# ratschlab/secedo

Hardware: AMD Instinct MI355X
Metric: cell-pair x locus updates/sec (similarity matrix) (higher is better)
Workload: dtype int64; 1 GPU; C3: 8000 cells x 100000 loci; entries=24345058, kept_entries=24223307, reads=23997029, block_cells=128, tiles=2016, normalization=ADD_MIN, max_fragment_length=1000, num_threads=8, parallelism=single GPU, backend=none, world_size=1, rccl_world_size=1

## Files before the change

include/secedo_simmat.h:

```cpp
#ifndef SECEDO_SIMMAT_H
#define SECEDO_SIMMAT_H

#include <stdint.h>

#ifdef __cplusplus
extern "C" {
#endif

#define SECEDO_OK 0
#define SECEDO_E_INVALID_ARG (-1)
#define SECEDO_E_INVALID_NORMALIZATION (-2)
#define SECEDO_E_NO_DEVICE (-3)
#define SECEDO_E_HIP (-4)
#define SECEDO_E_STATE (-5)
#define SECEDO_E_LIMIT (-6)

#define SECEDO_NORM_ADD_MIN 0
#define SECEDO_NORM_EXPONENTIATE 1
#define SECEDO_NORM_SCALE_MAX_1 2

int secedo_simmat_normalization_from_string(const char *name);

const char *secedo_simmat_last_error(void);
const char *secedo_simmat_version(void);
int secedo_simmat_device_count(void);

int secedo_simmat_compute(const uint32_t *chr_locus_off, uint32_t n_chr, const uint32_t *locus_pos,
                          const uint64_t *locus_entry_off, const uint32_t *read_ids,
                          const uint16_t *id_base16, const uint32_t *id_base32,
                          const uint32_t *group_id_to_pos, uint32_t n_groups, uint32_t num_cells,
                          uint32_t max_fragment_length, double mutation_rate,
                          double homozygous_rate, double seq_error_rate, uint32_t num_threads,
                          int normalization, double *out);
int secedo_simmat_set_devices(const int *device_ids, uint32_t n_devices);
int secedo_simmat_get_devices(int *device_ids, uint32_t capacity);

int secedo_simmat_staging_acquire(const uint64_t bytes[5], void *ptrs[5]);
void secedo_simmat_staging_release(void);

void secedo_simmat_release_cache(void);

typedef struct secedo_simmat secedo_simmat_t;

int secedo_simmat_create(secedo_simmat_t **handle, int device_id);
void secedo_simmat_destroy(secedo_simmat_t *handle);

int secedo_simmat_set_pileup(secedo_simmat_t *handle, const uint32_t *chr_locus_off, uint32_t n_chr,
                             const uint32_t *locus_pos, const uint64_t *locus_entry_off,
                             const uint32_t *read_ids, const uint16_t *id_base16,
                             const uint32_t *id_base32, const uint32_t *group_id_to_pos,
                             uint32_t n_groups);

int secedo_simmat_set_pileup_device(secedo_simmat_t *handle, const uint32_t *d_chr_locus_off,
                                    uint32_t n_chr, const uint32_t *d_locus_pos,
                                    const uint64_t *d_locus_entry_off, const uint32_t *d_read_ids,
                                    const uint16_t *d_id_base16, const uint32_t *d_id_base32,
                                    const uint32_t *d_group_id_to_pos, uint32_t n_groups,
                                    uint32_t n_loci, uint64_t n_entries);

int secedo_simmat_set_packing(secedo_simmat_t *handle, int mode);
int secedo_simmat_used_device_packing(const secedo_simmat_t *handle);

int secedo_simmat_prepare(secedo_simmat_t *handle, uint32_t num_cells, uint32_t max_fragment_length,
                          uint32_t num_threads, uint32_t block_cells, void *stream);

uint32_t secedo_simmat_num_tiles(const secedo_simmat_t *handle);
uint32_t secedo_simmat_block_cells(const secedo_simmat_t *handle);
uint64_t secedo_simmat_acc_elems(const secedo_simmat_t *handle);
uint64_t secedo_simmat_num_entries(const secedo_simmat_t *handle);
uint64_t secedo_simmat_num_reads(const secedo_simmat_t *handle);
uint64_t secedo_simmat_num_loci(const secedo_simmat_t *handle);

uint64_t secedo_simmat_pair_bound(const secedo_simmat_t *handle);
uint32_t secedo_simmat_max_read_entries(const secedo_simmat_t *handle);
int secedo_simmat_cell_squares(secedo_simmat_t *handle, uint64_t *d_out , void *stream);
int secedo_simmat_set_scale_bounds(secedo_simmat_t *handle, uint64_t pair_bound, uint32_t max_read_entries);
int secedo_simmat_set_pair_bound(secedo_simmat_t *handle, uint64_t pair_bound);
int secedo_simmat_scale_bounds_state(const secedo_simmat_t *handle);
int secedo_simmat_scale_log2(const secedo_simmat_t *handle);

int secedo_simmat_zero_acc(secedo_simmat_t *handle, int64_t *d_acc, void *stream);
int secedo_simmat_accumulate(secedo_simmat_t *handle, double mutation_rate, double homozygous_rate,
                             double seq_error_rate, uint32_t tile_begin, uint32_t tile_end,
                             int64_t *d_acc, void *stream);
int secedo_simmat_assign(secedo_simmat_t *handle, double mutation_rate, double homozygous_rate,
                         double seq_error_rate, uint32_t tile_begin, uint32_t tile_end, int64_t *d_acc,
                         void *stream);
int secedo_simmat_finalize(secedo_simmat_t *handle, int normalization, const int64_t *d_acc,
                           double *d_out, void *stream);
int secedo_simmat_assign_finalize(secedo_simmat_t *handle, double mutation_rate, double homozygous_rate,
                                  double seq_error_rate, int normalization, int64_t *d_acc, double *d_out,
                                  void *stream);
int secedo_simmat_tiles_of_rows(const secedo_simmat_t *handle, uint32_t row_begin, uint32_t row_end,
                                uint32_t *tile_ids, uint32_t *n_tile_ids);
int secedo_simmat_accumulate_list(secedo_simmat_t *handle, double mutation_rate, double homozygous_rate,
                                  double seq_error_rate, const uint32_t *tile_ids, uint32_t n_tile_ids,
                                  int64_t *d_acc, void *stream);
int secedo_simmat_assign_list(secedo_simmat_t *handle, double mutation_rate, double homozygous_rate,
                              double seq_error_rate, const uint32_t *tile_ids, uint32_t n_tile_ids,
                              int64_t *d_acc, void *stream);
int secedo_simmat_max_of_tiles(secedo_simmat_t *handle, const int64_t *d_acc, const uint32_t *tile_ids,
                               uint32_t n_tile_ids, double *max_value, void *stream);
int secedo_simmat_finalize_rows_max(secedo_simmat_t *handle, int normalization, const int64_t *d_acc,
                                    uint32_t row_begin, uint32_t row_end, double max_value, double *d_out_rows,
                                    void *stream);
int secedo_simmat_finalize_rows(secedo_simmat_t *handle, int normalization, const int64_t *d_acc,
                                uint32_t row_begin, uint32_t row_end, double *d_out_rows, void *stream);
int secedo_simmat_finalize_raw(secedo_simmat_t *handle, const int64_t *d_acc, double *d_out,
                               void *stream);

int secedo_simmat_last_counts(secedo_simmat_t *handle, uint64_t *updates, uint64_t *read_pairs);
int secedo_simmat_last_accumulate_ms(secedo_simmat_t *handle, float *ms);
int secedo_simmat_last_pair_kernel_ms(secedo_simmat_t *handle, float *ms);
const char *secedo_simmat_pair_kernel(const secedo_simmat_t *handle);
int secedo_simmat_last_correction_fused(const secedo_simmat_t *handle);
int secedo_simmat_last_locus_words(const secedo_simmat_t *handle);
uint32_t secedo_simmat_last_workgroups(const secedo_simmat_t *handle);
int secedo_simmat_debug_flag_lists(secedo_simmat_t *handle, uint64_t *n_flagged, uint32_t *grp, uint32_t *rec,
                                   uint32_t *idx);

double secedo_simmat_llr(uint32_t x_s, uint32_t x_d, double mutation_rate, double homozygous_rate,
                         double seq_error_rate);
double secedo_simmat_llr_closed_form(uint32_t x_s, uint32_t x_d, double mutation_rate, double homozygous_rate,
                                     double seq_error_rate);

int secedo_is_significant(const uint16_t *base_count , double seq_error_rate,
                          uint32_t cell_proportion);

int secedo_filter(const uint32_t *chr_locus_off, uint32_t n_chr, const uint32_t *locus_pos,
                  const uint64_t *locus_entry_off, const uint32_t *read_ids, const uint16_t *id_base16,
                  const uint32_t *id_base32, const uint32_t *id_to_pos, uint32_t n_groups,
                  double seq_error_rate, uint32_t cell_proportion, uint32_t *out_chr_locus_off,
                  uint32_t *out_locus_pos, uint64_t *out_locus_entry_off, uint32_t *out_read_ids,
                  void *out_id_base, uint64_t *out_n_loci, uint64_t *out_n_entries, double *avg_coverage);

int secedo_filter_device(const uint32_t *d_chr_locus_off, uint32_t n_chr, const uint32_t *d_locus_pos,
                         const uint64_t *d_locus_entry_off, const uint32_t *d_read_ids,
                         const uint16_t *d_id_base16, const uint32_t *d_id_base32, const uint32_t *d_id_to_pos,
                         uint32_t n_groups, uint32_t n_loci, uint64_t n_entries, double seq_error_rate,
                         uint32_t cell_proportion, uint32_t *d_out_chr_locus_off, uint32_t *d_out_locus_pos,
                         uint64_t *d_out_locus_entry_off, uint32_t *d_out_read_ids, void *d_out_id_base,
                         uint64_t *out_n_loci, uint64_t *out_n_entries, double *avg_coverage, void *stream);

typedef struct secedo_pileup_info {
    uint64_t n_loci;
    uint64_t n_entries;
    uint32_t num_cells;
    uint32_t max_read_length;
} secedo_pileup_info;

int secedo_pileup_read(const char *path, const uint16_t *id_to_group, uint32_t n_ids, uint32_t max_coverage,
                       const uint32_t *positions, uint64_t n_positions, int compute_max_read_len,
                       int write_bin, secedo_pileup_info *info, uint32_t *locus_pos,
                       uint64_t *locus_entry_off, uint32_t *read_ids, uint16_t *id_base16);
const char *secedo_pileup_last_error(void);

#ifdef __cplusplus
}
#endif
#endif
```

secedo_amd/_lib.py:

```python
from __future__ import annotations

import ctypes as C
import os

import numpy as np

HERE = os.path.dirname(os.path.abspath(__file__))
LIB_PATH = os.environ.get("SECEDO_LIB_PATH") or os.path.join(HERE, "libsecedo_simmat.so")

OK = 0
E_INVALID_ARG = -1
E_INVALID_NORMALIZATION = -2
E_NO_DEVICE = -3
E_HIP = -4
E_STATE = -5
E_LIMIT = -6

_u16p = C.POINTER(C.c_uint16)
_u32p = C.POINTER(C.c_uint32)
_u64p = C.POINTER(C.c_uint64)
_f64p = C.POINTER(C.c_double)
_vp = C.c_void_p


class PileupInfo(C.Structure):
    _fields_ = [("n_loci", C.c_uint64), ("n_entries", C.c_uint64), ("num_cells", C.c_uint32),
                ("max_read_length", C.c_uint32)]


class SpectralInfo(C.Structure):
    _fields_ = [("cycles", C.c_uint32), ("block_products", C.c_uint32), ("converged", C.c_uint32),
                ("reserved", C.c_uint32), ("max_residual_vectors", C.c_double),
                ("max_residual_values", C.c_double)]


ALLREDUCE_SUM_FN = C.CFUNCTYPE(C.c_int, C.c_void_p, C.c_void_p, C.c_uint64, C.c_void_p)


class SynthSpec(C.Structure):
    _fields_ = [
        ("num_cells", C.c_uint32), ("num_loci", C.c_uint32), ("num_chromosomes", C.c_uint32),
        ("gap_max", C.c_uint32), ("new_frag_prob", C.c_double), ("frag_min", C.c_uint32),
        ("frag_max", C.c_uint32), ("base_error", C.c_double), ("mate_frac", C.c_double),
        ("seed", C.c_uint64),
    ]


SIGNATURES = {
    "secedo_simmat_normalization_from_string": (C.c_int, [C.c_char_p]),
    "secedo_simmat_last_error": (C.c_char_p, []),
    "secedo_simmat_version": (C.c_char_p, []),
    "secedo_simmat_device_count": (C.c_int, []),
    "secedo_simmat_compute": (C.c_int, [_vp, C.c_uint32, _vp, _vp, _vp, _vp, _vp, _vp, C.c_uint32,
                                        C.c_uint32, C.c_uint32, C.c_double, C.c_double, C.c_double,
                                        C.c_uint32, C.c_int, _vp]),
    "secedo_simmat_release_cache": (None, []),
    "secedo_simmat_staging_acquire": (C.c_int, [_vp, _vp]),
    "secedo_simmat_staging_release": (None, []),
    "secedo_simmat_create": (C.c_int, [C.POINTER(_vp), C.c_int]),
    "secedo_simmat_destroy": (None, [_vp]),
    "secedo_simmat_set_pileup": (C.c_int, [_vp, _vp, C.c_uint32, _vp, _vp, _vp, _vp, _vp, _vp,
                                           C.c_uint32]),
    "secedo_simmat_set_pileup_device": (C.c_int, [_vp, _vp, C.c_uint32, _vp, _vp, _vp, _vp, _vp, _vp,
                                                  C.c_uint32, C.c_uint32, C.c_uint64]),
    "secedo_simmat_set_packing": (C.c_int, [_vp, C.c_int]),
    "secedo_simmat_used_device_packing": (C.c_int, [_vp]),
    "secedo_simmat_prepare": (C.c_int, [_vp, C.c_uint32, C.c_uint32, C.c_uint32, C.c_uint32, _vp]),
    "secedo_simmat_num_tiles": (C.c_uint32, [_vp]),
    "secedo_simmat_block_cells": (C.c_uint32, [_vp]),
    "secedo_simmat_acc_elems": (C.c_uint64, [_vp]),
    "secedo_simmat_num_entries": (C.c_uint64, [_vp]),
    "secedo_simmat_num_reads": (C.c_uint64, [_vp]),
    "secedo_simmat_num_loci": (C.c_uint64, [_vp]),
    "secedo_simmat_zero_acc": (C.c_int, [_vp, _vp, _vp]),
    "secedo_simmat_accumulate": (C.c_int, [_vp, C.c_double, C.c_double, C.c_double, C.c_uint32,
                                           C.c_uint32, _vp, _vp]),
    "secedo_simmat_finalize": (C.c_int, [_vp, C.c_int, _vp, _vp, _vp]),
    "secedo_simmat_tiles_of_rows": (C.c_int, [_vp, C.c_uint32, C.c_uint32, _vp, C.POINTER(C.c_uint32)]),
    "secedo_simmat_assign": (C.c_int, [_vp, C.c_double, C.c_double, C.c_double, C.c_uint32, C.c_uint32, _vp, _vp]),
    "secedo_simmat_assign_list": (C.c_int, [_vp, C.c_double, C.c_double, C.c_double, _vp, C.c_uint32, _vp, _vp]),
    "secedo_simmat_assign_finalize": (C.c_int, [_vp, C.c_double, C.c_double, C.c_double, C.c_int, _vp, _vp, _vp]),
    "secedo_simmat_accumulate_list": (C.c_int, [_vp, C.c_double, C.c_double, C.c_double, _vp, C.c_uint32, _vp, _vp]),
    "secedo_simmat_max_of_tiles": (C.c_int, [_vp, _vp, _vp, C.c_uint32, C.POINTER(C.c_double), _vp]),
    "secedo_simmat_finalize_rows_max": (C.c_int, [_vp, C.c_int, _vp, C.c_uint32, C.c_uint32, C.c_double, _vp, _vp]),
    "secedo_simmat_finalize_rows": (C.c_int, [_vp, C.c_int, _vp, C.c_uint32, C.c_uint32, _vp, _vp]),
    "secedo_simmat_finalize_raw": (C.c_int, [_vp, _vp, _vp, _vp]),
    "secedo_simmat_last_counts": (C.c_int, [_vp, _u64p, _u64p]),
    "secedo_simmat_last_accumulate_ms": (C.c_int, [_vp, C.POINTER(C.c_float)]),
    "secedo_simmat_last_pair_kernel_ms": (C.c_int, [_vp, C.POINTER(C.c_float)]),
    "secedo_simmat_pair_kernel": (C.c_char_p, [_vp]),
    "secedo_simmat_last_correction_fused": (C.c_int, [_vp]),
    "secedo_simmat_last_locus_words": (C.c_int, [_vp]),
    "secedo_simmat_last_workgroups": (C.c_uint32, [_vp]),
    "secedo_simmat_debug_flag_lists": (C.c_int, [_vp, _u64p, _vp, _vp, _vp]),
    "secedo_simmat_llr": (C.c_double, [C.c_uint32, C.c_uint32, C.c_double, C.c_double, C.c_double]),
    "secedo_simmat_llr_closed_form": (C.c_double, [C.c_uint32, C.c_uint32, C.c_double, C.c_double, C.c_double]),
    "secedo_simmat_pair_bound": (C.c_uint64, [_vp]),
    "secedo_simmat_set_pair_bound": (C.c_int, [_vp, C.c_uint64]),
    "secedo_simmat_max_read_entries": (C.c_uint32, [_vp]),
    "secedo_simmat_cell_squares": (C.c_int, [_vp, _vp, _vp]),
    "secedo_simmat_set_scale_bounds": (C.c_int, [_vp, C.c_uint64, C.c_uint32]),
    "secedo_simmat_scale_log2": (C.c_int, [_vp]),
    "secedo_simmat_scale_bounds_state": (C.c_int, [_vp]),
    "secedo_simmat_set_devices": (C.c_int, [C.POINTER(C.c_int), C.c_uint32]),
    "secedo_simmat_get_devices": (C.c_int, [C.POINTER(C.c_int), C.c_uint32]),
    "secedo_is_significant": (C.c_int, [_vp, C.c_double, C.c_uint32]),
    "secedo_filter": (C.c_int, [_vp, C.c_uint32, _vp, _vp, _vp, _vp, _vp, _vp, C.c_uint32, C.c_double,
                                C.c_uint32, _vp, _vp, _vp, _vp, _vp, _u64p, _u64p, _f64p]),
    "secedo_filter_device": (C.c_int, [_vp, C.c_uint32, _vp, _vp, _vp, _vp, _vp, _vp, C.c_uint32, C.c_uint32,
                                       C.c_uint64, C.c_double, C.c_uint32, _vp, _vp, _vp, _vp, _vp, _u64p,
                                       _u64p, _f64p, _vp]),
    "secedo_pileup_read": (C.c_int, [C.c_char_p, _vp, C.c_uint32, C.c_uint32, _vp, C.c_uint64, C.c_int, C.c_int,
                                     C.POINTER(PileupInfo), _vp, _vp, _vp, _vp]),
    "secedo_pileup_last_error": (C.c_char_p, []),
    "secedo_em_refine_device": (C.c_int, [C.c_int, _vp, C.c_uint32, C.c_uint64, _vp, _vp, _vp, C.c_uint32, C.c_double,
                                          _vp, C.c_uint32, C.c_uint32, C.POINTER(C.c_uint32), _vp]),
    "secedo_em_refine": (C.c_int, [C.c_int, _vp, C.c_uint32, _vp, _vp, _vp, C.c_uint32, C.c_double, _vp, C.c_uint32,
                                   C.c_uint32, C.POINTER(C.c_uint32)]),
    "secedo_laplacian_device": (C.c_int, [_vp, C.c_uint32, _vp, _vp]),
    "secedo_spectral_eigs_device": (C.c_int, [C.c_int, _vp, C.c_uint32, C.c_uint32, C.c_uint32, C.c_double,
                                              C.c_uint32, _vp, _vp, C.POINTER(SpectralInfo), _vp]),
    "secedo_spectral_eigs_rows_device": (C.c_int, [C.c_int, _vp, C.c_uint32, C.c_uint32, C.c_uint32, C.c_uint32,
                                                   C.c_uint32, C.c_double, C.c_uint32, _vp, _vp,
                                                   C.POINTER(SpectralInfo), _vp, _vp, _vp]),
    "secedo_spectral_eigs": (C.c_int, [C.c_int, _vp, C.c_uint32, C.c_uint32, C.c_uint32, C.c_double, C.c_uint32,
                                       _vp, _vp, C.POINTER(SpectralInfo)]),
}

_lib = None


class SecedoError(RuntimeError):
    def __init__(self, code, message):
        super().__init__("secedo_simmat error %d: %s" % (code, message))
        self.code = code


class InvalidNormalization(ValueError):
    """The reference throws std::logic_error here (similarity_matrix.cpp:264)."""


def lib():
    global _lib
    if _lib is None:
        if not os.path.exists(LIB_PATH):
            raise ImportError(
                "%s is missing: build it with `python -c 'import __graft_entry__ as g; g.build()'` "
                "or `make -C secedo_amd/csrc` (there is no fallback implementation)" % LIB_PATH)
        try:
            import torch
        except ImportError:
            pass
        l = C.CDLL(LIB_PATH)
        for name, (res, args) in SIGNATURES.items():
            f = getattr(l, name)
            f.restype = res
            f.argtypes = args
        _lib = l
    return _lib


def check(rc):
    if rc == OK:
        return
    msg = lib().secedo_simmat_last_error().decode(errors="replace")
    if rc == E_INVALID_NORMALIZATION:
        raise InvalidNormalization(msg)
    raise SecedoError(rc, msg)


def ptr(a):
    return None if a is None else a.ctypes.data
```

secedo_amd/csrc/pack_device.hip:

```cpp
#include "pack_device.hpp"

#include <hip/hip_runtime.h>
#include <hipcub/hipcub.hpp>

#include <algorithm>
#include <chrono>
#include <cstdio>
#include <cstdlib>
#include <cstring>
#include <functional>

namespace secedo {

DeviceArena::~DeviceArena() {
    if (p) (void)hipFree(p);
}

DevicePacked::~DevicePacked() {
    if (side) (void)hipStreamDestroy(side);
    if (ev_fork) (void)hipEventDestroy(ev_fork);
    if (ev_join) (void)hipEventDestroy(ev_join);
    if (ev_offsets) (void)hipEventDestroy(ev_offsets);
    if (ev_flush) (void)hipEventDestroy(ev_flush);
    if (mailbox) (void)hipHostFree(mailbox);
// ... 20 lines not shown
}

namespace {

constexpr int TPB = 256;

inline uint32_t blocks_for(uint64_t n) {
    return static_cast<uint32_t>(std::max<uint64_t>(1, std::min<uint64_t>((n + TPB - 1) / TPB, 1u << 16)));
}

struct Scalars {
    uint32_t error;
    uint32_t need_host;
    uint32_t num_ranges;
    uint32_t max_read_id;
    uint32_t regroup;
    uint32_t long_reads;
    uint32_t split_changed;
    uint32_t id_exceeded;
    uint32_t max_read_entries;
    uint32_t caps_wrong;
    uint32_t n_multi_id;
    uint32_t reads_total;
    uint32_t n_wide;
    uint32_t max_range_span;
    unsigned long long id_space;
    unsigned long long multi_entries;
    unsigned long long pair_bound;
};

struct Mailbox {
    Scalars sc;
    unsigned long long totals;
    unsigned long long seq;
};

__global__ void k_publish(const Scalars *sc, const unsigned long long *totals, Mailbox *box, unsigned long long seq) {
    if (threadIdx.x == 0) {
        box->sc = *sc;
        box->totals = totals ? *totals : 0ull;
        __hip_atomic_store(&box->seq, seq, __ATOMIC_RELEASE, __HIP_MEMORY_SCOPE_SYSTEM);
    }
}

hipError_t read_scalars(DevicePacked &pk, hipStream_t stream, const Scalars *sc, const unsigned long long *totals,
                        Scalars *out, unsigned long long *out_totals, const std::function<void()> &behind = nullptr) {
    static const bool plain = [] {
        const char *e = std::getenv("SECEDO_PACK_READBACK");
        return e && std::strcmp(e, "memcpy") == 0;
    }();
    hipError_t e;
    if (!plain && !pk.mailbox && !pk.mailbox_failed) {
        if (hipHostMalloc(&pk.mailbox, sizeof(Mailbox), hipHostMallocCoherent) == hipSuccess) {
            std::memset(pk.mailbox, 0, sizeof(Mailbox));
        } else {
            (void)hipGetLastError();
            pk.mailbox = nullptr;
            pk.mailbox_failed = true;
        }
    }
    if (!plain && pk.mailbox) {
        Mailbox *box = static_cast<Mailbox *>(pk.mailbox);
        const unsigned long long seq = ++pk.mailbox_seq;
        hipLaunchKernelGGL(k_publish, dim3(1), dim3(64), 0, stream, sc, totals, box, seq);
        if ((e = hipGetLastError()) != hipSuccess) return e;
        if (behind) behind();
        bool arrived = false;
        for (unsigned spins = 0;; ++spins) {
            if (__atomic_load_n(&box->seq, __ATOMIC_ACQUIRE) == seq) {
                arrived = true;
                break;
            }
            if ((spins & 0xFFFu) == 0xFFFu) {
                const hipError_t q = hipStreamQuery(stream);
                if (q != hipErrorNotReady) {
                    arrived = __atomic_load_n(&box->seq, __ATOMIC_ACQUIRE) == seq;
                    if (q != hipSuccess) return q;
                    break;
                }
            }
        }
        if (arrived) {
            *out = box->sc;
            if (out_totals) *out_totals = box->totals;
            return hipSuccess;
        }
    } else if (behind) {
        behind();
    }
    if (out_totals) {
        *out_totals = 0;
        if (totals && (e = hipMemcpyAsync(out_totals, totals, 8, hipMemcpyDeviceToHost, stream)) != hipSuccess) return e;
    }
    if ((e = hipMemcpyAsync(out, sc, sizeof(*out), hipMemcpyDeviceToHost, stream)) != hipSuccess) return e;
    return hipStreamSynchronize(stream);
}

struct HostTrace {
    bool on;
    std::chrono::steady_clock::time_point t0;
    HostTrace() : on(std::getenv("SECEDO_PACK_TRACE") != nullptr), t0(std::chrono::steady_clock::now()) {}
    void mark(const char *what) const {
        if (on)
            std::fprintf(stderr, "[pack-trace] %8.1f us  %s\n",
                         std::chrono::duration<double, std::micro>(std::chrono::steady_clock::now() - t0).count(), what);
    }
};

constexpr uint32_t kRankScanLimit = 8192;
constexpr int kNoRetry = 0, kRetryRadix = 1, kRetrySameScheme = 2;
constexpr int kMaxSplitRounds = 32;
constexpr uint32_t kIdSpaceFactor = 4;

struct Raw {
    const uint32_t *chr_locus_off;
    uint32_t n_chr;
    const uint32_t *locus_pos;
    const uint64_t *locus_entry_off;
    const uint32_t *read_ids;
    const uint16_t *id_base16;
    const uint32_t *id_base32;
    const uint32_t *g2p;
    uint32_t n_groups;
    uint32_t n_loci;
    uint32_t n_entries;
    __device__ __forceinline__ uint32_t id_base(uint32_t e) const {
        return id_base16 ? (uint32_t)id_base16[e] : id_base32[e];
    }
};

template <class T>
__device__ __forceinline__ uint32_t last_le(const T *a, uint32_t n, T x) {
    uint32_t lo = 0, hi = n;
    while (hi - lo > 1) {
        const uint32_t mid = lo + (hi - lo) / 2;
        if (a[mid] <= x) lo = mid; else hi = mid;
    }
    return lo;
}

__global__ __launch_bounds__(TPB) void k_entry_locus(Raw in, uint32_t *entry_locus, Scalars *sc) {
    const uint32_t lane = threadIdx.x & 63u;
    const uint32_t wave = (blockIdx.x * TPB + threadIdx.x) >> 6, n_waves = (gridDim.x * TPB) >> 6;
    for (uint32_t l = wave; l < in.n_loci; l += n_waves) {
        const uint32_t b = (uint32_t)in.locus_entry_off[l], e = (uint32_t)in.locus_entry_off[l + 1];
        for (uint32_t i = b + lane; i < e; i += 64u) entry_locus[i] = l;
        if (lane == 0u && l + 1 < in.n_loci && in.locus_pos[l + 1] <= in.locus_pos[l]) {
            const uint32_t c = last_le<uint32_t>(in.chr_locus_off, in.n_chr + 1, l);
            if (l + 1 < in.chr_locus_off[c + 1]) sc->error = 3;
        }
    }
}

__global__ __launch_bounds__(TPB) void k_id_range(Raw in, const uint32_t *entry_locus, uint32_t *id_max,
                                                 uint32_t *id_negmin, int vec) {
    __shared__ uint32_t s_hi[TPB / 64], s_neg[TPB / 64];
    const uint32_t E = in.n_entries;
    const uint32_t chunk = (E + gridDim.x - 1) / gridDim.x;
    uint32_t cur = min(E, blockIdx.x * chunk);
    const uint32_t e1 = min(E, cur + chunk);
    if (cur >= e1) return;
    uint32_t c = last_le<uint32_t>(in.chr_locus_off, in.n_chr + 1, entry_locus[cur]);
    while (cur < e1) {
        uint32_t c_end = (uint32_t)in.locus_entry_off[in.chr_locus_off[c + 1]];
        while (c_end <= cur && c + 1 < in.n_chr) {
            ++c;
            c_end = (uint32_t)in.locus_entry_off[in.chr_locus_off[c + 1]];
        }
        const uint32_t seg_end = (c + 1 < in.n_chr) ? min(e1, c_end) : e1;
        uint32_t hi = 0, neg = 0;
        uint32_t s_cur = cur, s_end = seg_end;
        if (vec) {
            const uint32_t a = min(seg_end, (cur + 3u) & ~3u), b = max(a, seg_end & ~3u);
            if (threadIdx.x < a - cur) {
                const uint32_t id = in.read_ids[cur + threadIdx.x];
                hi = max(hi, id);
                neg = max(neg, ~id);
            }
            if (threadIdx.x < seg_end - b) {
                const uint32_t id = in.read_ids[b + threadIdx.x];
                hi = max(hi, id);
                neg = max(neg, ~id);
            }
            const uint4 *src = reinterpret_cast<const uint4 *>(in.read_ids);
            for (uint32_t q = a / 4u + threadIdx.x; q < b / 4u; q += TPB * 4) {
                uint4 v[4];
#pragma unroll
                for (int u = 0; u < 4; ++u) v[u] = q + (uint32_t)u * TPB < b / 4u ? src[q + (uint32_t)u * TPB] : src[q];
#pragma unroll
                for (int u = 0; u < 4; ++u) {
                    hi = max(max(hi, v[u].x), max(max(v[u].y, v[u].z), v[u].w));
                    neg = max(max(neg, ~v[u].x), max(max(~v[u].y, ~v[u].z), ~v[u].w));
                }
            }
            s_cur = s_end = seg_end;
        }
        for (uint32_t e = s_cur + threadIdx.x; e < s_end; e += TPB * 8) {
            uint32_t id[8];
#pragma unroll
            for (int u = 0; u < 8; ++u) {
                const uint32_t eu = e + (uint32_t)u * TPB;
                id[u] = eu < s_end ? in.read_ids[eu] : in.read_ids[e];
            }
#pragma unroll
            for (int u = 0; u < 8; ++u) {
                hi = max(hi, id[u]);
                neg = max(neg, ~id[u]);
            }
        }
        for (int off = 32; off > 0; off >>= 1) {
            hi = max(hi, (uint32_t)__shfl_down(hi, off));
            neg = max(neg, (uint32_t)__shfl_down(neg, off));
        }
        __syncthreads();
        if ((threadIdx.x & 63u) == 0) {
            s_hi[threadIdx.x >> 6] = hi;
            s_neg[threadIdx.x >> 6] = neg;
        }
        __syncthreads();
        if (threadIdx.x == 0) {
            for (int w = 1; w < TPB / 64; ++w) {
                hi = max(hi, s_hi[w]);
                neg = max(neg, s_neg[w]);
            }
            atomicMax(&id_max[c], hi);
            atomicMax(&id_negmin[c], neg);
        }
        cur = seg_end;
    }
}

__global__ void k_id_bases(uint32_t n_chr, const uint32_t *id_max, const uint32_t *id_negmin, uint32_t *id_base,
                           unsigned long long assumed_space, Scalars *sc) {
    if (threadIdx.x != 0 || blockIdx.x != 0) return;
    unsigned long long sum = 0;
    uint32_t top = 0;
    for (uint32_t c = 0; c < n_chr; ++c) {
        id_base[c] = (uint32_t)min(sum, 0xFFFFFFFFull);
        const uint32_t lo = ~id_negmin[c];
        if ((id_max[c] | id_negmin[c]) != 0u) sum += (unsigned long long)(id_max[c] - lo) + 1ull;
        top = max(top, id_max[c]);
    }
    id_base[n_chr] = (uint32_t)min(sum, 0xFFFFFFFFull);
    sc->id_space = sum;
    sc->max_read_id = top;
    if (assumed_space && sum > assumed_space) sc->id_exceeded = 1;
}

__global__ void k_entry_keys(Raw in, const uint32_t *entry_locus, uint32_t id_bits, unsigned long long *key,
                             uint32_t *val) {
    for (uint32_t e = blockIdx.x * TPB + threadIdx.x; e < in.n_entries; e += gridDim.x * TPB) {
        const uint32_t c = last_le<uint32_t>(in.chr_locus_off, in.n_chr + 1, entry_locus[e]);
        key[e] = ((unsigned long long)c << id_bits) | in.read_ids[e];
        val[e] = e;
    }
}

constexpr uint32_t kSlocLocusMask = 0x3FFFFFFFu;
__device__ __forceinline__ uint32_t sloc_pack(uint32_t locus, uint32_t id_base) { return locus | (id_base << 30); }
__device__ __forceinline__ uint32_t sloc_locus(uint32_t v) { return v & kSlocLocusMask; }
__device__ __forceinline__ uint32_t sloc_base(uint32_t v) { return v >> 30; }

__global__ void k_sorted_locus(Raw in, const uint32_t *sval, const uint32_t *entry_locus, uint32_t n, uint32_t *sloc) {
    for (uint32_t s = blockIdx.x * TPB + threadIdx.x; s < n; s += gridDim.x * TPB)
        sloc[s] = sloc_pack(entry_locus[sval[s]], in.id_base(sval[s]));
}

constexpr uint32_t kChrLds = 1024;
struct ChrTables {
    uint32_t first[kChrLds + 1], base[kChrLds], min_id[kChrLds];
};
__device__ __forceinline__ bool chr_tables_load(const Raw &in, const uint32_t *id_base, const uint32_t *id_negmin,
                                                ChrTables &t) {
    const bool in_lds = in.n_chr <= kChrLds;
    if (in_lds) {
        for (uint32_t i = threadIdx.x; i <= in.n_chr; i += blockDim.x) t.first[i] = in.chr_locus_off[i];
        for (uint32_t i = threadIdx.x; i < in.n_chr; i += blockDim.x) {
            t.base[i] = id_base[i];
            t.min_id[i] = ~id_negmin[i];
        }
    }
    __syncthreads();
    return in_lds;
}
__device__ __forceinline__ uint32_t dense_id(const Raw &in, const uint32_t *id_base, const uint32_t *id_negmin,
                                             const ChrTables &t, bool in_lds, uint32_t locus, uint32_t id) {
    if (in_lds) {
        const uint32_t c = last_le<uint32_t>(t.first, in.n_chr + 1, locus);
        return t.base[c] + (id - t.min_id[c]);
    }
    const uint32_t c = last_le<uint32_t>(in.chr_locus_off, in.n_chr + 1, locus);
    return id_base[c] + (id - ~id_negmin[c]);
}

__global__ void k_id_hist(Raw in, const uint32_t *entry_locus, const uint32_t *id_base, const uint32_t *id_negmin,
                          const Scalars *sc, uint32_t *dense, uint32_t *hist) {
    if (sc->id_exceeded) return;
    __shared__ ChrTables tables;
    const bool in_lds = chr_tables_load(in, id_base, id_negmin, tables);
    for (uint32_t e = blockIdx.x * TPB + threadIdx.x; e < in.n_entries; e += gridDim.x * TPB) {
        const uint32_t d = dense_id(in, id_base, id_negmin, tables, in_lds, entry_locus[e], in.read_ids[e]);
        dense[e] = d;
        atomicAdd(&hist[d], 1u);
    }
}

__global__ void k_id_scatter(const uint32_t *dense, uint32_t n, const uint32_t *id_off, const Scalars *sc,
                             uint32_t *hist, uint32_t *grouped) {
    if (sc->id_exceeded) return;
    for (uint32_t e = blockIdx.x * TPB + threadIdx.x; e < n; e += gridDim.x * TPB) {
        const uint32_t d = dense[e];
        grouped[id_off[d] + atomicSub(&hist[d], 1u) - 1u] = e;
    }
}

__global__ void k_id_rank(Raw in, const uint32_t *dense, const uint32_t *id_off, const uint32_t *grouped,
                          const uint32_t *entry_locus, unsigned long long *skey, uint32_t *sval, uint32_t *sloc,
                          Scalars *sc) {
    const bool void_run = sc->id_exceeded != 0;
    for (uint32_t p = blockIdx.x * TPB + threadIdx.x; p < in.n_entries; p += gridDim.x * TPB) {
        if (void_run) {
            skey[p] = p;
            sval[p] = p;
            sloc[p] = 0;
            continue;
        }
        const uint32_t e = grouped[p];
        const uint32_t d = dense[e];
        const uint32_t b = id_off[d], n = id_off[d + 1] - b;
        uint32_t rank = p - b;
        if (n > kRankScanLimit) {
            sc->regroup = 1;
        } else if (n > 1) {
            rank = 0;
            for (uint32_t q = b; q < b + n; ++q) rank += grouped[q] < e ? 1u : 0u;
        }
        skey[b + rank] = d;
        sval[b + rank] = e;
        sloc[b + rank] = sloc_pack(entry_locus[e], in.id_base(e));
    }
}

constexpr uint32_t kFlagBlock = 4096;
__global__ void k_id_store(Raw in, const uint32_t *entry_locus, const uint32_t *id_base, const uint32_t *id_negmin,
                           const Scalars *sc, uint32_t *dense, uint32_t *last, int vec) {
    if (sc->id_exceeded) return;
    __shared__ ChrTables tables;
    const bool in_lds = chr_tables_load(in, id_base, id_negmin, tables);
    const uint32_t n = in.n_entries, stride = gridDim.x * TPB;
    for (uint32_t q = blockIdx.x * TPB + threadIdx.x; q < (n + 3u) / 4u; q += stride) {
        const uint32_t e0 = q * 4u;
        uint32_t l[4], id[4], d[4];
        if (vec && e0 + 4u <= n) {
            const uint4 lv = reinterpret_cast<const uint4 *>(entry_locus)[q];
            const uint4 iv = reinterpret_cast<const uint4 *>(in.read_ids)[q];
            l[0] = lv.x, l[1] = lv.y, l[2] = lv.z, l[3] = lv.w;
            id[0] = iv.x, id[1] = iv.y, id[2] = iv.z, id[3] = iv.w;
        } else {
#pragma unroll
            for (int u = 0; u < 4; ++u) {
                const uint32_t e = min(e0 + (uint32_t)u, n - 1u);
                l[u] = entry_locus[e];
                id[u] = in.read_ids[e];
            }
        }
#pragma unroll
        for (int u = 0; u < 4; ++u) d[u] = dense_id(in, id_base, id_negmin, tables, in_lds, l[u], id[u]);
        if (e0 + 4u <= n) {
            reinterpret_cast<uint4 *>(dense)[q] = make_uint4(d[0], d[1], d[2], d[3]);
#pragma unroll
            for (int u = 0; u < 4; ++u) last[d[u]] = e0 + (uint32_t)u + 1u;
        } else {
            for (uint32_t u = 0; e0 + u < n; ++u) {
                dense[e0 + u] = d[u];
                last[d[u]] = e0 + u + 1u;
            }
        }
    }
}
__global__ void k_id_check(uint32_t n, const Scalars *sc, const uint32_t *dense, const uint32_t *last, uint8_t *multi) {
    if (sc->id_exceeded) return;
    const uint32_t stride = gridDim.x * TPB;
    for (uint32_t q = blockIdx.x * TPB + threadIdx.x; q < (n + 3u) / 4u; q += stride) {
        const uint32_t e0 = q * 4u;
        uint32_t d[4], w[4];
        if (e0 + 4u <= n) {
            const uint4 dv = reinterpret_cast<const uint4 *>(dense)[q];
            d[0] = dv.x, d[1] = dv.y, d[2] = dv.z, d[3] = dv.w;
        } else {
#pragma unroll
            for (int u = 0; u < 4; ++u) d[u] = dense[min(e0 + (uint32_t)u, n - 1u)];
        }
#pragma unroll
        for (int u = 0; u < 4; ++u) w[u] = last[d[u]];
#pragma unroll
        for (int u = 0; u < 4; ++u) {
            const uint32_t e = e0 + (uint32_t)u;
            if (e < n && w[u] != e + 1u) {
                multi[e] = 1;
                multi[w[u] - 1u] = 1;
            }
        }
    }
}
__global__ __launch_bounds__(TPB) void k_flag_count(const uint8_t *multi, uint32_t *block_sum) {
    __shared__ uint32_t part[TPB / 64];
    static_assert(kFlagBlock == TPB * 16, "a thread takes 16 consecutive flags");
    const uint4 w = reinterpret_cast<const uint4 *>(multi + (size_t)blockIdx.x * kFlagBlock)[threadIdx.x];
    uint32_t n = ((w.x * 0x01010101u) >> 24) + ((w.y * 0x01010101u) >> 24) + ((w.z * 0x01010101u) >> 24)
            + ((w.w * 0x01010101u) >> 24);
    for (int off = 32; off > 0; off >>= 1) n += __shfl_down(n, off);
    if ((threadIdx.x & 63u) == 0u) part[threadIdx.x >> 6] = n;
    __syncthreads();
    if (threadIdx.x == 0u) {
        for (int w2 = 1; w2 < TPB / 64; ++w2) n += part[w2];
        block_sum[blockIdx.x] = n;
    }
}
constexpr int TPB_SCAN = 1024;
__global__ __launch_bounds__(TPB_SCAN) void k_flag_scan(const uint32_t *block_sum, uint32_t n_blocks, uint32_t *block_off,
                                                       uint32_t *m_idx_end, Scalars *sc) {
    constexpr int TPB = TPB_SCAN;
    __shared__ uint32_t part[TPB / 64];
    __shared__ uint32_t carry;
    if (threadIdx.x == 0u) carry = 0;
    __syncthreads();
    const uint32_t lane = threadIdx.x & 63u, wv = threadIdx.x >> 6;
    for (uint32_t base = 0; base < n_blocks; base += TPB) {
        const uint32_t i = base + threadIdx.x;
        const uint32_t v = i < n_blocks ? block_sum[i] : 0u;
        uint32_t incl = v;
        for (int off = 1; off < 64; off <<= 1) {
            const uint32_t up = __shfl_up(incl, off);
            if (lane >= (uint32_t)off) incl += up;
        }
        if (lane == 63u) part[wv] = incl;
        __syncthreads();
        uint32_t before = carry;
        for (uint32_t w2 = 0; w2 < wv; ++w2) before += part[w2];
        if (i < n_blocks) block_off[i] = before + incl - v;
        __syncthreads();
        if (threadIdx.x == TPB - 1) carry = before + incl;
        __syncthreads();
    }
    if (threadIdx.x == 0u) {
        *m_idx_end = carry;
        if (sc) sc->n_multi_id = carry;
    }
}
__global__ __launch_bounds__(TPB) void k_compact_m(Raw in, const uint8_t *multi, const uint32_t *block_off,
                                                  uint32_t *m_idx, uint32_t *m_entry) {
    __shared__ uint32_t part[TPB / 64];
    const uint32_t lane = threadIdx.x & 63u, wv = threadIdx.x >> 6;
    const uint32_t e0 = blockIdx.x * kFlagBlock + threadIdx.x * 16u;
    const uint4 w = reinterpret_cast<const uint4 *>(multi + (size_t)blockIdx.x * kFlagBlock)[threadIdx.x];
    const uint32_t words[4] = {w.x, w.y, w.z, w.w};
    uint32_t mine = 0;
#pragma unroll
    for (int i = 0; i < 4; ++i) mine += (words[i] * 0x01010101u) >> 24;
    uint32_t incl = mine;
    for (int off = 1; off < 64; off <<= 1) {
        const uint32_t up = __shfl_up(incl, off);
        if (lane >= (uint32_t)off) incl += up;
    }
    if (lane == 63u) part[wv] = incl;
    __syncthreads();
    uint32_t j = block_off[blockIdx.x] + incl - mine;
    for (uint32_t w2 = 0; w2 < wv; ++w2) j += part[w2];
    const uint32_t n = in.n_entries;
    __shared__ uint32_t tile[TPB * 17];
    {
        uint32_t jj = j;
#pragma unroll
        for (int i = 0; i < 16; ++i) {
            tile[threadIdx.x * 17u + (uint32_t)i] = jj;
            jj += (words[i >> 2] >> ((i & 3) * 8)) & 1u;
        }
    }
    __syncthreads();
#pragma unroll
    for (int k = 0; k < 16; ++k) {
        const uint32_t i = (uint32_t)k * TPB + threadIdx.x;
        const uint32_t e = blockIdx.x * kFlagBlock + i;
        if (e < n) m_idx[e] = tile[(i >> 4) * 17u + (i & 15u)];
    }
#pragma unroll
    for (int i = 0; i < 16; ++i) {
        const uint32_t e = e0 + (uint32_t)i;
        if (e >= n) break;
        if ((words[i >> 2] >> ((i & 3) * 8)) & 1u) m_entry[j++] = e;
    }
}
__global__ __launch_bounds__(TPB) void k_pflag_count(const uint32_t *entry32, uint32_t n, uint32_t *block_sum) {
    __shared__ uint32_t part[TPB / 64];
    const uint32_t b0 = blockIdx.x * kFlagBlock + threadIdx.x;
    uint32_t c = 0;
#pragma unroll
    for (int k = 0; k < 16; ++k) {
        const uint32_t e = b0 + (uint32_t)k * TPB;
        c += (e < n && (entry32[e] & (kC_Tail | kC_Multi)) != 0u) ? 1u : 0u;
    }
    for (int off = 32; off > 0; off >>= 1) c += __shfl_down(c, off);
    if ((threadIdx.x & 63u) == 0u) part[threadIdx.x >> 6] = c;
    __syncthreads();
    if (threadIdx.x == 0u) {
        for (int w = 1; w < TPB / 64; ++w) c += part[w];
        block_sum[blockIdx.x] = c;
    }
}
__global__ __launch_bounds__(TPB) void k_pflag_compact(const uint32_t *entry32, const uint4 *entry, uint32_t n,
                                                      const uint32_t *block_off, uint4 *rec, uint32_t *idx,
                                                      uint32_t *chunk_pre, unsigned long long *chunk_mask) {
    constexpr int WAVES = TPB / 64;
    static_assert(16 * WAVES == 64, "one wave scans the (round, wave) counts");
    __shared__ uint32_t cnt[16 * WAVES];
    const uint32_t lane = threadIdx.x & 63u, wv = threadIdx.x >> 6;
    const uint32_t b0 = blockIdx.x * kFlagBlock + threadIdx.x;
    unsigned long long m[16];
#pragma unroll
    for (int k = 0; k < 16; ++k) {
        const uint32_t e = b0 + (uint32_t)k * TPB;
        m[k] = __ballot(e < n && (entry32[e] & (kC_Tail | kC_Multi)) != 0u);
        if (lane == 0u) cnt[k * WAVES + wv] = (uint32_t)__popcll(m[k]);
    }
    __syncthreads();
    if (threadIdx.x < 64u) {
        const uint32_t v = cnt[threadIdx.x];
        uint32_t incl = v;
        for (int off = 1; off < 64; off <<= 1) {
            const uint32_t up = __shfl_up(incl, off);
            if (lane >= (uint32_t)off) incl += up;
        }
        cnt[threadIdx.x] = incl - v;
    }
    __syncthreads();
    const uint32_t base = block_off[blockIdx.x];
#pragma unroll
    for (int k = 0; k < 16; ++k) {
        const uint32_t e = b0 + (uint32_t)k * TPB;
        const uint32_t before = base + cnt[k * WAVES + wv];
        if (lane == 0u) {
            const uint32_t chunk = (blockIdx.x * kFlagBlock + (uint32_t)k * TPB) / 64u + wv;
            chunk_pre[chunk] = before;
            chunk_mask[chunk] = m[k];
        }
        if ((m[k] >> lane) & 1ull) {
            const uint32_t j = before + (uint32_t)__popcll(m[k] & ((1ull << lane) - 1ull));
            rec[j] = entry[e];
            idx[j] = e;
        }
    }
}
__global__ __launch_bounds__(TPB) void k_pflag_compact_masks(const unsigned long long *chunk_mask, const uint4 *entry,
                                                            const uint32_t *block_off, uint4 *rec, uint32_t *idx,
                                                            uint32_t *chunk_pre) {
    constexpr int WAVES = TPB / 64;
    constexpr uint32_t CHUNKS = kFlagBlock / 64u;
    static_assert(CHUNKS == 64, "one wave scans the chunks' counts");
    __shared__ unsigned long long mask[CHUNKS];
    __shared__ uint32_t pre[CHUNKS];
    const uint32_t lane = threadIdx.x & 63u, wv = threadIdx.x >> 6;
    const uint32_t chunk0 = blockIdx.x * CHUNKS;
    if (threadIdx.x < 64u) {
        const unsigned long long m = chunk_mask[chunk0 + threadIdx.x];
        const uint32_t v = (uint32_t)__popcll(m);
        uint32_t incl = v;
        for (int off = 1; off < 64; off <<= 1) {
            const uint32_t up = __shfl_up(incl, off);
            if (lane >= (uint32_t)off) incl += up;
        }
        mask[threadIdx.x] = m;
        pre[threadIdx.x] = incl - v;
        chunk_pre[chunk0 + threadIdx.x] = block_off[blockIdx.x] + incl - v;
    }
    __syncthreads();
    const uint32_t base = block_off[blockIdx.x];
#pragma unroll 4
    for (uint32_t c = wv; c < CHUNKS; c += WAVES) {
        const unsigned long long m = mask[c];
        if ((m >> lane) & 1ull) {
            const uint32_t e = (chunk0 + c) * 64u + lane;
            const uint32_t j = base + pre[c] + (uint32_t)__popcll(m & ((1ull << lane) - 1ull));
            rec[j] = entry[e];
            idx[j] = e;
        }
    }
}
__global__ __launch_bounds__(TPB) void k_pflag_groups(const uint32_t *blk_off, size_t n_off, const uint32_t *chunk_pre,
                                                     const unsigned long long *chunk_mask, uint32_t *grp) {
    for (size_t i = (size_t)blockIdx.x * TPB + threadIdx.x; i < n_off; i += (size_t)gridDim.x * TPB) {
        const uint32_t d = blk_off[i], c = d >> 6, r = d & 63u;
        grp[i] = chunk_pre[c] + (r ? (uint32_t)__popcll(chunk_mask[c] & ((1ull << r) - 1ull)) : 0u);
    }
}
uint32_t flag_blocks(uint32_t n_entries) { return std::max<uint32_t>(1u, (n_entries + kFlagBlock - 1) / kFlagBlock); }
struct FlagScratch {
    uint32_t nb;
    uint32_t *block_sum, *block_off, *chunk_pre;
    unsigned long long *chunk_mask;
    FlagScratch(void *scratch, uint32_t n_entries) : nb(flag_blocks(n_entries)) {
        block_sum = block_off = chunk_pre = nullptr;
        chunk_mask = nullptr;
        if (!scratch) return;
        block_sum = static_cast<uint32_t *>(scratch);
        block_off = block_sum + nb;
        chunk_pre = block_off + nb;
        chunk_mask = reinterpret_cast<unsigned long long *>(chunk_pre + 64 * (size_t)nb + 2);
    }
    static size_t bytes(uint32_t n_entries) {
        const size_t nb = flag_blocks(n_entries);
        return (2 * nb + 64 * nb + 2) * 4 + 64 * nb * 8;
    }
};
void flag_groups(const FlagScratch &fs, const uint32_t *blk_off, size_t n_off, uint32_t *grp, hipStream_t stream) {
    if (!n_off) return;
    const uint32_t blocks = (uint32_t)std::min<size_t>((n_off + TPB - 1) / TPB, 256 * 32);
    hipLaunchKernelGGL(k_pflag_groups, dim3(blocks), dim3(TPB), 0, stream, blk_off, n_off, fs.chunk_pre, fs.chunk_mask, grp);
}
void flag_lists_from_masks(const FlagScratch &fs, const uint4 *entry, const uint32_t *blk_off, size_t n_off,
                           uint32_t *grp, uint4 *rec, uint32_t *idx, hipStream_t stream) {
    hipLaunchKernelGGL(k_flag_scan, dim3(1), dim3(TPB_SCAN), 0, stream, fs.block_sum, fs.nb, fs.block_off,
                       fs.chunk_pre + 64 * (size_t)fs.nb, static_cast<Scalars *>(nullptr));
    hipLaunchKernelGGL(k_pflag_compact_masks, dim3(fs.nb), dim3(TPB), 0, stream, fs.chunk_mask, entry, fs.block_off, rec,
                       idx, fs.chunk_pre);
    flag_groups(fs, blk_off, n_off, grp, stream);
}

__global__ void k_m_fields(Raw in, const uint32_t *eloc, const uint32_t *dense, const uint32_t *last,
                           const uint32_t *m_idx, const uint32_t *m_entry, uint32_t n_m, uint32_t *rid_m,
                           uint32_t *idb_m, uint32_t *eloc_m, uint32_t *winner_m, uint32_t *count_m) {
    for (uint32_t j = blockIdx.x * TPB + threadIdx.x; j < n_m; j += gridDim.x * TPB) {
        const uint32_t e = m_entry[j];
        rid_m[j] = in.read_ids[e];
        idb_m[j] = in.id_base(e);
        eloc_m[j] = eloc[e];
        const uint32_t w = m_idx[last[dense[e]] - 1u];
        winner_m[j] = w;
        atomicAdd(&count_m[w], 1u);
    }
}
__global__ void k_group_scatter(const uint32_t *winner_m, uint32_t n_m, const uint32_t *goff, uint32_t *count_m,
                                uint32_t *members, uint32_t *g_begin, uint32_t *g_len) {
    for (uint32_t j = blockIdx.x * TPB + threadIdx.x; j < n_m; j += gridDim.x * TPB) {
        const uint32_t w = winner_m[j];
        const uint32_t b = goff[w], n = goff[w + 1] - b;
        members[b + atomicSub(&count_m[w], 1u) - 1u] = j;
        g_begin[j] = b;
        g_len[j] = n;
    }
}
__global__ void k_group_rank(Raw sub, const uint32_t *members, const uint32_t *g_begin, const uint32_t *g_len,
                             const uint32_t *eloc_m, uint32_t n_m, unsigned long long *skey, uint32_t *sval,
                             uint32_t *sloc, Scalars *sc) {
    for (uint32_t p = blockIdx.x * TPB + threadIdx.x; p < n_m; p += gridDim.x * TPB) {
        const uint32_t m = members[p];
        const uint32_t b = g_begin[m], n = g_len[m];
        uint32_t rank = p - b;
        if (n > kRankScanLimit) {
            sc->regroup = 1;
        } else {
            rank = 0;
            for (uint32_t q = b; q < b + n; ++q) rank += members[q] < m ? 1u : 0u;
        }
        skey[b + rank] = b;
        sval[b + rank] = m;
        sloc[b + rank] = sloc_pack(eloc_m[m], sub.id_base(m));
    }
}

constexpr uint32_t kCibBits = 7;
constexpr uint32_t kNoEntry = 0xFFFFFFFFu;
constexpr uint32_t kSingle = 0x80000000u;
constexpr uint32_t kSingleBaseShift = 29;
constexpr uint32_t kSingleTail = 4u;

struct Ranks {
    const uint32_t *m_idx, *unm;
    const uint32_t *arank;
    __device__ __forceinline__ uint32_t operator()(uint32_t e) const { return unm ? e - unm[m_idx[e]] : arank[e]; }
};
struct UnmarkedM {
    const uint32_t *mark_m;
    uint32_t n_m;
    __device__ __forceinline__ uint32_t operator()(uint32_t j) const { return j < n_m ? 1u - mark_m[j] : 0u; }
};
__global__ void k_arank_m(const uint32_t *unm, const uint32_t *m_entry, uint32_t n_m, uint32_t n, uint32_t *arank_m,
                          Scalars *sc) {
    for (uint32_t j = blockIdx.x * TPB + threadIdx.x; j < n_m; j += gridDim.x * TPB) arank_m[j] = m_entry[j] - unm[j];
    if (blockIdx.x == 0 && threadIdx.x == 0) sc->reads_total = n - unm[n_m];
}
__global__ void k_rbeg(Raw in, Ranks rank, uint32_t *rbeg) {
    for (uint32_t c = blockIdx.x * TPB + threadIdx.x; c <= in.n_chr; c += gridDim.x * TPB)
        rbeg[c] = rank((uint32_t)in.locus_entry_off[in.chr_locus_off[c]]);
}
struct HeadKeepOp {
    const unsigned long long *skey;
    const uint32_t *keep;
    const uint32_t *split;
    __device__ __forceinline__ unsigned long long operator()(uint32_t s) const {
        const unsigned long long head = (s == 0 || skey[s] != skey[s - 1] || (split && split[s])) ? 1ull : 0ull;
        return head | ((unsigned long long)keep[s] << 32);
    }
};
__device__ __forceinline__ uint32_t incl_reads(unsigned long long v) { return (uint32_t)v; }
__device__ __forceinline__ uint32_t incl_kept(unsigned long long v) { return (uint32_t)(v >> 32); }

__global__ void k_dup_mark(Raw in, const unsigned long long *skey, const uint32_t *sval,
                           const uint32_t *sloc, const uint32_t *split, uint32_t n, uint32_t *keep,
                           uint32_t *mark) {
    for (uint32_t s = blockIdx.x * TPB + threadIdx.x; s < n; s += gridDim.x * TPB) {
        const uint32_t e = sval[s];
        const uint32_t l = sloc_locus(sloc[s]);
        const bool same_read = s > 0 && skey[s] == skey[s - 1];
        mark[e] = (same_read && !(split && split[s])) ? 0u : 1u;
        if (s == 0) mark[n] = 0u;
        if (same_read && sloc_locus(sloc[s - 1]) == l) continue;
        uint32_t stored = s;
        bool have = true;
        keep[s] = 0u;
        for (uint32_t t = s + 1; t < n && skey[t] == skey[s] && sloc_locus(sloc[t]) == l; ++t) {
            keep[t] = 0u;
            if (have) {
                if (sloc_base(sloc[t]) != sloc_base(sloc[stored])) have = false;
            } else {
                stored = t;
                have = true;
            }
        }
        if (have) keep[stored] = 1u;
    }
}

__global__ void k_runs_csr(Raw in, const unsigned long long *incl, const uint32_t *sval,
                           const uint32_t *sloc, uint32_t n, uint32_t *run_start, uint32_t *read_locus,
                           uint8_t *read_base) {
    for (uint32_t s = blockIdx.x * TPB + threadIdx.x; s < n; s += gridDim.x * TPB) {
        const unsigned long long cur = incl[s], prev = s ? incl[s - 1] : 0ull;
        if (incl_reads(cur) != incl_reads(prev)) run_start[incl_reads(cur) - 1] = s;
        if (s == n - 1) run_start[incl_reads(cur)] = n;
        if (incl_kept(cur) != incl_kept(prev)) {
            const uint32_t k = incl_kept(prev), v = sloc[s];
            read_locus[k] = sloc_locus(v);
            read_base[k] = (uint8_t)sloc_base(v);
        }
    }
}

__global__ __launch_bounds__(TPB) void k_read_info(Raw in, const unsigned long long *incl, const uint32_t *run_start,
                                                  const uint32_t *sval, const uint32_t *sloc,
                                                  const uint32_t *arank, uint32_t mfl, uint32_t *run_rank,
                                                  uint32_t *rbeg, uint32_t *read_off, Scalars *sc) {
    __shared__ unsigned long long part[TPB / 64];
    __shared__ uint32_t part_len[TPB / 64];
    const uint32_t n = in.n_entries;
    const uint32_t n_runs = n ? incl_reads(incl[n - 1]) : 0u;
    unsigned long long multi = 0;
    uint32_t longest = 0;
    for (uint32_t r = blockIdx.x * TPB + threadIdx.x; r < n_runs; r += gridDim.x * TPB) {
        const uint32_t s0 = run_start[r], s1 = run_start[r + 1];
        const uint32_t e0 = sval[s0];
        const uint32_t p0 = in.locus_pos[sloc_locus(sloc[s0])], p1 = in.locus_pos[sloc_locus(sloc[s1 - 1])];
        if (p1 - p0 >= mfl) sc->long_reads = 1;
        if ((unsigned long long)p1 + mfl > 0xFFFFFFFFull) sc->need_host = 1;
        const uint32_t rk = arank[e0];
        run_rank[r] = rk;
        const uint32_t k0 = s0 ? incl_kept(incl[s0 - 1]) : 0u, k1 = incl_kept(incl[s1 - 1]);
        read_off[r] = k0;
        if (r == n_runs - 1) read_off[n_runs] = k1;
        if (k1 - k0 > 1) multi += k1 - k0;
        longest = max(longest, k1 - k0);
    }
    if (rbeg) {
        for (uint32_t c = blockIdx.x * TPB + threadIdx.x; c <= in.n_chr; c += gridDim.x * TPB)
            rbeg[c] = arank[(uint32_t)in.locus_entry_off[in.chr_locus_off[c]]];
    }
    for (int off = 32; off > 0; off >>= 1) {
        multi += __shfl_down(multi, off);
        longest = max(longest, (uint32_t)__shfl_down(longest, off));
    }
    if ((threadIdx.x & 63) == 0) {
        part[threadIdx.x >> 6] = multi;
        part_len[threadIdx.x >> 6] = longest;
    }
    __syncthreads();
    if (threadIdx.x == 0) {
        unsigned long long sum = 0;
        uint32_t len = 0;
        for (int w = 0; w < TPB / 64; ++w) {
            sum += part[w];
            len = max(len, part_len[w]);
        }
        if (sum) atomicAdd(&sc->multi_entries, sum);
        if (len > 1) atomicMax(&sc->max_read_entries, len);
    }
}

__global__ void k_completed(Raw in, Ranks rank, const uint32_t *rbeg, uint32_t mfl, uint32_t *cnt, Scalars *sc) {
    for (uint32_t l = blockIdx.x * TPB + threadIdx.x; l < in.n_loci; l += gridDim.x * TPB) {
        const uint32_t c = last_le<uint32_t>(in.chr_locus_off, in.n_chr + 1, l);
        const uint32_t pos = in.locus_pos[l], l0 = in.chr_locus_off[c];
        if ((unsigned long long)pos + mfl > 0xFFFFFFFFull && in.locus_entry_off[l + 1] > in.locus_entry_off[l])
            sc->need_host = 1;
        uint32_t done = 0;
        if (pos >= mfl && in.locus_pos[l0] <= pos - mfl) {
            const uint32_t lp = l0 + last_le<uint32_t>(in.locus_pos + l0, l - l0 + 1, pos - mfl);
            done = rank((uint32_t)in.locus_entry_off[lp + 1]) - rbeg[c];
        }
        cnt[l] = done;
    }
}

__global__ __launch_bounds__(TPB) void k_flush_chain(Raw in, const uint32_t *cnt, uint32_t threshold,
                                                    const Scalars *sc, uint32_t *flushed_out,
                                                    uint32_t *flush_loci, uint32_t *flush_count, Ranks rank,
                                                    const uint32_t *rbeg, uint32_t *tail_begin) {
    __shared__ uint32_t buf[2048];
    __shared__ uint32_t hits[2048];
    __shared__ uint32_t s_flushed, s_listed, s_hits;
    const uint32_t c = blockIdx.x;
    const uint32_t l0 = in.chr_locus_off[c], l1 = in.chr_locus_off[c + 1];
    if (threadIdx.x == 0) {
        s_flushed = 0;
        s_listed = 0;
    }
    for (uint32_t base = l0; base < l1; base += 2048) {
        const uint32_t n = min(2048u, l1 - base);
        __syncthreads();
        for (uint32_t i = threadIdx.x; i < n; i += TPB) buf[i] = cnt[base + i];
        __syncthreads();
        if (threadIdx.x == 0) {
            uint32_t f = s_flushed, h = 0;
            if (sc->long_reads) {
                for (uint32_t i = 0; i < n; ++i) {
                    const uint32_t v = buf[i];
                    if (v - f >= threshold) {
                        f = v;
                        hits[h++] = base + i;
                    }
                }
            } else {
                for (uint32_t i = 0; i < n; ++i) {
                    const uint32_t v = buf[i];
                    if (v - f >= threshold) f = v;
                }
            }
            s_flushed = f;
            s_hits = h;
        }
        __syncthreads();
        const uint32_t h = s_hits, listed = s_listed;
        for (uint32_t i = threadIdx.x; i < h; i += TPB) flush_loci[l0 + listed + i] = hits[i];
        __syncthreads();
        if (threadIdx.x == 0) s_listed = listed + h;
    }
    __syncthreads();
    if (threadIdx.x == 0) {
        flushed_out[c] = s_flushed;
        flush_count[c] = s_listed;
    }
    if (tail_begin) {
        __shared__ uint32_t s_first;
        const unsigned long long want = (unsigned long long)rbeg[c] + s_flushed;
        uint32_t lo = (uint32_t)in.locus_entry_off[l0], hi = (uint32_t)in.locus_entry_off[l1];
        while (lo < hi) {
            const uint32_t step = (hi - lo + TPB - 1) / TPB;
            const unsigned long long probe = (unsigned long long)lo + (unsigned long long)threadIdx.x * step;
            const bool reached = probe < hi && (unsigned long long)rank((uint32_t)probe) >= want;
            __syncthreads();
            if (threadIdx.x == 0) s_first = TPB;
            __syncthreads();
            if (reached) atomicMin(&s_first, threadIdx.x);
            __syncthreads();
            const uint32_t first = s_first;
            if (first == TPB) {
                lo = lo + ((hi - lo - 1) / step) * step + 1;
            } else {
                hi = lo + first * step;
                if (first) lo = lo + (first - 1) * step + 1;
            }
        }
        if (threadIdx.x == 0) tail_begin[c] = lo;
    }
}

__global__ void k_split_update(Raw in, const unsigned long long *skey, const uint32_t *sloc, uint32_t mfl, const uint32_t *flush_loci,
                               const uint32_t *flush_count, uint32_t *split, Scalars *sc) {
    const uint32_t n = in.n_entries;
    for (uint32_t s = blockIdx.x * TPB + threadIdx.x; s < n; s += gridDim.x * TPB) {
        if (s > 0 && skey[s] == skey[s - 1]) continue;
        uint32_t end = s + 1;
        while (end < n && skey[end] == skey[s]) ++end;
        if (end == s + 1) continue;
        const uint32_t l_first = sloc_locus(sloc[s]);
        const uint32_t p_first = in.locus_pos[l_first], p_last = in.locus_pos[sloc_locus(sloc[end - 1])];
        if (p_last - p_first < mfl) continue;
        const uint32_t c = last_le<uint32_t>(in.chr_locus_off, in.n_chr + 1, l_first);
        const uint32_t *fl = flush_loci + in.chr_locus_off[c];
        const uint32_t n_fl = flush_count[c];
        uint32_t seg_start = p_first, l_prev = l_first;
        for (uint32_t t = s + 1; t < end; ++t) {
            const uint32_t l_t = sloc_locus(sloc[t]);
            uint32_t cut = 0;
            if (l_t != l_prev) {
                uint32_t lo = 0, hi = n_fl;
                const unsigned long long reach = (unsigned long long)seg_start + mfl;
                while (lo < hi) {
                    const uint32_t mid = lo + (hi - lo) / 2;
                    if (fl[mid] <= l_prev || in.locus_pos[fl[mid]] < reach) lo = mid + 1; else hi = mid;
                }
                if (lo < n_fl && fl[lo] <= l_t) {
                    cut = 1;
                    seg_start = in.locus_pos[l_t];
                }
            }
            if (split[t] != cut) {
                split[t] = cut;
                sc->split_changed = 1;
            }
            l_prev = l_t;
        }
    }
}

__device__ __forceinline__ unsigned long long bin_key(uint32_t blk, uint32_t l, uint32_t cib, uint32_t lbits) {
    return ((((unsigned long long)blk << lbits) | l) << kCibBits) | cib;
}

__global__ void k_keys2(Raw in, const uint32_t *sval, const unsigned long long *incl,
                        const uint32_t *read_locus, const uint32_t *run_rank, const uint32_t *read_off,
                        uint32_t num_cells, uint32_t B,
                        uint32_t lbits, unsigned long long *key2, uint32_t *val2, uint32_t *t_read,
                        uint32_t *krank, uint8_t *kflags, unsigned long long *entry_kc, const uint32_t *entry_map,
                        uint32_t *blk_cnt_add, uint32_t L, Scalars *sc) {
    const uint32_t n = in.n_entries;
    for (uint32_t s = blockIdx.x * TPB + threadIdx.x; s < n; s += gridDim.x * TPB) {
        const unsigned long long cur = incl[s], prev = s ? incl[s - 1] : 0ull;
        const uint32_t e_out = entry_map ? entry_map[sval[s]] : sval[s];
        if (incl_kept(cur) == incl_kept(prev)) {
            if (entry_kc) entry_kc[e_out] = kNoEntry;
            continue;
        }
        const uint32_t k = incl_kept(prev);
        const uint32_t group = in.id_base(sval[s]) >> 2;
        uint32_t cell = 0;
        if (group >= in.n_groups) {
            sc->error = 1;
        } else {
            cell = in.g2p[group];
            if (cell >= num_cells) {
                sc->error = 2;
                cell = 0;
            }
        }
        const uint32_t blk = cell / B, cib = cell - blk * B;
        if (key2) {
            key2[k] = bin_key(blk, read_locus[k], cib, lbits);
            val2[k] = k;
        }
        const uint32_t r = incl_reads(cur) - 1;
        t_read[k] = r;
        krank[k] = run_rank[r];
        kflags[k] = (uint8_t)((in.id_base(sval[s]) & 3u) | (read_off[r + 1] - read_off[r] > 1u ? 4u : 0u));
        if (entry_kc) entry_kc[e_out] = ((unsigned long long)((blk << kCibBits) | cib) << 32) | k;
        if (blk_cnt_add) atomicAdd(&blk_cnt_add[(size_t)blk * (L + 1) + read_locus[k]], 1u);
    }
}

__device__ __forceinline__ uint32_t tile_locus(const uint32_t *s_off, uint32_t lo, uint32_t hi, uint32_t e) {
    while (hi - lo > 1u) {
        const uint32_t mid = (lo + hi) >> 1;
        if (s_off[mid] <= e) lo = mid; else hi = mid;
    }
    return lo;
}

__global__ __launch_bounds__(TPB) void k_bin_hist(Raw in, uint32_t nb, uint32_t TL, unsigned long long *__restrict__ entry_kc,
                                                 const uint32_t *__restrict__ m_idx, uint32_t num_cells,
                                                 uint32_t B_log2, uint32_t *__restrict__ blk_cnt, Scalars *sc,
                                                 uint32_t g2p_lds) {
    extern __shared__ uint32_t lds_hist[];
    __shared__ uint32_t s_off[65];
    static_assert(TPB >= 65, "one thread per offset");
    const uint32_t L = in.n_loci, TLP = TL + 1u, TL_log2 = 31u - (uint32_t)__clz((int)TL);
    const uint32_t n_tiles = (L + TL - 1u) / TL;
    constexpr int U = 4;
    uint16_t *s_g2p = reinterpret_cast<uint16_t *>(lds_hist + nb * TLP);
    if (g2p_lds) {
        for (uint32_t i = threadIdx.x; i < in.n_groups; i += TPB) s_g2p[i] = (uint16_t)min(in.g2p[i], 0xFFFFu);
    }
    for (uint32_t tile = blockIdx.x; tile < n_tiles; tile += gridDim.x) {
        const uint32_t l0 = tile * TL, n_l = min(TL, L - l0);
        for (uint32_t i = threadIdx.x; i < nb * TLP; i += TPB) lds_hist[i] = 0;
        if (threadIdx.x <= n_l) s_off[threadIdx.x] = (uint32_t)in.locus_entry_off[l0 + threadIdx.x];
        __syncthreads();
        const uint32_t eb = s_off[0], ee = s_off[n_l];
        for (uint32_t base = eb + threadIdx.x; base < ee; base += TPB * U) {
            uint32_t slot[U];
            constexpr uint32_t kNone = 0xFFFFFFFFu;
            if (m_idx) {
                uint32_t m0[U], m1[U], ib[U], cell[U];
#pragma unroll
                for (int u = 0; u < U; ++u) {
                    const uint32_t e = base + (uint32_t)u * TPB;
                    const bool in_tile = e < ee;
                    m0[u] = in_tile ? m_idx[e] : 0u;
                    m1[u] = in_tile ? m_idx[e + 1] : 1u;
                    ib[u] = in_tile ? in.id_base(e) : 0u;
                }
#pragma unroll
                for (int u = 0; u < U; ++u) {
                    const uint32_t group = ib[u] >> 2;
                    cell[u] = 0;
                    if (m1[u] == m0[u]) {
                        if (group >= in.n_groups) sc->error = 1;
                        else cell[u] = g2p_lds ? (uint32_t)s_g2p[group] : in.g2p[group];
                    }
                }
#pragma unroll
                for (int u = 0; u < U; ++u) {
                    slot[u] = kNone;
                    if (m1[u] != m0[u]) continue;
                    const uint32_t e = base + (uint32_t)u * TPB;
                    uint32_t c = cell[u];
                    if (c >= num_cells) {
                        sc->error = 2;
                        c = 0;
                    }
                    const uint32_t blk = c >> B_log2, cib = c - (blk << B_log2);
                    entry_kc[e] = ((unsigned long long)(((ib[u] & 3u) << kSingleBaseShift) | (blk << kCibBits) | cib) << 32)
                            | kSingle;
                    slot[u] = blk;
                }
            } else {
#pragma unroll
                for (int u = 0; u < U; ++u) {
                    const uint32_t e = base + (uint32_t)u * TPB;
                    const unsigned long long kc = e < ee ? entry_kc[e] : (unsigned long long)kNoEntry;
                    slot[u] = (uint32_t)kc != kNoEntry ? (uint32_t)(kc >> 32) >> kCibBits : kNone;
                }
            }
#pragma unroll
            for (int u = 0; u < U; ++u) {
                if (slot[u] == kNone) continue;
                const uint32_t j = tile_locus(s_off, 0u, n_l, base + (uint32_t)u * TPB);
                atomicAdd(&lds_hist[slot[u] * TLP + j], 1u);
            }
        }
        __syncthreads();
        for (uint32_t i = threadIdx.x; i < nb * TL; i += TPB) {
            const uint32_t b = i >> TL_log2, j = i & (TL - 1u);
            if (j < n_l) {
                blk_cnt[(size_t)b * (L + 1) + l0 + j] = lds_hist[b * TLP + j];
                if (l0 + j == L - 1) blk_cnt[(size_t)b * (L + 1) + L] = 0;
            }
        }
        __syncthreads();
    }
}

__global__ __launch_bounds__(TPB) void k_bin_place(Raw in, uint32_t nb, uint32_t TL,
                                                  const unsigned long long *__restrict__ entry_kc,
                                                  const uint32_t *__restrict__ blk_off, uint32_t B_log2, uint32_t bm_words,
                                                  const uint32_t *tail_begin,
                                                  unsigned long long *__restrict__ grouped, uint8_t *dupflag) {
    extern __shared__ uint32_t lds_hist[];
    __shared__ uint32_t s_off[65];
    __shared__ uint32_t s_tail[64];
    constexpr uint32_t NW = TPB / 64;
    constexpr int D = 4;
    const uint32_t lane = threadIdx.x & 63u, wv = threadIdx.x >> 6, L = in.n_loci, TLP = TL + 1u;
    const uint32_t TL_log2 = 31u - (uint32_t)__clz((int)TL);
    uint32_t *bm = lds_hist + nb * TLP + wv * bm_words;
    for (uint32_t i = lane; i < bm_words; i += 64u) bm[i] = 0;
    const uint32_t n_tiles = (L + TL - 1u) / TL;
    for (uint32_t tile = blockIdx.x; tile < n_tiles; tile += gridDim.x) {
        const uint32_t l0 = tile * TL, n_l = min(TL, L - l0);
        for (uint32_t i = threadIdx.x; i < nb * TL; i += TPB) {
            const uint32_t b = i >> TL_log2, j = i & (TL - 1u);
            if (j < n_l) lds_hist[b * TLP + j] = blk_off[(size_t)b * (L + 1) + l0 + j];
        }
        if (threadIdx.x <= n_l) s_off[threadIdx.x] = (uint32_t)in.locus_entry_off[l0 + threadIdx.x];
        if (threadIdx.x < n_l)
            s_tail[threadIdx.x] = tail_begin
                    ? tail_begin[last_le<uint32_t>(in.chr_locus_off, in.n_chr + 1, l0 + threadIdx.x)] : 0u;
        __syncthreads();
        const uint32_t per_wave = (n_l + NW - 1u) / NW;
        const uint32_t ja = min(n_l, wv * per_wave), jb = min(n_l, ja + per_wave);
        const uint32_t E0 = s_off[ja], E1 = s_off[jb];
        uint32_t cur = ja;
        bool twice = bm_words == 0u;
        auto close_locus = [&]() {
            const bool any_twice = __ballot(twice) != 0ull;
            if (lane == 0u) dupflag[l0 + cur] = any_twice ? 1 : 0;
            if (bm_words) {
                __builtin_amdgcn_fence(__ATOMIC_RELEASE, "wavefront");
                __builtin_amdgcn_wave_barrier();
                for (uint32_t i = lane; i < bm_words; i += 64u) bm[i] = 0;
                __builtin_amdgcn_fence(__ATOMIC_RELEASE, "wavefront");
                __builtin_amdgcn_wave_barrier();
            }
            twice = bm_words == 0u;
            ++cur;
        };
        auto chunk = [&](unsigned long long kc, uint32_t base) {
            const uint32_t e = base + lane;
            const bool valid = e < E1;
            const uint32_t j = valid ? tile_locus(s_off, cur, jb, e) : 0xFFFFFFFFu;
            const uint32_t chunk_end = min(E1, base + 64u);
            while (true) {
                if (valid && j == cur) {
                    uint32_t k = (uint32_t)kc;
                    if (k != kNoEntry) {
                        uint32_t cc = (uint32_t)(kc >> 32);
                        if (k & kSingle) {
                            k = kSingle | (e >= s_tail[cur] ? kSingleTail : 0u) | (cc >> kSingleBaseShift);
                            cc &= (1u << kSingleBaseShift) - 1u;
                        }
                        if (bm_words) {
                            const uint32_t cell = ((cc >> kCibBits) << B_log2) + (cc & ((1u << kCibBits) - 1u));
                            const uint32_t bit = 1u << (cell & 31u);
                            twice |= (atomicOr(&bm[cell >> 5], bit) & bit) != 0u;
                        }
                        const uint32_t pos = atomicAdd(&lds_hist[(cc >> kCibBits) * TLP + cur], 1u);
                        grouped[pos] = ((unsigned long long)((cc & ((1u << kCibBits) - 1u)) | ((l0 + cur) << kCibBits)) << 32) | k;
                    }
                }
                if (s_off[cur + 1] > chunk_end) break;
                close_locus();
                if (cur >= jb) break;
            }
        };
        unsigned long long ring[D];
#pragma unroll
        for (int d = 0; d < D; ++d) {
            const uint32_t e = E0 + (uint32_t)d * 64u + lane;
            ring[d] = e < E1 ? entry_kc[e] : (unsigned long long)kNoEntry;
        }
        for (uint32_t base = E0; base < E1; base += 64u * D) {
#pragma unroll
            for (int d = 0; d < D; ++d) {
                const uint32_t b = base + (uint32_t)d * 64u;
                if (b >= E1) break;
                const unsigned long long kc = ring[d];
                const uint32_t nxt = b + 64u * D + lane;
                ring[d] = nxt < E1 ? entry_kc[nxt] : (unsigned long long)kNoEntry;
                chunk(kc, b);
            }
        }
        while (cur < jb) close_locus();
        __syncthreads();
    }
}

__global__ __launch_bounds__(TPB) void k_group_counts(const unsigned long long *skey2, uint32_t n, uint32_t B,
                                                     uint32_t L, uint32_t lbits, uint32_t *blk_cnt,
                                                     unsigned long long *per_cell_sq) {
    constexpr uint32_t SLOTS = 512;
    __shared__ unsigned long long sq[SLOTS];
    __shared__ uint32_t first_cell;
    const uint32_t per_block = (n + gridDim.x - 1) / gridDim.x;
    const uint32_t d0 = blockIdx.x * per_block, d1 = min(n, d0 + per_block);
    for (uint32_t i = threadIdx.x; i < SLOTS; i += TPB) sq[i] = 0;
    if (threadIdx.x == 0 && d0 < n) {
        const unsigned long long key = skey2[d0];
        first_cell = (uint32_t)(key >> (kCibBits + lbits)) * B;
    }
    __syncthreads();
    for (uint32_t d = d0 + threadIdx.x; d < d1; d += TPB) {
        const unsigned long long key = skey2[d];
        const unsigned long long grp = key >> kCibBits;
        const uint32_t blk = (uint32_t)(grp >> lbits), l = (uint32_t)grp & ((1u << lbits) - 1u);
        if (d == 0 || skey2[d - 1] >> kCibBits != grp) {
            uint32_t len = 1;
            for (uint32_t t = d + 1; t < n && skey2[t] >> kCibBits == grp; ++t) ++len;
// ... 301 lines not shown
    t.entry32[d] = cib | (base << kC_BaseShift) | (tail ? kC_Tail : 0u) | (multi ? kC_Multi : 0u)
            | (wide ? kC_Wide : 0u) | (lrel << 16);
    if (t.mask32)
        t.mask32[d] = (masks & 0xFFu) | (((masks >> 16) & 0xFFu) << 8) | ((bases & 0xFFu) << 16)
                | (((bases >> 16) & 0xFFu) << 24);
    return multi || tail;
}

constexpr int TPB_REC = 512;
__global__ __launch_bounds__(TPB_REC) void k_entry_records(const unsigned long long *grouped, const uint32_t *blk_off,
                                                          uint32_t n, uint32_t nb, uint32_t L, uint32_t B,
                                                          uint32_t lbits, RecordTables t,
                                                          unsigned long long *per_cell_sq, Scalars *sc,
                                                          unsigned long long *chunk_mask, uint32_t *block_sum) {
    constexpr uint32_t SLOTS = 512;
    __shared__ unsigned long long sq[SLOTS];
    __shared__ uint32_t blk_start[1025];
    __shared__ uint32_t first_cell;
    __shared__ uint32_t n_flagged;
    constexpr int U = 4;
    static_assert(kFlagBlock % (TPB_REC * U) == 0, "whole rounds per block of the lists");
    const uint32_t d0 = blockIdx.x * kFlagBlock, d1 = min(n, d0 + kFlagBlock);
    if (threadIdx.x == 0) n_flagged = 0;
    for (uint32_t i = threadIdx.x; i < SLOTS; i += TPB_REC) sq[i] = 0;
    for (uint32_t i = threadIdx.x; i <= nb; i += TPB_REC) blk_start[i] = i < nb ? blk_off[(size_t)i * (L + 1)] : n;
    __syncthreads();
    auto block_of = [&](uint32_t p) {
        uint32_t lo = 0, hi = nb;
        while (hi - lo > 1) {
            const uint32_t mid = (lo + hi) >> 1;
            if (blk_start[mid] <= p) lo = mid; else hi = mid;
        }
        return lo;
    };
    if (threadIdx.x == 0 && d0 < n) first_cell = block_of(d0) * B;
    __syncthreads();
    const uint32_t lmask = (1u << lbits) - 1u;
    uint32_t wave_flagged = 0;
    for (uint32_t base = d0; base < d0 + kFlagBlock; base += TPB_REC * U) {
        if (base >= d1 && !chunk_mask) break;
        unsigned long long mine[U];
        uint32_t blk[U], linfo[U], same[U];
        uint4 rec[U];
#pragma unroll
        for (int u = 0; u < U; ++u) {
            const uint32_t p = base + (uint32_t)u * TPB_REC + threadIdx.x;
            mine[u] = p < d1 ? grouped[p] : (unsigned long long)kSingle;
        }
#pragma unroll
        for (int u = 0; u < U; ++u) {
            const uint32_t p = base + (uint32_t)u * TPB_REC + threadIdx.x;
            const uint32_t l = (uint32_t)(mine[u] >> (32 + kCibBits)) & lmask;
            blk[u] = p < d1 ? block_of(p) : 0u;
            linfo[u] = t.locus_rel[l];
            rec[u] = make_uint4(0u, 0u, 0u, 0u);
            if (((uint32_t)mine[u] & kSingle) == 0u) rec[u] = t.m_rec[(uint32_t)mine[u]];
        }
#pragma unroll
        for (int u = 0; u < U; ++u) {
            const uint32_t p = base + (uint32_t)u * TPB_REC + threadIdx.x;
            same[u] = 1;
            if (p < d1 && (linfo[u] & kLocusDup)) {
                const uint32_t l = (uint32_t)(mine[u] >> (32 + kCibBits)) & lmask;
                const uint32_t cib = (uint32_t)(mine[u] >> 32) & ((1u << kCibBits) - 1u);
                const size_t g = (size_t)blk[u] * (L + 1) + l;
                const uint32_t gb = blk_off[g], ge = blk_off[g + 1];
                if (ge - gb > kRankScanLimit) {
                    sc->regroup = 1;
                } else if (ge - gb > 1) {
                    same[u] = 0;
                    for (uint32_t q = gb; q < ge; ++q)
                        same[u] += ((uint32_t)(grouped[q] >> 32) & ((1u << kCibBits) - 1u)) == cib ? 1u : 0u;
                }
            }
        }
#pragma unroll
        for (int u = 0; u < U; ++u) {
            const uint32_t p = base + (uint32_t)u * TPB_REC + threadIdx.x;
            bool flagged = false;
            if (p < d1) {
                const uint32_t k = (uint32_t)mine[u], cib = (uint32_t)(mine[u] >> 32) & ((1u << kCibBits) - 1u);
                const uint32_t l = (uint32_t)(mine[u] >> (32 + kCibBits)) & lmask;
                const uint32_t cell = blk[u] * B + cib;
                flagged = emit_record(t, p, k, rec[u], cib, cell, l, linfo[u] & 0xFFFFu);
                const uint32_t rel = cell - first_cell;
                if (rel < SLOTS) atomicAdd(&sq[rel], (unsigned long long)same[u]);
                else atomicAdd(&per_cell_sq[cell], (unsigned long long)same[u]);
            }
            if (chunk_mask) {
                const unsigned long long m = __ballot(flagged);
                wave_flagged += (uint32_t)__popcll(m);
                if ((threadIdx.x & 63u) == 0u) chunk_mask[p >> 6] = m;
            }
        }
    }
    if (chunk_mask && (threadIdx.x & 63u) == 0u && wave_flagged) atomicAdd(&n_flagged, wave_flagged);
    __syncthreads();
    if (block_sum && threadIdx.x == 0) block_sum[blockIdx.x] = n_flagged;
    if (d0 < n)
        for (uint32_t i = threadIdx.x; i < SLOTS; i += TPB_REC)
            if (sq[i]) atomicAdd(&per_cell_sq[first_cell + i], sq[i]);
}

__global__ __launch_bounds__(TPB) void k_pair_bound(const unsigned long long *per_cell_sq, uint32_t n_cells_padded,
                                                   CapChoice caps, uint32_t assumed_counts, Scalars *sc) {
    __shared__ unsigned long long s_best[TPB / 64];
    unsigned long long best = 0;
    for (uint32_t i = threadIdx.x; i < n_cells_padded; i += TPB) best = max(best, per_cell_sq[i]);
    for (int off = 32; off > 0; off >>= 1) best = max(best, (unsigned long long)__shfl_down(best, off));
    if ((threadIdx.x & 63) == 0) s_best[threadIdx.x >> 6] = best;
    __syncthreads();
    if (threadIdx.x == 0) {
        for (int w = 1; w < TPB / 64; ++w) best = max(best, s_best[w]);
        sc->pair_bound = max(sc->pair_bound, best);
        sc->caps_wrong = (assumed_counts && !caps.counts(sc)) ? 1u : 0u;
    }
}

__global__ __launch_bounds__(TPB) void k_fix_locus_rel(const uint32_t *blk_off, uint32_t nb, uint32_t L,
                                                      const uint32_t *locus_rel, uint32_t *entry32) {
    const uint32_t n_groups = nb * (L + 1);
    for (uint32_t g = blockIdx.x * TPB + threadIdx.x; g < n_groups; g += gridDim.x * TPB) {
        const uint32_t l = g % (L + 1);
        if (l == L) continue;
        const uint32_t b = blk_off[g], e = blk_off[g + 1];
        if (b == e) continue;
        const uint32_t lrel = (locus_rel[l] & 0xFFFFu) << 16;
        for (uint32_t d = b; d < e; ++d) entry32[d] = (entry32[d] & 0xFFFFu) | lrel;
    }
}

int bits_for(unsigned long long max_value) {
    int b = 1;
    while (b < 64 && (max_value >> b) != 0) ++b;
    return b;
}

#define HIP_OK(expr)                                                                      \
    do {                                                                                  \
        hipError_t e__ = (expr);                                                          \
        if (e__ != hipSuccess) return std::string(#expr) + ": " + hipGetErrorString(e__); \
    } while (0)

std::string pack_attempt(const DeviceFlatPileup &in, uint32_t num_cells, uint32_t mfl, uint32_t num_threads,
                         uint32_t block_cells, StageGeometry (*geometry)(uint32_t), bool allow_count_tile,
                         bool force_radix, bool no_assumptions, bool overlap, hipStream_t stream, DevicePacked *out,
                         bool *need_host, int *retry) {
    *retry = kNoRetry;
    const uint32_t E = static_cast<uint32_t>(in.n_entries);
    const uint32_t L = in.n_loci, C = in.n_chr;
    DevicePacked &pk = *out;
    const size_t n_off_max = (size_t)((num_cells + 63) / 64) * ((size_t)L + 1);
    enum { KEY_A, KEY_B, VAL_A, VAL_B, ELOC, WORK_A, WORK_B, RUNS, CUB, TMP, MISC, BIN, ENTRY_KC,
           M_IDX, M_ENTRY, RID_M, IDB_M, ELOC_M, DENSE_M, MARK_M, ARANK_M, DUPF, SEGS };
    auto &S = pk.scratch;
    const size_t id_space_cap = std::min<size_t>((size_t)kIdSpaceFactor * E + 1024, (size_t)1 << 30);

    Raw raw{in.chr_locus_off, C, in.locus_pos, in.locus_entry_off, in.read_ids, in.id_base16,
            in.id_base32, in.group_id_to_pos, in.n_groups, L, E};

    HIP_OK(S[MISC].ensure(sizeof(Scalars) + sizeof(uint32_t) * ((size_t)7 * C + 4 + (size_t)4 * L) + 64));
    Scalars *sc = S[MISC].as<Scalars>();
    uint32_t *id_max = reinterpret_cast<uint32_t *>(sc + 1);
    uint32_t *id_negmin = id_max + C;
    uint32_t *id_base = id_negmin + C;
    uint32_t *rbeg = id_base + C + 1;
    uint32_t *flushed = rbeg + C + 1;
    uint32_t *cnt = flushed + C;
    uint32_t *locus_chr = cnt + L, *locus_rel = locus_chr + L;
    uint32_t *flush_loci = locus_rel + L, *flush_count = flush_loci + L;
    uint32_t *tail_begin = flush_count + C;
    HIP_OK(S[KEY_A].ensure(std::max<size_t>((size_t)E * 8, ((size_t)2 * E + 4 + n_off_max + 1) * 4)));
    HIP_OK(S[KEY_B].ensure((size_t)E * 8));
    HIP_OK(S[VAL_A].ensure(std::max<size_t>(E, 64) * 4));
    HIP_OK(S[VAL_B].ensure((size_t)E * 4));
    HIP_OK(S[ELOC].ensure((size_t)E * 4 + 16));
    HIP_OK(S[WORK_A].ensure(((size_t)E + 1) * 4));
    HIP_OK(S[WORK_B].ensure(((size_t)2 * E + 2) * 4));
    HIP_OK(S[RUNS].ensure(((size_t)3 * E + 8) * 4));
    HIP_OK(S[ENTRY_KC].ensure((size_t)E * 8));
    uint32_t *sloc = S[ENTRY_KC].as<uint32_t>();
    HIP_OK(S[TMP].ensure((size_t)E * 4 + 64));
    HIP_OK(S[BIN].ensure((size_t)E * 24 + ((size_t)num_cells + 130) * 8 + 64));
    unsigned long long *key_a = S[KEY_A].as<unsigned long long>(), *key_b = S[KEY_B].as<unsigned long long>();
    uint32_t *val_a = S[VAL_A].as<uint32_t>(), *val_b = S[VAL_B].as<uint32_t>();
    uint32_t *eloc = S[ELOC].as<uint32_t>();
    {
        size_t need = 0, most = 0;
        HIP_OK(hipcub::DeviceRadixSort::SortPairs(nullptr, need, key_a, key_b, val_a, val_b, (int)E, 0, 64, stream));
        most = std::max(most, need);
        {
            hipcub::CountingInputIterator<uint32_t> positions(0u);
            hipcub::TransformInputIterator<unsigned long long, HeadKeepOp, hipcub::CountingInputIterator<uint32_t>>
                    flags(positions, HeadKeepOp{key_b, val_a, val_a});
            HIP_OK(hipcub::DeviceScan::InclusiveSum(nullptr, need, flags, key_a, (int)E, stream));
            most = std::max(most, need);
        }
        HIP_OK(hipcub::DeviceScan::ExclusiveSum(nullptr, need, val_a, val_b, (int)E + 1, stream));
        most = std::max(most, need);
        HIP_OK(hipcub::DeviceScan::ExclusiveSum(nullptr, need, val_a, val_b,
                                                (int)std::max<size_t>(n_off_max, id_space_cap + 2), stream));
        most = std::max(most, need);
        HIP_OK(S[CUB].ensure(most + 1024));
    }
    void *cub_tmp = S[CUB].p;
    size_t cub_cap = 0;
    HIP_OK(hipMemsetAsync(sc, 0, sizeof(Scalars) + sizeof(uint32_t) * ((size_t)3 * C + 1), stream));

    if (!pk.side) {
        HIP_OK(hipStreamCreateWithFlags(&pk.side, hipStreamNonBlocking));
        HIP_OK(hipEventCreateWithFlags(&pk.ev_fork, hipEventDisableTiming));
        HIP_OK(hipEventCreateWithFlags(&pk.ev_join, hipEventDisableTiming));
        HIP_OK(hipEventCreateWithFlags(&pk.ev_offsets, hipEventDisableTiming));
        HIP_OK(hipEventCreateWithFlags(&pk.ev_flush, hipEventDisableTiming));
    }
    auto bin_tiles = [&](uint32_t nb_, uint32_t *TL_, uint32_t *grid_, size_t *lds_) {
        uint32_t TL = 64;
        while (TL > 1 && (size_t)nb_ * (TL + 1) * 4 > 32768) TL >>= 1;
        *TL_ = TL;
        *grid_ = std::min<uint32_t>((L + TL - 1) / TL, 8192);
        *lds_ = (size_t)nb_ * (TL + 1) * 4;
    };

    const HostTrace trace;
    trace.mark("begin");
    hipLaunchKernelGGL(k_entry_locus, dim3(blocks_for((uint64_t)L * 64)), dim3(TPB), 0, stream, raw, eloc, sc);
    hipLaunchKernelGGL(k_id_range, dim3(std::min<uint32_t>(256, (E + 4095) / 4096)), dim3(TPB), 0, stream, raw,
                       eloc, id_max, id_negmin, (reinterpret_cast<uintptr_t>(raw.read_ids) & 15u) == 0 ? 1 : 0);
    const bool assume = !force_radix && !no_assumptions && pk.id_space_hint && pk.id_space_hint <= id_space_cap;
    hipLaunchKernelGGL(k_id_bases, dim3(1), dim3(64), 0, stream, C, id_max, id_negmin, id_base,
                       (unsigned long long)(assume ? pk.id_space_hint : 0), sc);
    Scalars hsc;
    std::memset(&hsc, 0, sizeof(hsc));
    if (!assume) {
        HIP_OK(read_scalars(pk, stream, sc, nullptr, &hsc, nullptr));
        if (hsc.error == 3) return "positions must be strictly increasing within a chromosome";
    }
    const size_t id_space = assume ? (size_t)pk.id_space_hint
                                   : (size_t)std::min<unsigned long long>(hsc.id_space, 1ull << 40);
    const bool counting = !force_radix && id_space <= id_space_cap;
    HIP_OK(S[WORK_A].ensure(std::max<size_t>((size_t)E + 1, counting ? id_space + 1 : 0) * 4));
    HIP_OK(S[WORK_B].ensure(std::max<size_t>((size_t)2 * E + 2, counting ? id_space + 1 : 0) * 4));
    uint32_t *work_a = S[WORK_A].as<uint32_t>(), *work_b = S[WORK_B].as<uint32_t>();
    static const bool split_allowed = [] {
        const char *e = std::getenv("SECEDO_PACK_SPLIT");
        return !(e && std::atoi(e) == 0);
    }();
    if (!pk.split_pays && ++pk.calls_without_split >= 16) {
        pk.split_pays = true;
        pk.calls_without_split = 0;
    }
    bool split_singles = counting && split_allowed && pk.split_pays;
    Raw sub = raw;
    const uint32_t *sub_eloc = eloc;
    uint32_t n_m = E;
    uint32_t *m_idx = nullptr, *m_entry = nullptr;
    if (counting) {
        uint32_t *hist = work_a, *id_off = work_b, *grouped = val_a;
        uint32_t *dense = S[KEY_A].as<uint32_t>();
        if (!split_singles) HIP_OK(hipMemsetAsync(hist, 0, (id_space + 1) * 4, stream));
        if (split_singles) {
            const size_t padded = ((size_t)E + kFlagBlock - 1) / kFlagBlock * kFlagBlock + 16;
            const uint32_t n_flag_blocks = (uint32_t)((padded - 16) / kFlagBlock);
            HIP_OK(S[M_IDX].ensure(((size_t)E + 2) * 4));
            m_idx = S[M_IDX].as<uint32_t>();
            HIP_OK(S[MARK_M].ensure(std::max(((size_t)E + 2) * 4, padded)));
            uint8_t *multi = S[MARK_M].as<uint8_t>();
            HIP_OK(hipMemsetAsync(multi, 0, padded, stream));
            hipLaunchKernelGGL(k_id_store, dim3(blocks_for((E + 3) / 4)), dim3(TPB), 0, stream, raw, eloc, id_base, id_negmin,
                               sc, dense, hist, (reinterpret_cast<uintptr_t>(raw.read_ids) & 15u) == 0 ? 1 : 0);
            hipLaunchKernelGGL(k_id_check, dim3(blocks_for((E + 3) / 4)), dim3(TPB), 0, stream, E, sc, dense, hist, multi);
            for (int a : {M_ENTRY, RID_M, IDB_M, ELOC_M, ARANK_M}) HIP_OK(S[a].ensure((size_t)E * 4 + 16));
            HIP_OK(S[DENSE_M].ensure(((size_t)6 * (E / 2 + 1) + 8) * 4));
            m_entry = S[M_ENTRY].as<uint32_t>();
            uint32_t *block_sum = grouped, *block_off = grouped + n_flag_blocks + 1;
            hipLaunchKernelGGL(k_flag_count, dim3(n_flag_blocks), dim3(TPB), 0, stream, multi, block_sum);
            hipLaunchKernelGGL(k_flag_scan, dim3(1), dim3(TPB_SCAN), 0, stream, block_sum, n_flag_blocks, block_off, m_idx + E,
                               sc);
            hipLaunchKernelGGL(k_compact_m, dim3(n_flag_blocks), dim3(TPB), 0, stream, raw, multi, block_off, m_idx, m_entry);
            HIP_OK(read_scalars(pk, stream, sc, nullptr, &hsc, nullptr));
            if (hsc.error == 3) return "positions must be strictly increasing within a chromosome";
            if (hsc.id_exceeded) {
                pk.id_space_hint = 0;
                *retry = kRetrySameScheme;
                return std::string();
            }
            n_m = hsc.n_multi_id;
            if ((uint64_t)n_m * 2 > E) {
                split_singles = false;
                pk.split_pays = false;
                pk.calls_without_split = 0;
                n_m = E;
                m_idx = nullptr;
                m_entry = nullptr;
                HIP_OK(hipMemsetAsync(hist, 0, (id_space + 1) * 4, stream));
            }
        }
        if (split_singles) {
            sub = raw;
            sub.read_ids = S[RID_M].as<uint32_t>();
            sub.id_base16 = nullptr;
            sub.id_base32 = S[IDB_M].as<uint32_t>();
            sub.n_entries = n_m;
            sub_eloc = S[ELOC_M].as<uint32_t>();
            if (n_m) {
                uint32_t *count_m = S[DENSE_M].as<uint32_t>(), *goff = count_m + n_m + 1, *winner_m = goff + n_m + 1;
                uint32_t *g_begin = winner_m + n_m, *g_len = g_begin + n_m, *members = g_len + n_m;
                HIP_OK(hipMemsetAsync(count_m, 0, ((size_t)n_m + 1) * 4, stream));
                hipLaunchKernelGGL(k_m_fields, dim3(blocks_for(n_m)), dim3(TPB), 0, stream, raw, eloc, dense, hist, m_idx, m_entry,
                                   n_m, S[RID_M].as<uint32_t>(), S[IDB_M].as<uint32_t>(), S[ELOC_M].as<uint32_t>(), winner_m,
                                   count_m);
                cub_cap = S[CUB].bytes;
                HIP_OK(hipcub::DeviceScan::ExclusiveSum(cub_tmp, cub_cap, count_m, goff, (int)n_m + 1, stream));
                hipLaunchKernelGGL(k_group_scatter, dim3(blocks_for(n_m)), dim3(TPB), 0, stream, winner_m, n_m, goff, count_m,
                                   members, g_begin, g_len);
                hipLaunchKernelGGL(k_group_rank, dim3(blocks_for(n_m)), dim3(TPB), 0, stream, sub, members, g_begin, g_len,
                                   sub_eloc, n_m, key_b, val_b, sloc, sc);
            }
        } else {
            hipLaunchKernelGGL(k_id_hist, dim3(blocks_for(E)), dim3(TPB), 0, stream, raw, eloc, id_base, id_negmin, sc,
                               dense, hist);
            cub_cap = S[CUB].bytes;
            HIP_OK(hipcub::DeviceScan::ExclusiveSum(cub_tmp, cub_cap, hist, id_off, (int)(id_space + 1), stream));
            hipLaunchKernelGGL(k_id_scatter, dim3(blocks_for(E)), dim3(TPB), 0, stream, dense, E, id_off, sc, hist,
                               grouped);
            hipLaunchKernelGGL(k_id_rank, dim3(blocks_for(E)), dim3(TPB), 0, stream, raw, dense, id_off, grouped, eloc,
                               key_b, val_b, sloc, sc);
        }
    } else {
        const uint32_t id_bits = (uint32_t)bits_for(hsc.max_read_id);
        hipLaunchKernelGGL(k_entry_keys, dim3(blocks_for(E)), dim3(TPB), 0, stream, raw, eloc, id_bits, key_a, val_a);
        cub_cap = S[CUB].bytes;
        HIP_OK(hipcub::DeviceRadixSort::SortPairs(cub_tmp, cub_cap, key_a, key_b, val_a, val_b, (int)E, 0,
                                                   (int)id_bits + bits_for(C), stream));
        hipLaunchKernelGGL(k_sorted_locus, dim3(blocks_for(E)), dim3(TPB), 0, stream, raw, val_b, eloc, E, sloc);
    }
    const unsigned long long *skey = key_b;
    const uint32_t *sval = val_b;

    uint32_t *keep = work_a;
    unsigned long long *incl = reinterpret_cast<unsigned long long *>(work_b);
    uint32_t *mark = S[KEY_A].as<uint32_t>();
    uint32_t *arank = mark + (E + 1);
    uint32_t *run_start = S[RUNS].as<uint32_t>();
    uint32_t *run_rank = run_start + E + 1;
    uint32_t *split = nullptr;
    HIP_OK(pk.read_off.ensure(((size_t)E + 1) * 4));
    HIP_OK(pk.read_locus.ensure((size_t)E * 4));
    HIP_OK(pk.read_base.ensure(E));
    HIP_OK(pk.range_off.ensure(((size_t)L + 2) * 4));
    HIP_OK(pk.entry.ensure((size_t)E * 16));
    HIP_OK(pk.entry32.ensure((size_t)E * 4));
    HIP_OK(pk.mask32.ensure((size_t)E * 4));
    HIP_OK(pk.entry_read.ensure((size_t)E * 4));
    HIP_OK(pk.blk_off.ensure((n_off_max + 1) * 4));
    uint32_t *read_off = pk.read_off.as<uint32_t>(), *read_locus = pk.read_locus.as<uint32_t>();
    uint8_t *read_base = pk.read_base.as<uint8_t>();
    const Ranks ranks{split_singles ? m_idx : nullptr, split_singles ? arank : nullptr, arank};
    auto build_reads = [&]() -> std::string {
        uint32_t *mark_sub = split_singles ? S[MARK_M].as<uint32_t>() : mark;
        if (n_m) {
            hipLaunchKernelGGL(k_dup_mark, dim3(blocks_for(n_m)), dim3(TPB), 0, stream, sub, skey, sval, sloc, split, n_m,
                               keep, mark_sub);
            hipcub::CountingInputIterator<uint32_t> positions(0u);
            hipcub::TransformInputIterator<unsigned long long, HeadKeepOp, hipcub::CountingInputIterator<uint32_t>>
                    flags(positions, HeadKeepOp{skey, keep, split});
            cub_cap = S[CUB].bytes;
            HIP_OK(hipcub::DeviceScan::InclusiveSum(cub_tmp, cub_cap, flags, incl, (int)n_m, stream));
        }
        cub_cap = S[CUB].bytes;
        const uint32_t *arank_sub = arank;
        if (split_singles) {
            hipcub::CountingInputIterator<uint32_t> entries(0u);
            hipcub::TransformInputIterator<uint32_t, UnmarkedM, hipcub::CountingInputIterator<uint32_t>> unmarked(
                    entries, UnmarkedM{mark_sub, n_m});
            HIP_OK(hipcub::DeviceScan::ExclusiveSum(cub_tmp, cub_cap, unmarked, arank, (int)n_m + 1, stream));
            uint32_t *arank_m = S[ARANK_M].as<uint32_t>();
            hipLaunchKernelGGL(k_arank_m, dim3(blocks_for(std::max(n_m, 1u))), dim3(TPB), 0, stream, arank, m_entry, n_m,
                               E, arank_m, sc);
            arank_sub = arank_m;
            hipLaunchKernelGGL(k_rbeg, dim3(1), dim3(TPB), 0, stream, raw, ranks, rbeg);
        } else {
            HIP_OK(hipcub::DeviceScan::ExclusiveSum(cub_tmp, cub_cap, mark, arank, (int)E + 1, stream));
        }
        if (n_m) {
            hipLaunchKernelGGL(k_runs_csr, dim3(blocks_for(n_m)), dim3(TPB), 0, stream, sub, incl, sval, sloc, n_m,
                               run_start, read_locus, read_base);
            hipLaunchKernelGGL(k_read_info, dim3(std::min<uint32_t>(blocks_for(n_m), 2048)), dim3(TPB), 0, stream, sub,
                               incl, run_start, sval, sloc, arank_sub, mfl, run_rank, split_singles ? nullptr : rbeg,
                               read_off, sc);
        }
        HIP_OK(hipEventRecord(pk.ev_fork, stream));
        HIP_OK(hipStreamWaitEvent(pk.side, pk.ev_fork, 0));
        hipLaunchKernelGGL(k_completed, dim3(blocks_for(L)), dim3(TPB), 0, pk.side, raw, ranks, rbeg, mfl, cnt, sc);
        hipLaunchKernelGGL(k_flush_chain, dim3(C), dim3(TPB), 0, pk.side, raw, cnt, 4u * num_threads, sc, flushed,
                           flush_loci, flush_count, ranks, rbeg, split_singles ? tail_begin : nullptr);
        HIP_OK(hipEventRecord(pk.ev_flush, pk.side));
        HIP_OK(hipEventRecord(pk.ev_join, pk.side));
        return std::string();
    };
    {
        const std::string err = build_reads();
        if (!err.empty()) return err;
    }
    struct SideJoin {
        hipStream_t side;
        bool joined = false;
        ~SideJoin() { if (!joined) (void)hipStreamSynchronize(side); }
    } side_join{pk.side};

    unsigned long long totals = 0;
    trace.mark("reads built (launched)");
    HIP_OK(read_scalars(pk, stream, sc, n_m ? incl + (n_m - 1) : nullptr, &hsc, &totals));
    trace.mark("read-back 2 arrived");
    if (hsc.error == 3) return "positions must be strictly increasing within a chromosome";
    if (hsc.id_exceeded) {
        pk.id_space_hint = 0;
        *retry = kRetrySameScheme;
        return std::string();
    }
    pk.id_space_hint = counting ? std::max<uint64_t>(hsc.id_space, 1) : 0;
    if (hsc.regroup) {
        *retry = kRetryRadix;
        return std::string();
    }
    if (hsc.need_host) {
        *need_host = true;
        return std::string();
    }
    if (hsc.long_reads) {
        bool stable = false;
        split = S[TMP].as<uint32_t>();
        HIP_OK(hipMemsetAsync(split, 0, (size_t)std::max(n_m, 1u) * 4, stream));
        for (int round = 0; round < kMaxSplitRounds && !stable; ++round) {
            HIP_OK(hipStreamWaitEvent(stream, pk.ev_join, 0));
            HIP_OK(hipMemsetAsync(&sc->split_changed, 0, 4, stream));
            hipLaunchKernelGGL(k_split_update, dim3(blocks_for(n_m)), dim3(TPB), 0, stream, sub, skey, sloc, mfl,
                               flush_loci, flush_count, split, sc);
            HIP_OK(read_scalars(pk, stream, sc, nullptr, &hsc, nullptr));
            if (!hsc.split_changed) {
                stable = true;
                break;
            }
            HIP_OK(hipMemsetAsync(&sc->multi_entries, 0, 8, stream));
            const std::string err = build_reads();
            if (!err.empty()) return err;
            HIP_OK(read_scalars(pk, stream, sc, n_m ? incl + (n_m - 1) : nullptr, &hsc, &totals));
        }
        if (!stable) {
            *need_host = true;
            return std::string();
        }
    }
    const uint32_t kept_m = (uint32_t)(totals >> 32);
    const uint32_t R = split_singles ? hsc.reads_total : (uint32_t)totals;
    const uint32_t n_kept = split_singles ? kept_m + (E - n_m) : kept_m;
    const size_t nk = std::max<uint32_t>(n_kept, 1);
    pk.multi_entries = hsc.multi_entries;
    pk.max_read_entries = std::max(hsc.max_read_entries, n_kept ? 1u : 0u);
    if (block_cells == 0) {
        const StageGeometry g64 = geometry(64);
        const bool clustered = n_kept && (double)pk.multi_entries > g64.masks_threshold * (double)n_kept;
        block_cells = (clustered || num_cells <= 64) ? 64 : 128;
    }
    const StageGeometry geo = geometry(block_cells);
    const uint32_t B = block_cells, nb = (num_cells + B - 1) / B;
    if (B != 64 && B != 128) return "block_cells must be 64 or 128";
    const uint32_t B_log2 = B == 64 ? 6u : 7u;
    const uint32_t lbits = (uint32_t)bits_for(L - 1);
    if (!force_radix && (lbits + kCibBits > 32u || E >= kSingle)) {
        *retry = kRetryRadix;
        return std::string();
    }
    pk.num_cells = num_cells;
    pk.block_cells = B;
    pk.num_blocks = nb;
    pk.num_loci = L;
    pk.num_entries = n_kept;
    pk.num_reads = R;
    pk.stage_masks = n_kept && (double)pk.multi_entries > geo.masks_threshold * (double)n_kept;

    uint32_t *t_read = S[TMP].as<uint32_t>();
    unsigned long long *key2_a = S[BIN].as<unsigned long long>();
    unsigned long long *key2_b = key2_a + nk;
    uint4 *m_rec = S[BIN].as<uint4>();
    unsigned long long *per_cell_sq = key2_b + nk;
    uint32_t *val2_a = reinterpret_cast<uint32_t *>(per_cell_sq + (size_t)nb * B + 1);
    uint32_t *val2_b = val2_a + nk;
    const size_t n_off = (size_t)nb * ((size_t)L + 1);
    uint32_t *blk_off = pk.blk_off.as<uint32_t>();
    uint32_t *blk_cnt = S[KEY_A].as<uint32_t>() + 2 * ((size_t)E + 1);
    unsigned long long *entry_kc = force_radix ? nullptr : S[ENTRY_KC].as<unsigned long long>();
    HIP_OK(S[DUPF].ensure((size_t)L + 16));
    uint8_t *dupflag = S[DUPF].as<uint8_t>();
    CapChoice caps;
    caps.entries_plain = pk.stage_masks ? geo.cap_entries_masks : geo.cap_entries_plain;
    caps.loci_plain = pk.stage_masks ? geo.cap_loci_masks : geo.cap_loci_plain;
    caps.entries_counts = geo.cap_entries_counts;
    caps.loci_counts = geo.cap_loci_counts;
    caps.count_limit = kCountTileLimit;
    caps.allow_counts = (allow_count_tile && !pk.stage_masks) ? 1u : 0u;
    if (caps.allow_counts && n_kept && L) {
        const double density = (double)n_kept / ((double)num_cells / B) / (double)L;
        const double per_segment = density * caps.loci_counts / caps.entries_counts;
        if (per_segment > 1.0) {
            const double greedy = std::ceil((double)L / caps.loci_counts) * std::ceil(per_segment);
            const uint32_t one = std::max(64u, (uint32_t)(0.93 * caps.entries_counts / density));
            if (one < caps.loci_counts && std::ceil((double)L / one) * 1.05 < greedy) caps.loci_counts = one;
        }
    }
    const uint32_t lo_loci = caps.allow_counts ? std::min(caps.loci_plain, caps.loci_counts) : caps.loci_plain;
    const uint32_t hi_loci = caps.allow_counts ? std::max(caps.loci_plain, caps.loci_counts) : caps.loci_plain;
    const uint32_t n_seg = (L + lo_loci - 1) / lo_loci;
    const size_t variant_stride = (size_t)n_seg * hi_loci + n_seg + 2;
    HIP_OK(S[SEGS].ensure(2 * variant_stride * 4));
    uint32_t *seg_count = S[SEGS].as<uint32_t>();
    uint32_t *seg_ends = seg_count + n_seg;
    auto cut_ranges_on_side = [&]() -> std::string {
        HIP_OK(hipEventRecord(pk.ev_offsets, stream));
        HIP_OK(hipStreamWaitEvent(pk.side, pk.ev_offsets, 0));
        hipLaunchKernelGGL(k_ranges_segment, dim3(n_seg, caps.allow_counts ? 2u : 1u), dim3(TPB), 0, pk.side, blk_off, nb,
                           L, caps, seg_ends, seg_count, variant_stride);
        HIP_OK(hipEventRecord(pk.ev_join, pk.side));
        return std::string();
    };
    if (force_radix) HIP_OK(hipMemsetAsync(blk_cnt, 0, (n_off + 1) * 4, stream));
    HIP_OK(hipMemsetAsync(per_cell_sq, 0, ((size_t)nb * B + 1) * 8, stream));
    uint32_t *krank = work_a;
    uint8_t *kflags = S[VAL_A].as<uint8_t>();
    uint32_t TL = 0, locus_grid = 0;
    size_t lds = 0;
    if (!force_radix) bin_tiles(nb, &TL, &locus_grid, &lds);
    const bool hist_first = split_singles && !force_radix;
    if (hist_first) {
        static const bool g2p_allowed = [] { const char *e = std::getenv("SECEDO_PACK_G2P_LDS"); return !(e && std::atoi(e) == 0); }();
        const size_t g2p_bytes = ((size_t)in.n_groups * 2 + 15) / 16 * 16;
        const bool g2p_lds = g2p_allowed && num_cells <= 0xFFFFu && lds + g2p_bytes <= 49152;
        hipLaunchKernelGGL(k_bin_hist, dim3(g2p_lds ? std::min<uint32_t>(locus_grid, 1024) : locus_grid), dim3(TPB),
                           lds + (g2p_lds ? g2p_bytes : 0), stream, raw, nb, TL, entry_kc, m_idx, num_cells, B_log2, blk_cnt,
                           sc, g2p_lds ? 1u : 0u);
    }
    if (n_m)
        hipLaunchKernelGGL(k_keys2, dim3(blocks_for(n_m)), dim3(TPB), 0, stream, sub, sval, incl, read_locus, run_rank,
                           read_off, num_cells, B, lbits, force_radix ? key2_a : nullptr, force_radix ? val2_a : nullptr,
                           t_read, krank, kflags, entry_kc, split_singles ? m_entry : nullptr,
                           hist_first ? blk_cnt : nullptr, L, sc);
    trace.mark("k_keys2 launched");
    const uint32_t slice_grid = std::min<uint32_t>(2048, (n_kept + 4095) / 4096);
    if (force_radix) {
        if (n_kept) {
            cub_cap = S[CUB].bytes;
            HIP_OK(hipcub::DeviceRadixSort::SortPairs(cub_tmp, cub_cap, key2_a, key2_b, val2_a, val2_b, (int)n_kept,
                                                       0, (int)(kCibBits + lbits) + bits_for(nb - 1), stream));
            hipLaunchKernelGGL(k_group_counts, dim3(slice_grid), dim3(TPB), 0, stream, key2_b, n_kept, B, L, lbits,
                               blk_cnt, per_cell_sq);
        }
        cub_cap = S[CUB].bytes;
        HIP_OK(hipcub::DeviceScan::ExclusiveSum(cub_tmp, cub_cap, blk_cnt, blk_off, (int)n_off, stream));
        const std::string err = cut_ranges_on_side();
        if (!err.empty()) return err;
    } else {
        if (!hist_first)
            hipLaunchKernelGGL(k_bin_hist, dim3(locus_grid), dim3(TPB), lds, stream, raw, nb, TL, entry_kc, nullptr, num_cells,
                               B_log2, blk_cnt, sc, 0u);
        trace.mark("k_bin_hist launched");
        const bool records_first = kept_m && (uint64_t)kept_m * 4u > (uint64_t)n_kept;
        if (records_first) {
            HIP_OK(hipEventRecord(pk.ev_offsets, stream));
            HIP_OK(hipStreamWaitEvent(pk.side, pk.ev_offsets, 0));
            hipLaunchKernelGGL(k_m_records, dim3(blocks_for(kept_m)), dim3(TPB), 0, pk.side, raw, kept_m, t_read, read_off,
                               read_locus, read_base, krank, kflags, rbeg, flushed, m_rec, sc);
            HIP_OK(hipEventRecord(pk.ev_join, pk.side));
        }
        cub_cap = S[CUB].bytes;
        HIP_OK(hipcub::DeviceScan::ExclusiveSum(cub_tmp, cub_cap, blk_cnt, blk_off, (int)n_off, stream));
        trace.mark("offset scan launched");
        if (records_first) {
            hipLaunchKernelGGL(k_ranges_segment, dim3(n_seg, caps.allow_counts ? 2u : 1u), dim3(TPB), 0, stream, blk_off, nb,
                               L, caps, seg_ends, seg_count, variant_stride);
        } else {
            const std::string err = cut_ranges_on_side();
            if (!err.empty()) return err;
            if (kept_m) {
                hipLaunchKernelGGL(k_m_records, dim3(blocks_for(kept_m)), dim3(TPB), 0, pk.side, raw, kept_m, t_read,
                                   read_off, read_locus, read_base, krank, kflags, rbeg, flushed, m_rec, sc);
                HIP_OK(hipEventRecord(pk.ev_join, pk.side));
            }
        }
        if (n_kept) {
            unsigned long long *grouped = key_b;
            HIP_OK(hipStreamWaitEvent(stream, pk.ev_flush, 0));
            uint32_t bm_words = (nb * B + 31) / 32;
            if (lds + (size_t)(TPB / 64) * bm_words * 4 > 49152) bm_words = 0;
            hipLaunchKernelGGL(k_bin_place, dim3(locus_grid), dim3(TPB), lds + (size_t)(TPB / 64) * bm_words * 4, stream,
                               raw, nb, TL, entry_kc, blk_off, B_log2, bm_words, split_singles ? tail_begin : nullptr,
                               grouped, dupflag);
        }
    }
    HIP_OK(hipStreamWaitEvent(stream, pk.ev_join, 0));
    side_join.joined = true;
    bool lists_launched = false;
    if (force_radix) {
        hipLaunchKernelGGL(k_ranges_compact, dim3(1), dim3(TPB), 0, stream, seg_ends, seg_count, variant_stride, n_seg,
                           caps, pk.range_off.as<uint32_t>(), per_cell_sq, n_kept ? nb * B : 0u, -1, sc);
        if (n_kept) {
            hipLaunchKernelGGL(k_locus_info, dim3(blocks_for(L)), dim3(TPB), 0, stream, raw, pk.range_off.as<uint32_t>(),
                               sc, nullptr, locus_chr, locus_rel);
            hipLaunchKernelGGL(k_records, dim3(blocks_for(n_kept)), dim3(TPB), 0, stream, raw, key2_b, val2_b, n_kept,
                               t_read, read_off, read_locus, read_base, krank, kflags, rbeg, flushed, locus_chr,
                               locus_rel, B, lbits, pk.entry.as<uint4>(), pk.entry32.as<uint32_t>(),
                               pk.stage_masks ? pk.mask32.as<uint32_t>() : nullptr, pk.entry_read.as<uint32_t>(), sc);
        }
    } else {
        const int assumed = caps.allow_counts ? 1 : 0;
        hipLaunchKernelGGL(k_ranges_compact, dim3(1), dim3(TPB), 0, stream, seg_ends, seg_count, variant_stride, n_seg,
                           caps, pk.range_off.as<uint32_t>(), per_cell_sq, 0u, assumed, sc);
        if (n_kept) {
            hipLaunchKernelGGL(k_locus_info, dim3(blocks_for(L)), dim3(TPB), 0, stream, raw, pk.range_off.as<uint32_t>(),
                               sc, dupflag, locus_chr, locus_rel);
            const RecordTables tables{m_rec, locus_rel, pk.entry.as<uint4>(), pk.entry32.as<uint32_t>(),
                                      pk.stage_masks ? pk.mask32.as<uint32_t>() : nullptr,
                                      pk.entry_read.as<uint32_t>()};
            const unsigned long long *grouped = key_b;
            const bool lists_here = overlap && caps.allow_counts && !pk.stage_masks && pk.flag_lists.scratch;
            const FlagScratch fs(pk.flag_lists.scratch, n_kept);
            hipLaunchKernelGGL(k_entry_records, dim3((n_kept + kFlagBlock - 1) / kFlagBlock), dim3(TPB_REC), 0, stream,
                               grouped, blk_off, n_kept, nb, L, B, lbits, tables, per_cell_sq, sc,
                               lists_here ? fs.chunk_mask : nullptr, lists_here ? fs.block_sum : nullptr);
            lists_launched = lists_here;
        }
        hipLaunchKernelGGL(k_pair_bound, dim3(1), dim3(TPB), 0, stream, per_cell_sq, n_kept ? nb * B : 0u, caps,
                           (uint32_t)assumed, sc);
    }
    trace.mark("records launched");
    HIP_OK(read_scalars(pk, stream, sc, nullptr, &hsc, nullptr, [&] {
        if (lists_launched)
            flag_lists_from_masks(FlagScratch(pk.flag_lists.scratch, n_kept), pk.entry.as<uint4>(), blk_off, n_off,
                                  pk.flag_lists.grp, pk.flag_lists.rec, pk.flag_lists.idx, stream);
    }));
    trace.mark("read-back 3 arrived");
    if (!force_radix && hsc.caps_wrong && !hsc.regroup && hsc.error == 0) {
        hipLaunchKernelGGL(k_ranges_compact, dim3(1), dim3(TPB), 0, stream, seg_ends, seg_count, variant_stride, n_seg,
                           caps, pk.range_off.as<uint32_t>(), per_cell_sq, 0u, 0, sc);
        if (n_kept) {
            hipLaunchKernelGGL(k_locus_info, dim3(blocks_for(L)), dim3(TPB), 0, stream, raw, pk.range_off.as<uint32_t>(),
                               sc, nullptr, locus_chr, locus_rel);
            hipLaunchKernelGGL(k_fix_locus_rel, dim3(blocks_for(n_off)), dim3(TPB), 0, stream, blk_off, nb, L, locus_rel,
                               pk.entry32.as<uint32_t>());
        }
        HIP_OK(read_scalars(pk, stream, sc, nullptr, &hsc, nullptr));
    }
    if (hsc.error == 1) return "group id outside group_id_to_pos";
    if (hsc.error == 2) return "group_id_to_pos maps outside the matrix";
    if (hsc.regroup) {
        *retry = kRetryRadix;
        return std::string();
    }
    pk.pair_bound = hsc.pair_bound;
    pk.cell_sq = per_cell_sq;
    pk.cell_sq_n = n_kept ? nb * B : 0u;
    pk.cell_sq_host.clear();
    pk.count_tile = caps.allow_counts && pk.pair_bound < kCountTileLimit;
    pk.cap_entries = pk.count_tile ? caps.entries_counts : caps.entries_plain;
    pk.cap_loci = pk.count_tile ? caps.loci_counts : caps.loci_plain;
    pk.num_ranges = hsc.num_ranges;
    pk.max_range_span = hsc.max_range_span;
    pk.n_wide = hsc.n_wide;
    pk.flag_lists_built = lists_launched;
    HIP_OK(hipGetLastError());
    return std::string();
}

}

std::string pack_pileup_device(const DeviceFlatPileup &in, uint32_t num_cells, uint32_t mfl,
                               uint32_t num_threads, uint32_t block_cells,
                               StageGeometry (*geometry)(uint32_t), bool allow_count_tile,
                               hipStream_t stream, DevicePacked *out, bool *need_host) {
    *need_host = false;
    out->flag_lists_built = false;
    if ((in.id_base16 != nullptr) == (in.id_base32 != nullptr))
        return "exactly one of id_base16 / id_base32 must be given";
    if (num_threads == 0) return "num_threads must be positive";
    if (num_cells == 0 || num_cells > 65535) return "num_cells must be in [1, 65535]";
    if (block_cells != 0 && block_cells != 64 && block_cells != 128) return "block_cells must be 0, 64 or 128";
    const uint64_t E64 = in.n_entries;
    const uint32_t L = in.n_loci;
    const size_t n_off_max = (size_t)((num_cells + 63) / 64) * ((size_t)L + 1);
    if (E64 >= (1ull << 31) || L == 0 || L >= (1u << 30) || E64 == 0 || (uint64_t)4 * num_threads > 0xFFFFFFFFull
        || n_off_max >= (1ull << 31)) {
        *need_host = true;
        return std::string();
    }
    bool force_radix = false;
    if (const char *env = std::getenv("SECEDO_PACK_GROUPING")) force_radix = std::string(env) == "radix";
    bool overlap = true;
    if (const char *env = std::getenv("SECEDO_PACK_OVERLAP")) overlap = std::atoi(env) != 0;
    int retry = kNoRetry;
    bool no_assumptions = false;
    std::string err;
    for (int attempt = 0; attempt < 3; ++attempt) {
        if (poison_level() >= 2) {
            if (hipStreamSynchronize(stream) != hipSuccess || (out->side && hipStreamSynchronize(out->side) != hipSuccess))
                return "poison: synchronise failed";
            DeviceArena *outputs[] = {&out->blk_off, &out->entry32, &out->mask32, &out->entry,
                                      &out->entry_read, &out->range_off, &out->read_off, &out->read_locus, &out->read_base};
            for (DeviceArena *a : outputs)
                if (a->p && hipMemset(a->p, 0xA5, a->bytes) != hipSuccess) return "poison: memset failed";
            for (DeviceArena &a : out->scratch)
                if (a.p && hipMemset(a.p, 0xA5, a.bytes) != hipSuccess) return "poison: memset failed";
        }
        err = pack_attempt(in, num_cells, mfl, num_threads, block_cells, geometry, allow_count_tile, force_radix,
                           no_assumptions, overlap, stream, out, need_host, &retry);
        if (!err.empty() || retry == kNoRetry) break;
        if (retry == kRetryRadix) force_radix = true;
        if (retry == kRetrySameScheme) no_assumptions = true;
    }
    if (err.empty() && retry != kNoRetry) *need_host = true;
    return err;
}


size_t flag_list_scratch_bytes(uint32_t n_entries) { return FlagScratch::bytes(n_entries); }

hipError_t pack_flag_lists(const uint32_t *entry32, const uint4 *entry, uint32_t n_entries, const uint32_t *blk_off,
                           size_t n_off, void *scratch, uint32_t *grp, uint4 *rec, uint32_t *idx, hipStream_t stream) {
    const FlagScratch fs(scratch, n_entries);
    hipLaunchKernelGGL(k_pflag_count, dim3(fs.nb), dim3(TPB), 0, stream, entry32, n_entries, fs.block_sum);
    hipLaunchKernelGGL(k_flag_scan, dim3(1), dim3(TPB_SCAN), 0, stream, fs.block_sum, fs.nb, fs.block_off,
                       fs.chunk_pre + 64 * (size_t)fs.nb, static_cast<Scalars *>(nullptr));
    hipLaunchKernelGGL(k_pflag_compact, dim3(fs.nb), dim3(TPB), 0, stream, entry32, entry, n_entries, fs.block_off, rec, idx,
                       fs.chunk_pre, fs.chunk_mask);
    flag_groups(fs, blk_off, n_off, grp, stream);
    return hipGetLastError();
}

}
```

secedo_amd/csrc/pack_device.hpp:

```cpp
#pragma once

#include "pack_host.hpp"

#include <hip/hip_runtime_api.h>
#include <hip/hip_vector_types.h>

#include <cstdint>
#include <string>
#include <vector>

namespace secedo {

struct DeviceFlatPileup {
    const uint32_t *chr_locus_off = nullptr;
    uint32_t n_chr = 0;
    const uint32_t *locus_pos = nullptr;
    const uint64_t *locus_entry_off = nullptr;
    const uint32_t *read_ids = nullptr;
    const uint16_t *id_base16 = nullptr;
    const uint32_t *id_base32 = nullptr;
    const uint32_t *group_id_to_pos = nullptr;
    uint32_t n_groups = 0;
    uint32_t n_loci = 0;
    uint64_t n_entries = 0;
};

int poison_level();

struct DeviceArena {
    void *p = nullptr;
    size_t bytes = 0;
    ~DeviceArena();
    hipError_t ensure(size_t n);
    template <class T>
    __attribute__((visibility("hidden"))) hipError_t upload(const std::vector<T> &v) {
        hipError_t e = ensure(v.size() * sizeof(T));
        if (e != hipSuccess || v.empty()) return e;
        return hipMemcpy(p, v.data(), v.size() * sizeof(T), hipMemcpyHostToDevice);
    }
    template <class T>
    T *as() const { return static_cast<T *>(p); }
};

struct DevicePacked {
    DeviceArena blk_off, entry32, mask32, entry, entry_read, range_off, read_off, read_locus, read_base;
    DeviceArena scratch[24];
    uint32_t num_cells = 0, block_cells = 0, num_blocks = 0, num_loci = 0, num_ranges = 0;
    uint64_t num_entries = 0, num_reads = 0, pair_bound = 0, multi_entries = 0;
    uint32_t max_read_entries = 0;
    uint32_t n_wide = 0;
    const unsigned long long *cell_sq = nullptr;
    uint32_t cell_sq_n = 0;
    std::vector<uint64_t> cell_sq_host;
    bool stage_masks = false;
    bool count_tile = false;
    uint32_t cap_entries = 0, cap_loci = 0;
    uint32_t max_range_span = 0xFFFFFFFFu;
    uint64_t id_space_hint = 0;
    bool split_pays = true;
    uint32_t calls_without_split = 0;
    hipStream_t side = nullptr;
    hipEvent_t ev_fork = nullptr, ev_join = nullptr, ev_offsets = nullptr, ev_flush = nullptr;
    struct FlagListBuffers {
        void *scratch = nullptr;
        uint32_t *grp = nullptr;
        uint4 *rec = nullptr;
        uint32_t *idx = nullptr;
    } flag_lists;
    bool flag_lists_built = false;
    void *mailbox = nullptr;
    unsigned long long mailbox_seq = 0;
    bool mailbox_failed = false;
    DevicePacked() = default;
    DevicePacked(const DevicePacked &) = delete;
    DevicePacked &operator=(const DevicePacked &) = delete;
    ~DevicePacked();
};

std::string pack_pileup_device(const DeviceFlatPileup &in, uint32_t num_cells,
                               uint32_t max_fragment_length, uint32_t num_threads,
                               uint32_t block_cells, StageGeometry (*geometry)(uint32_t),
                               bool allow_count_tile, hipStream_t stream, DevicePacked *out,
                               bool *need_host);

size_t flag_list_scratch_bytes(uint32_t n_entries);
hipError_t pack_flag_lists(const uint32_t *entry32, const uint4 *entry, uint32_t n_entries, const uint32_t *blk_off,
                           size_t n_off, void *scratch, uint32_t *grp, uint4 *rec, uint32_t *idx, hipStream_t stream);

}
```

secedo_amd/csrc/simmat_api.cpp:

```cpp
#include "simmat_handle.hpp"

#include <algorithm>
#include <cstdio>
#include <new>
#include <utility>

using namespace secedo::host;

namespace {

void note_pileup(secedo_simmat *h, uint32_t n_chr, uint64_t n_loci, uint64_t n_entries, const void *read_ids) {
    Fnv1a id;
    for (uint64_t v : {(uint64_t)n_chr, n_loci, n_entries, (uint64_t)reinterpret_cast<uintptr_t>(read_ids)}) id.add(v);
    h->pileup_identity = id.id();
    if (h->override_identity != h->pileup_identity) {
        if (h->pair_bound_override || h->max_shared_override) h->override_dropped = true;
        h->pair_bound_override = 0;
        h->max_shared_override = 0;
        h->override_identity = 0;
    }
}

int check_pileup_args(const secedo_simmat *h, const void *chr_locus_off, const void *locus_entry_off,
                      const void *id_base16, const void *id_base32, const void *group_id_to_pos, uint32_t n_groups) {
// ... 191 lines not shown
                     st[8], st[7] / w, st[2] / w, st[3] / w, st[4] / w, st[5] / w, st[6] / w,
                     (double)st[5] / std::max<double>(1, (double)st[9]), (double)st[6] / std::max<double>(1, (double)st[10]),
                     (double)st[10] / std::max<double>(1, (double)st[9]));
        unsigned long long pw[64] = {0};
        SECEDO_TRY(hipMemcpy(pw, counters + 16, sizeof(pw), hipMemcpyDeviceToHost));
        const double wgs = w / 16.0;
        for (int k = 0; k < 16; ++k)
            std::fprintf(stderr, "[stamps-counts] wave %2d: barrier-A %8.0f  pairs %8.0f  items %8.0f  stage+B %8.0f\n", k,
                         pw[k * 4] / wgs, pw[k * 4 + 1] / wgs, pw[k * 4 + 2] / wgs, pw[k * 4 + 3] / wgs);
    } else if (st[8]) {
        std::fprintf(stderr, "[stamps] waves %llu batches %llu trips %llu | per wave: lifetime %.0f cyc, setup %.0f, "
                             "fill %.0f, trips %.0f | per batch: setup %.0f fill %.0f trips %.0f (%.2f trips)\n",
                     st[8], st[5], st[6], (double)st[7] / st[8], (double)st[2] / st[8], (double)st[3] / st[8],
                     (double)st[4] / st[8], (double)st[2] / st[5], (double)st[3] / st[5], (double)st[4] / st[5],
                     (double)st[6] / st[5]);
        std::fprintf(stderr, "[stamps] per wave: barrier-1 wait %.0f, staging+barrier-2 %.0f, prefetch issue %.0f\n",
                     (double)st[9] / st[8], (double)st[10] / st[8], (double)st[11] / st[8]);
        std::fprintf(stderr, "[stamps] per wave: post-trip %.0f, batch loop total %.0f\n",
                     (double)st[12] / st[8], (double)st[13] / st[8]);
        std::fprintf(stderr, "[stamps] longest wave lifetime %llu cyc; ranges %u workgroups %u\n", st[14],
                     h->pk.num_ranges, h->plan_workgroups);
        std::vector<unsigned long long> wg(std::min<uint32_t>(h->plan_workgroups, 2048u));
        SECEDO_TRY(hipMemcpy(wg.data(), counters + 16, wg.size() * 8, hipMemcpyDeviceToHost));
        std::vector<unsigned long long> det(wg.size() * 8);
        SECEDO_TRY(hipMemcpy(det.data(), counters + 16 + 2048, det.size() * 8, hipMemcpyDeviceToHost));
        for (size_t k = 0; k < wg.size(); ++k)
            std::fprintf(stderr, "[stamps-wg] %zu %llu %llu %llu | hwid %llx ranges %llu listflush %llu endbarrier %llu slab %llu | realbegin %llu realend %llu batchloop %llu\n", k,
                         wg[k] & 0xFFFFFFFFull, (wg[k] >> 32) & 0xFFF, (wg[k] >> 44) & 0xFFF, det[k * 8], det[k * 8 + 1] / 1000,
                         det[k * 8 + 2] / 1000, det[k * 8 + 3] / 1000, det[k * 8 + 4] / 1000, det[k * 8 + 5], det[k * 8 + 6], det[k * 8 + 7] / 1000);
    }
    return SECEDO_OK;
}

}

int secedo::host::set_pileup_view(secedo_simmat *h, const secedo::FlatPileupView &v) {
    SECEDO_CALL(check_pileup_args(h, v.chr_locus_off, v.locus_entry_off, v.id_base16, v.id_base32, v.group_id_to_pos,
                                  v.n_groups));
    h->view = v;
    h->have_host = true;
    h->have_device = false;
    h->prepared = false;
    note_pileup(h, v.n_chr, v.n_loci(), v.n_entries(), v.read_ids);
    return SECEDO_OK;
}

int secedo::host::finalize_mode(secedo_simmat *h, int mode, const int64_t *d_acc, uint32_t row_begin, uint32_t row_end,
                                double *d_out, void *stream, bool keep_max) {
    SECEDO_CALL(check_ready(h, true, d_acc && d_out));
    SECEDO_CALL(check_row_range(h, row_begin, row_end));
    SECEDO_TRY(hipSetDevice(h->device));
    SECEDO_TRY(secedo::launch_finalize(d_acc, h->tile_row.as<uint16_t>(), h->tile_col.as<uint16_t>(), h->num_tiles,
                                       h->pk.num_cells, h->pk.block_cells, h->scale_log2, mode,
                                       h->max_bits.as<unsigned long long>(), row_begin, row_end, d_out,
                                       static_cast<hipStream_t>(stream), keep_max));
    return SECEDO_OK;
}

extern "C" {

const char *secedo_simmat_last_error(void) { return g_error.c_str(); }

const char *secedo_simmat_version(void) { return "secedo-simmat-mi355x 0.1 (gfx950)"; }

int secedo_simmat_device_count(void) {
    int n = 0;
    if (hipGetDeviceCount(&n) != hipSuccess) return 0;
    return n;
}

int secedo_simmat_normalization_from_string(const char *name) {
    if (name) {
        if (!std::strcmp(name, "ADD_MIN")) return SECEDO_NORM_ADD_MIN;
        if (!std::strcmp(name, "EXPONENTIATE")) return SECEDO_NORM_EXPONENTIATE;
        if (!std::strcmp(name, "SCALE_MAX_1")) return SECEDO_NORM_SCALE_MAX_1;
    }
    return fail(SECEDO_E_INVALID_NORMALIZATION,
                std::string("Invalid normalization: ") + (name ? name : "(null)"));
}

double secedo_simmat_llr(uint32_t x_s, uint32_t x_d, double eps, double h, double theta) {
    if (x_s + x_d >= 1 && !secedo::llr_exact_mode()) return secedo::reference_llr_any(eps, h, theta, x_s, x_d, 8);
    return secedo::llr(secedo::make_llr_model(eps, h, theta), x_s, x_d);
}

double secedo_simmat_llr_closed_form(uint32_t x_s, uint32_t x_d, double eps, double h, double theta) {
    return secedo::llr(secedo::make_llr_model(eps, h, theta), x_s, x_d);
}

int secedo_simmat_create(secedo_simmat_t **handle, int device_id) {
    if (!handle) return fail(SECEDO_E_INVALID_ARG, "handle is null");
    *handle = nullptr;
    const int n = secedo_simmat_device_count();
    if (n <= 0) return no_device("the similarity-matrix path");
    if (device_id < 0 || device_id >= n) return fail(SECEDO_E_NO_DEVICE, "device id out of range");
    SECEDO_TRY(hipSetDevice(device_id));
    secedo_simmat *h = new (std::nothrow) secedo_simmat();
    if (!h) return fail(SECEDO_E_LIMIT, "out of host memory");
    h->device = device_id;
    hipError_t e = hipEventCreate(&h->ev_begin);
    if (e == hipSuccess) e = hipEventCreate(&h->ev_end);
    if (e == hipSuccess) e = hipEventCreate(&h->ev_mid);
    if (e != hipSuccess) {
        delete h;
        return fail(SECEDO_E_HIP, std::string("hipEventCreate: ") + hipGetErrorString(e));
    }
    *handle = h;
    return SECEDO_OK;
}

void secedo_simmat_destroy(secedo_simmat_t *h) {
    if (!h) return;
    (void)hipSetDevice(h->device);
    if (h->ev_begin) (void)hipEventDestroy(h->ev_begin);
    if (h->ev_end) (void)hipEventDestroy(h->ev_end);
    if (h->ev_mid) (void)hipEventDestroy(h->ev_mid);
    h->uploads.destroy();
    delete h;
}

int secedo_simmat_set_pileup(secedo_simmat_t *h, const uint32_t *chr_locus_off, uint32_t n_chr,
                             const uint32_t *locus_pos, const uint64_t *locus_entry_off,
                             const uint32_t *read_ids, const uint16_t *id_base16,
                             const uint32_t *id_base32, const uint32_t *group_id_to_pos,
                             uint32_t n_groups) {
    return set_pileup_view(h, secedo::FlatPileupView{chr_locus_off, n_chr, locus_pos, locus_entry_off, read_ids,
                                                     id_base16, id_base32, group_id_to_pos, n_groups});
}

int secedo_simmat_set_pileup_device(secedo_simmat_t *h, const uint32_t *d_chr_locus_off, uint32_t n_chr,
                                    const uint32_t *d_locus_pos, const uint64_t *d_locus_entry_off,
                                    const uint32_t *d_read_ids, const uint16_t *d_id_base16,
                                    const uint32_t *d_id_base32, const uint32_t *d_group_id_to_pos,
                                    uint32_t n_groups, uint32_t n_loci, uint64_t n_entries) {
    SECEDO_CALL(check_pileup_args(h, d_chr_locus_off, d_locus_entry_off, d_id_base16, d_id_base32, d_group_id_to_pos,
                                  n_groups));
    h->dview = make_device_view(d_chr_locus_off, n_chr, d_locus_pos, d_locus_entry_off, d_read_ids, d_id_base16,
                                d_id_base32, d_group_id_to_pos, n_groups, n_loci, n_entries);
    h->have_device = true;
    h->have_host = false;
    h->prepared = false;
    note_pileup(h, n_chr, n_loci, n_entries, d_read_ids);
    return SECEDO_OK;
}

int secedo_simmat_set_packing(secedo_simmat_t *h, int mode) {
    if (!h) return fail(SECEDO_E_INVALID_ARG, "handle is null");
    if (mode < 0 || mode > 2) return fail(SECEDO_E_INVALID_ARG, "packing mode must be 0 (auto), 1 (host) or 2 (device)");
    h->packing_mode = mode;
    return SECEDO_OK;
}

int secedo_simmat_used_device_packing(const secedo_simmat_t *h) { return h ? h->used_device_packing : 0; }

int secedo_simmat_prepare(secedo_simmat_t *h, uint32_t num_cells, uint32_t max_fragment_length,
                          uint32_t num_threads, uint32_t block_cells, void *stream) {
    if (!h) return fail(SECEDO_E_INVALID_ARG, "handle is null");
    if (!h->have_host && !h->have_device) return fail(SECEDO_E_STATE, "set_pileup was not called");
    if (block_cells == 0) {
        const int v = env_int("SECEDO_BLOCK_CELLS", 0);
        if (v == 64 || v == 128) block_cells = static_cast<uint32_t>(v);
    }
    PrepareArgs p{num_cells, max_fragment_length, num_threads, block_cells, env_enabled("SECEDO_COUNT_TILE"),
                  h->packing_mode};
    if (env_is("SECEDO_PACKING", "host")) p.mode = 1;
    if (env_is("SECEDO_PACKING", "device")) p.mode = 2;
    SECEDO_TRY(hipSetDevice(h->device));
    hipStream_t s = static_cast<hipStream_t>(stream);
    h->prepared = false;
    h->used_device_packing = 0;
    h->num_threads = num_threads;

    bool need_host = (p.mode == 1);
    if (!need_host) SECEDO_CALL(pack_on_device(h, p, s, &need_host));
    if (need_host) SECEDO_CALL(pack_on_host(h, p, s));
    h->have_host = h->have_device = false;

    SECEDO_CALL(build_tile_table(h));
    SECEDO_TRY(h->counters.ensure((16 + 2048 * 9) * sizeof(unsigned long long)));
    SECEDO_TRY(h->max_bits.ensure(sizeof(unsigned long long)));
    SECEDO_TRY(hipMemsetAsync(h->counters.p, 0, 16 * sizeof(unsigned long long), s));
    h->prepared = true;
    h->timed = false;
    h->flags_ready = false;
    h->wide_known = false;
    return build_flag_lists(h, s);
}

uint32_t secedo_simmat_num_tiles(const secedo_simmat_t *h) { return h ? h->num_tiles : 0; }
uint32_t secedo_simmat_block_cells(const secedo_simmat_t *h) { return h ? h->pk.block_cells : 0; }
uint64_t secedo_simmat_acc_elems(const secedo_simmat_t *h) {
    return h ? static_cast<uint64_t>(h->num_tiles) * h->pk.block_cells * h->pk.block_cells : 0;
}
uint64_t secedo_simmat_num_entries(const secedo_simmat_t *h) { return h ? h->pk.num_entries : 0; }
uint64_t secedo_simmat_num_reads(const secedo_simmat_t *h) { return h ? h->pk.num_reads : 0; }
uint64_t secedo_simmat_num_loci(const secedo_simmat_t *h) { return h ? h->pk.num_loci : 0; }

uint64_t secedo_simmat_pair_bound(const secedo_simmat_t *h) { return h ? h->pk.pair_bound : 0; }
int secedo_simmat_scale_log2(const secedo_simmat_t *h) { return h ? h->scale_log2 : 0; }
uint32_t secedo_simmat_max_read_entries(const secedo_simmat_t *h) { return h ? h->pk.max_read_entries : 0; }
int secedo_simmat_set_scale_bounds(secedo_simmat_t *h, uint64_t pair_bound, uint32_t max_read_entries) {
    if (!h) return fail(SECEDO_E_INVALID_ARG, "handle is null");
    h->pair_bound_override = pair_bound;
    h->max_shared_override = max_read_entries;
    h->override_identity = (pair_bound || max_read_entries) ? h->pileup_identity : 0;
    h->override_dropped = false;
    return SECEDO_OK;
}
int secedo_simmat_scale_bounds_state(const secedo_simmat_t *h) {
    if (!h) return 0;
    if ((h->pair_bound_override || h->max_shared_override) && h->override_identity == h->pileup_identity) return 1;
    return h->override_dropped ? 2 : 0;
}
int secedo_simmat_set_pair_bound(secedo_simmat_t *h, uint64_t pair_bound) {
    return secedo_simmat_set_scale_bounds(h, pair_bound, h ? h->max_shared_override : 0);
}
int secedo_simmat_cell_squares(secedo_simmat_t *h, uint64_t *d_out, void *stream) {
    SECEDO_CALL(check_ready(h, false, d_out));
    SECEDO_TRY(hipSetDevice(h->device));
    hipStream_t s = static_cast<hipStream_t>(stream);
    const size_t n = h->pk.num_cells;
    SECEDO_TRY(hipMemsetAsync(d_out, 0, n * 8, s));
    if (h->pk.cell_sq && h->pk.cell_sq_n) {
        SECEDO_TRY(hipMemcpyAsync(d_out, h->pk.cell_sq, std::min<size_t>(n, h->pk.cell_sq_n) * 8, hipMemcpyDeviceToDevice, s));
    } else if (!h->pk.cell_sq_host.empty()) {
        SECEDO_TRY(hipMemcpyAsync(d_out, h->pk.cell_sq_host.data(), std::min(n, h->pk.cell_sq_host.size()) * 8,
                                  hipMemcpyHostToDevice, s));
        SECEDO_TRY(hipStreamSynchronize(s));
    }
    return SECEDO_OK;
}

int secedo_simmat_zero_acc(secedo_simmat_t *h, int64_t *d_acc, void *stream) {
    SECEDO_CALL(check_ready(h, false, d_acc));
    SECEDO_TRY(hipSetDevice(h->device));
    SECEDO_TRY(hipMemsetAsync(d_acc, 0, secedo_simmat_acc_elems(h) * sizeof(int64_t),
                              static_cast<hipStream_t>(stream)));
    return SECEDO_OK;
}

int secedo_simmat_tiles_of_rows(const secedo_simmat_t *h, uint32_t row_begin, uint32_t row_end, uint32_t *tile_ids,
                                uint32_t *n_tile_ids) {
    SECEDO_CALL(check_ready(h, false, n_tile_ids));
    SECEDO_CALL(check_row_range(h, row_begin, row_end));
    uint32_t n = 0;
    if (row_begin < row_end) {
        const uint32_t B = h->pk.block_cells, b0 = row_begin / B, b1 = (row_end - 1) / B;
        for (uint32_t t = 0; t < h->num_tiles; ++t) {
            const uint32_t I = h->host_tile_row[t], J = h->host_tile_col[t];
            if ((I >= b0 && I <= b1) || (J >= b0 && J <= b1)) {
                if (tile_ids) tile_ids[n] = t;
                ++n;
            }
        }
    }
    *n_tile_ids = n;
    return SECEDO_OK;
}

int secedo_simmat_max_of_tiles(secedo_simmat_t *h, const int64_t *d_acc, const uint32_t *tile_ids, uint32_t n_tile_ids,
                               double *max_value, void *stream) {
    SECEDO_CALL(check_ready(h, true, d_acc && max_value && (tile_ids || !n_tile_ids)));
    for (uint32_t k = 0; k < n_tile_ids; ++k)
        if (tile_ids[k] >= h->num_tiles) return fail(SECEDO_E_INVALID_ARG, "tile id outside [0, num_tiles)");
    SECEDO_TRY(hipSetDevice(h->device));
    hipStream_t s = static_cast<hipStream_t>(stream);
    DevBuf ids;
    SECEDO_TRY(ids.ensure((size_t)std::max(n_tile_ids, 1u) * 4));
    if (n_tile_ids) SECEDO_TRY(hipMemcpyAsync(ids.p, tile_ids, (size_t)n_tile_ids * 4, hipMemcpyHostToDevice, s));
    SECEDO_TRY(secedo::launch_tile_max(d_acc, h->tile_row.as<uint16_t>(), h->tile_col.as<uint16_t>(), ids.as<uint32_t>(),
                                       n_tile_ids, h->pk.block_cells, h->scale_log2, h->max_bits.as<unsigned long long>(),
                                       s));
    unsigned long long bits = 0;
    SECEDO_TRY(hipMemcpyAsync(&bits, h->max_bits.p, 8, hipMemcpyDeviceToHost, s));
    SECEDO_TRY(hipStreamSynchronize(s));
    std::memcpy(max_value, &bits, 8);
    return SECEDO_OK;
}

int secedo_simmat_finalize_rows_max(secedo_simmat_t *h, int normalization, const int64_t *d_acc, uint32_t row_begin,
                                    uint32_t row_end, double max_value, double *d_out_rows, void *stream) {
    SECEDO_CALL(check_normalization(normalization));
    SECEDO_CALL(check_ready(h, true, d_acc && d_out_rows));
    SECEDO_CALL(check_row_range(h, row_begin, row_end));
    if (!(max_value >= 0.0)) return fail(SECEDO_E_INVALID_ARG, "max_value must be the (non-negative) maximum of D");
    SECEDO_TRY(hipSetDevice(h->device));
    hipStream_t s = static_cast<hipStream_t>(stream);
    unsigned long long bits;
    std::memcpy(&bits, &max_value, 8);
    SECEDO_TRY(hipMemcpyAsync(h->max_bits.p, &bits, 8, hipMemcpyHostToDevice, s));
    SECEDO_TRY(hipStreamSynchronize(s));
    SECEDO_TRY(secedo::launch_finalize(d_acc, h->tile_row.as<uint16_t>(), h->tile_col.as<uint16_t>(), h->num_tiles,
                                       h->pk.num_cells, h->pk.block_cells, h->scale_log2, normalization,
                                       h->max_bits.as<unsigned long long>(), row_begin, row_end, d_out_rows, s, true));
    return SECEDO_OK;
}

int secedo_simmat_finalize(secedo_simmat_t *h, int normalization, const int64_t *d_acc, double *d_out,
                           void *stream) {
    SECEDO_CALL(check_normalization(normalization));
    return finalize_mode(h, normalization, d_acc, 0, h ? h->pk.num_cells : 0, d_out, stream);
}

int secedo_simmat_finalize_rows(secedo_simmat_t *h, int normalization, const int64_t *d_acc, uint32_t row_begin,
                                uint32_t row_end, double *d_out_rows, void *stream) {
    SECEDO_CALL(check_normalization(normalization));
// ... 68 lines not shown
```

secedo_amd/similarity_matrix.py:

```python
from __future__ import annotations

import ctypes as C
from typing import Optional, Sequence, Union

import numpy as np

from . import _lib
from ._lib import InvalidNormalization, SecedoError
from .pileup import FlatPileup, PosData, flatten

NORMALIZATIONS = ("ADD_MIN", "EXPONENTIATE", "SCALE_MAX_1")


def to_enum(normalization: str) -> int:
    if not isinstance(normalization, str):
        raise InvalidNormalization("Invalid normalization: %r" % (normalization,))
    rc = _lib.lib().secedo_simmat_normalization_from_string(normalization.encode())
    if rc < 0:
        raise InvalidNormalization("Invalid normalization: " + normalization)
    return rc


def _as_flat(pos_data) -> FlatPileup:
    if isinstance(pos_data, FlatPileup):
        return pos_data
    return flatten(pos_data)


def _id_arrays(p: FlatPileup):
    if p.n_entries == 0 or int(p.id_base.max()) <= 0xFFFF:
        return np.ascontiguousarray(p.id_base.astype(np.uint16)), None
    return None, p.id_base


def compute_similarity_matrix(pos_data: Union[FlatPileup, Sequence[Sequence[PosData]]],
                              num_cells: int,
                              max_fragment_length: int,
                              group_id_to_pos: Optional[Sequence[int]],
                              mutation_rate: float,
                              homozygous_rate: float,
                              seq_error_rate: float,
                              num_threads: int,
                              marker: str = "",
                              normalization: str = "ADD_MIN") -> np.ndarray:
    del marker
    norm = to_enum(normalization)
    p = _as_flat(pos_data)
    g2p = np.arange(num_cells, dtype=np.uint32) if group_id_to_pos is None \
        else np.ascontiguousarray(group_id_to_pos, dtype=np.uint32)
    id16, id32 = _id_arrays(p)
    out = np.empty((num_cells, num_cells), dtype=np.float64)
    rc = _lib.lib().secedo_simmat_compute(
        _lib.ptr(p.chr_locus_off), p.n_chr, _lib.ptr(p.locus_pos), _lib.ptr(p.locus_entry_off),
        _lib.ptr(p.read_ids), _lib.ptr(id16), _lib.ptr(id32), _lib.ptr(g2p), len(g2p), num_cells,
        max_fragment_length, mutation_rate, homozygous_rate, seq_error_rate, num_threads, norm,
        _lib.ptr(out))
    _lib.check(rc)
    return out


def set_devices(device_ids: Optional[Sequence[int]] = None) -> None:
    ids = [int(d) for d in (device_ids or [])]
    arr = (C.c_int * max(len(ids), 1))(*ids)
    _lib.check(_lib.lib().secedo_simmat_set_devices(arr if ids else None, len(ids)))


def get_devices():
    arr = (C.c_int * 16)()
    n = _lib.lib().secedo_simmat_get_devices(arr, 16)
    if n < 0:
        _lib.check(n)
    return [int(arr[i]) for i in range(min(n, 16))]


def llr(x_s: int, x_d: int, mutation_rate: float, homozygous_rate: float,
        seq_error_rate: float) -> float:
    return float(_lib.lib().secedo_simmat_llr(x_s, x_d, mutation_rate, homozygous_rate, seq_error_rate))


def llr_closed_form(x_s: int, x_d: int, mutation_rate: float, homozygous_rate: float,
                    seq_error_rate: float) -> float:
    return float(_lib.lib().secedo_simmat_llr_closed_form(x_s, x_d, mutation_rate, homozygous_rate,
                                                          seq_error_rate))


class SimilarityMatrixPlan:

    def __init__(self, device: int = 0):
        import torch
        self._torch = torch
        self.device = device
        self._h = C.c_void_p()
        _lib.check(_lib.lib().secedo_simmat_create(C.byref(self._h), device))
        self.num_cells = 0
        self._keep = None

    def close(self):
        if self._h:
            _lib.lib().secedo_simmat_destroy(self._h)
            self._h = C.c_void_p()

    def __del__(self):
        try:
            self.close()
        except Exception:
            pass

    def __enter__(self):
        return self

    def __exit__(self, *exc):
        self.close()

    def set_packing(self, mode: str = "auto"):
        _lib.check(_lib.lib().secedo_simmat_set_packing(self._h, {"auto": 0, "host": 1, "device": 2}[mode]))
        return self

    @property
    def used_device_packing(self) -> bool:
        return bool(_lib.lib().secedo_simmat_used_device_packing(self._h))

    def upload(self, pos_data, group_id_to_pos=None, num_cells=None):
        p = _as_flat(pos_data)
        t = self._torch
        dev = "cuda:%d" % self.device
        if group_id_to_pos is None:
            n = num_cells if num_cells is not None else (int(p.id_base.max() >> 2) + 1 if p.n_entries else 1)
            group_id_to_pos = np.arange(n, dtype=np.uint32)
        g2p = np.ascontiguousarray(group_id_to_pos, dtype=np.uint32)
        id16, id32 = _id_arrays(p)

        def dev_tensor(a, view):
            a = np.ascontiguousarray(a)
            if a.size == 0:
                a = np.zeros(1, dtype=a.dtype)
            return t.from_numpy(a.view(view)).to(dev)

        res = dict(
            chr=dev_tensor(p.chr_locus_off, np.int32), pos=dev_tensor(p.locus_pos, np.int32),
            off=dev_tensor(p.locus_entry_off, np.int64), rid=dev_tensor(p.read_ids, np.int32),
            idb=dev_tensor(id16, np.int16) if id16 is not None else dev_tensor(id32, np.int32),
            idb_is16=id16 is not None, g2p=dev_tensor(g2p, np.int32), n_chr=p.n_chr, n_loci=p.n_loci,
            n_entries=p.n_entries, n_groups=len(g2p))
        return res

    def prepare_resident(self, res, num_cells, max_fragment_length, num_threads=8, block_cells=0):
        L = _lib.lib()
        idb = C.c_void_p(res["idb"].data_ptr())
        _lib.check(L.secedo_simmat_set_pileup_device(
            self._h, C.c_void_p(res["chr"].data_ptr()), res["n_chr"], C.c_void_p(res["pos"].data_ptr()),
            C.c_void_p(res["off"].data_ptr()), C.c_void_p(res["rid"].data_ptr()),
            idb if res["idb_is16"] else None, None if res["idb_is16"] else idb,
            C.c_void_p(res["g2p"].data_ptr()), res["n_groups"], res["n_loci"], res["n_entries"]))
        _lib.check(L.secedo_simmat_prepare(self._h, num_cells, max_fragment_length, num_threads, block_cells,
                                           self._stream()))
        self.num_cells = num_cells
        return self

    def prepare(self, pos_data, num_cells, max_fragment_length, group_id_to_pos=None,
                num_threads=8, block_cells=0):
        p = _as_flat(pos_data)
        g2p = np.arange(num_cells, dtype=np.uint32) if group_id_to_pos is None \
            else np.ascontiguousarray(group_id_to_pos, dtype=np.uint32)
        id16, id32 = _id_arrays(p)
        L = _lib.lib()
        _lib.check(L.secedo_simmat_set_pileup(
            self._h, _lib.ptr(p.chr_locus_off), p.n_chr, _lib.ptr(p.locus_pos),
            _lib.ptr(p.locus_entry_off), _lib.ptr(p.read_ids), _lib.ptr(id16), _lib.ptr(id32),
            _lib.ptr(g2p), len(g2p)))
        _lib.check(L.secedo_simmat_prepare(self._h, num_cells, max_fragment_length, num_threads,
                                           block_cells, self._stream()))
        self.num_cells = num_cells
        return self

    @property
    def num_tiles(self) -> int:
        return int(_lib.lib().secedo_simmat_num_tiles(self._h))

    @property
    def block_cells(self) -> int:
        return int(_lib.lib().secedo_simmat_block_cells(self._h))

    @property
    def acc_elems(self) -> int:
        return int(_lib.lib().secedo_simmat_acc_elems(self._h))

    @property
    def num_entries(self) -> int:
        return int(_lib.lib().secedo_simmat_num_entries(self._h))

    @property
    def num_reads(self) -> int:
        return int(_lib.lib().secedo_simmat_num_reads(self._h))

    @property
    def num_loci(self) -> int:
        return int(_lib.lib().secedo_simmat_num_loci(self._h))

    @property
    def pair_bound(self) -> int:
        return int(_lib.lib().secedo_simmat_pair_bound(self._h))

    def set_pair_bound(self, pair_bound: int):
        _lib.check(_lib.lib().secedo_simmat_set_pair_bound(self._h, int(pair_bound)))
        return self

    @property
    def max_read_entries(self) -> int:
        return int(_lib.lib().secedo_simmat_max_read_entries(self._h))

    def cell_squares(self):
        t = self._torch
        out = t.empty(max(self.num_cells, 1), dtype=t.int64, device="cuda:%d" % self.device)
        _lib.check(_lib.lib().secedo_simmat_cell_squares(self._h, C.c_void_p(out.data_ptr()), self._stream()))
        return out[:self.num_cells]

    def set_scale_bounds(self, pair_bound: int, max_read_entries: int):
        _lib.check(_lib.lib().secedo_simmat_set_scale_bounds(self._h, int(pair_bound), int(max_read_entries)))
        return self

    @property
    def scale_bounds_state(self) -> int:
        return int(_lib.lib().secedo_simmat_scale_bounds_state(self._h))

    @property
    def scale_log2(self) -> int:
        return int(_lib.lib().secedo_simmat_scale_log2(self._h))

    def _stream(self):
        return C.c_void_p(self._torch.cuda.current_stream(self.device).cuda_stream)

    def new_acc(self, pad_tiles_to: int = 1):
        b2 = self.block_cells ** 2
        tiles = -(-self.num_tiles // pad_tiles_to) * pad_tiles_to
        return self._torch.zeros(tiles * b2, dtype=self._torch.int64, device="cuda:%d" % self.device)

    def zero_acc(self, acc):
        _lib.check(_lib.lib().secedo_simmat_zero_acc(self._h, C.c_void_p(acc.data_ptr()), self._stream()))

    def accumulate(self, acc, mutation_rate, homozygous_rate, seq_error_rate, tile_begin=0,
                   tile_end=None, overwrite=False):
        tile_end = self.num_tiles if tile_end is None else tile_end
        assert acc.dtype == self._torch.int64 and acc.is_contiguous() and acc.numel() >= self.acc_elems
        fn = _lib.lib().secedo_simmat_assign if overwrite else _lib.lib().secedo_simmat_accumulate
        _lib.check(fn(self._h, mutation_rate, homozygous_rate, seq_error_rate, tile_begin, tile_end,
                      C.c_void_p(acc.data_ptr()), self._stream()))

    def assign_finalize(self, acc, mutation_rate, homozygous_rate, seq_error_rate, normalization="ADD_MIN", out=None):
        norm = to_enum(normalization)
        if out is None:
            out = self._torch.empty((self.num_cells, self.num_cells), dtype=self._torch.float64,
                                    device="cuda:%d" % self.device)
        assert acc.dtype == self._torch.int64 and acc.is_contiguous() and acc.numel() >= self.acc_elems
        assert out.dtype == self._torch.float64 and out.is_contiguous()
        _lib.check(_lib.lib().secedo_simmat_assign_finalize(
            self._h, mutation_rate, homozygous_rate, seq_error_rate, norm, C.c_void_p(acc.data_ptr()),
            C.c_void_p(out.data_ptr()), self._stream()))
        return out

    def finalize(self, acc, normalization="ADD_MIN", out=None):
        norm = to_enum(normalization)
        if out is None:
            out = self._torch.empty((self.num_cells, self.num_cells), dtype=self._torch.float64,
                                    device="cuda:%d" % self.device)
        assert out.dtype == self._torch.float64 and out.is_contiguous()
        _lib.check(_lib.lib().secedo_simmat_finalize(
            self._h, norm, C.c_void_p(acc.data_ptr()), C.c_void_p(out.data_ptr()), self._stream()))
        return out

    def finalize_rows(self, acc, row_begin, row_end, normalization="ADD_MIN", out=None):
        norm = to_enum(normalization)
        if out is None:
            out = self._torch.empty((row_end - row_begin, self.num_cells), dtype=self._torch.float64,
                                    device="cuda:%d" % self.device)
# ... 68 lines not shown
```

Baseline: 784.5 billion updates/s.

## Drop per-entry locus and dense-id arrays from device packing split path

The device packing pipeline stops materialising the per-entry locus array and per-entry dense id array on the split-singles path. Chromosome lookups now use per-chromosome first-entry offsets, so dense ids are recomputed on the fly, and the strictly-increasing check moves into the id range kernel. The full per-entry multi-index array is replaced by a chunk prefix plus 64-bit mask with popcount lookup. This cuts memory traffic and scratch footprint in the prepare phase, at the cost of extra binary searches and recomputation. A query for whether the single-entry path was used is also added.

```diff
diff --git a/include/secedo_simmat.h b/include/secedo_simmat.h
--- a/include/secedo_simmat.h
+++ b/include/secedo_simmat.h
@@ -60,6 +60,7 @@
 
 int secedo_simmat_set_packing(secedo_simmat_t *handle, int mode);
 int secedo_simmat_used_device_packing(const secedo_simmat_t *handle);
+int secedo_simmat_used_single_entry_path(const secedo_simmat_t *handle);
 
 int secedo_simmat_prepare(secedo_simmat_t *handle, uint32_t num_cells, uint32_t max_fragment_length,
                           uint32_t num_threads, uint32_t block_cells, void *stream);
diff --git a/secedo_amd/_lib.py b/secedo_amd/_lib.py
--- a/secedo_amd/_lib.py
+++ b/secedo_amd/_lib.py
@@ -65,6 +65,7 @@
                                                   C.c_uint32, C.c_uint32, C.c_uint64]),
     "secedo_simmat_set_packing": (C.c_int, [_vp, C.c_int]),
     "secedo_simmat_used_device_packing": (C.c_int, [_vp]),
+    "secedo_simmat_used_single_entry_path": (C.c_int, [_vp]),
     "secedo_simmat_prepare": (C.c_int, [_vp, C.c_uint32, C.c_uint32, C.c_uint32, C.c_uint32, _vp]),
     "secedo_simmat_num_tiles": (C.c_uint32, [_vp]),
     "secedo_simmat_block_cells": (C.c_uint32, [_vp]),
diff --git a/secedo_amd/csrc/pack_device.hip b/secedo_amd/csrc/pack_device.hip
--- a/secedo_amd/csrc/pack_device.hip
+++ b/secedo_amd/csrc/pack_device.hip
@@ -196,15 +196,34 @@
     }
 }
 
-__global__ __launch_bounds__(TPB) void k_id_range(Raw in, const uint32_t *entry_locus, uint32_t *id_max,
-                                                 uint32_t *id_negmin, int vec) {
+__device__ __forceinline__ uint32_t chr_first_entry(const Raw &in, uint32_t c) {
+    return (uint32_t)in.locus_entry_off[in.chr_locus_off[c]];
+}
+
+__global__ __launch_bounds__(TPB) void k_id_range(Raw in, uint32_t *id_max, uint32_t *id_negmin, int vec, Scalars *sc) {
     __shared__ uint32_t s_hi[TPB / 64], s_neg[TPB / 64];
+    __shared__ uint32_t s_chr;
+    for (uint32_t l = blockIdx.x * TPB + threadIdx.x; l + 1 < in.n_loci; l += gridDim.x * TPB) {
+        if (in.locus_pos[l + 1] <= in.locus_pos[l]) {
+            const uint32_t c = last_le<uint32_t>(in.chr_locus_off, in.n_chr + 1, l);
+            if (l + 1 < in.chr_locus_off[c + 1]) sc->error = 3;
+        }
+    }
     const uint32_t E = in.n_entries;
     const uint32_t chunk = (E + gridDim.x - 1) / gridDim.x;
     uint32_t cur = min(E, blockIdx.x * chunk);
     const uint32_t e1 = min(E, cur + chunk);
     if (cur >= e1) return;
-    uint32_t c = last_le<uint32_t>(in.chr_locus_off, in.n_chr + 1, entry_locus[cur]);
+    if (threadIdx.x == 0) s_chr = 0;
+    __syncthreads();
+    {
+        uint32_t best = 0;
+        for (uint32_t i = threadIdx.x; i < in.n_chr; i += TPB)
+            if (chr_first_entry(in, i) <= cur) best = i;
+        if (best) atomicMax(&s_chr, best);
+    }
+    __syncthreads();
+    uint32_t c = s_chr;
     while (cur < e1) {
         uint32_t c_end = (uint32_t)in.locus_entry_off[in.chr_locus_off[c + 1]];
         while (c_end <= cur && c + 1 < in.n_chr) {
@@ -274,9 +293,12 @@
     }
 }
 
-__global__ void k_id_bases(uint32_t n_chr, const uint32_t *id_max, const uint32_t *id_negmin, uint32_t *id_base,
-                           unsigned long long assumed_space, Scalars *sc) {
-    if (threadIdx.x != 0 || blockIdx.x != 0) return;
+__global__ void k_id_bases(Raw in, const uint32_t *id_max, const uint32_t *id_negmin, uint32_t *id_base,
+                           uint32_t *chr_entry, unsigned long long assumed_space, Scalars *sc) {
+    const uint32_t n_chr = in.n_chr;
+    if (blockIdx.x != 0) return;
+    for (uint32_t c = threadIdx.x; c <= n_chr; c += blockDim.x) chr_entry[c] = chr_first_entry(in, c);
+    if (threadIdx.x != 0) return;
     unsigned long long sum = 0;
     uint32_t top = 0;
     for (uint32_t c = 0; c < n_chr; ++c) {
@@ -314,11 +336,11 @@
 struct ChrTables {
     uint32_t first[kChrLds + 1], base[kChrLds], min_id[kChrLds];
 };
-__device__ __forceinline__ bool chr_tables_load(const Raw &in, const uint32_t *id_base, const uint32_t *id_negmin,
-                                                ChrTables &t) {
+__device__ __forceinline__ bool chr_tables_load(const Raw &in, const uint32_t *first, const uint32_t *id_base,
+                                                const uint32_t *id_negmin, ChrTables &t) {
     const bool in_lds = in.n_chr <= kChrLds;
     if (in_lds) {
-        for (uint32_t i = threadIdx.x; i <= in.n_chr; i += blockDim.x) t.first[i] = in.chr_locus_off[i];
+        for (uint32_t i = threadIdx.x; i <= in.n_chr; i += blockDim.x) t.first[i] = first[i];
         for (uint32_t i = threadIdx.x; i < in.n_chr; i += blockDim.x) {
             t.base[i] = id_base[i];
             t.min_id[i] = ~id_negmin[i];
@@ -327,23 +349,39 @@
     __syncthreads();
     return in_lds;
 }
-__device__ __forceinline__ uint32_t dense_id(const Raw &in, const uint32_t *id_base, const uint32_t *id_negmin,
-                                             const ChrTables &t, bool in_lds, uint32_t locus, uint32_t id) {
-    if (in_lds) {
-        const uint32_t c = last_le<uint32_t>(t.first, in.n_chr + 1, locus);
-        return t.base[c] + (id - t.min_id[c]);
-    }
-    const uint32_t c = last_le<uint32_t>(in.chr_locus_off, in.n_chr + 1, locus);
-    return id_base[c] + (id - ~id_negmin[c]);
+__device__ __forceinline__ uint32_t chr_of(const Raw &in, const uint32_t *first, const ChrTables &t, bool in_lds,
+                                           uint32_t key) {
+    return last_le<uint32_t>(in_lds ? t.first : first, in.n_chr + 1, key);
+}
+__device__ __forceinline__ uint32_t dense_of(const uint32_t *id_base, const uint32_t *id_negmin, const ChrTables &t,
+                                             bool in_lds, uint32_t c, uint32_t id) {
+    return in_lds ? t.base[c] + (id - t.min_id[c]) : id_base[c] + (id - ~id_negmin[c]);
+}
+__device__ __forceinline__ uint32_t dense_id(const Raw &in, const uint32_t *first, const uint32_t *id_base,
+                                             const uint32_t *id_negmin, const ChrTables &t, bool in_lds, uint32_t key,
+                                             uint32_t id) {
+    return dense_of(id_base, id_negmin, t, in_lds, chr_of(in, first, t, in_lds, key), id);
+}
+__device__ __forceinline__ void dense_id_quad(const Raw &in, const uint32_t *chr_entry, const uint32_t *id_base,
+                                              const uint32_t *id_negmin, const ChrTables &t, bool in_lds, uint32_t e0,
+                                              const uint32_t (&id)[4], uint32_t (&d)[4]) {
+    const uint32_t c0 = chr_of(in, chr_entry, t, in_lds, e0);
+    const uint32_t next = in_lds ? t.first[c0 + 1] : chr_entry[c0 + 1];
+#pragma unroll
+    for (int u = 0; u < 4; ++u) {
+        const uint32_t e = min(e0 + (uint32_t)u, in.n_entries - 1u);
+        const uint32_t c = e < next ? c0 : chr_of(in, chr_entry, t, in_lds, e);
+        d[u] = dense_of(id_base, id_negmin, t, in_lds, c, id[u]);
+    }
 }
 
 __global__ void k_id_hist(Raw in, const uint32_t *entry_locus, const uint32_t *id_base, const uint32_t *id_negmin,
                           const Scalars *sc, uint32_t *dense, uint32_t *hist) {
     if (sc->id_exceeded) return;
     __shared__ ChrTables tables;
-    const bool in_lds = chr_tables_load(in, id_base, id_negmin, tables);
+    const bool in_lds = chr_tables_load(in, in.chr_locus_off, id_base, id_negmin, tables);
     for (uint32_t e = blockIdx.x * TPB + threadIdx.x; e < in.n_entries; e += gridDim.x * TPB) {
-        const uint32_t d = dense_id(in, id_base, id_negmin, tables, in_lds, entry_locus[e], in.read_ids[e]);
+        const uint32_t d = dense_id(in, in.chr_locus_off, id_base, id_negmin, tables, in_lds, entry_locus[e], in.read_ids[e]);
         dense[e] = d;
         atomicAdd(&hist[d], 1u);
     }
@@ -386,57 +424,45 @@
 }
 
 constexpr uint32_t kFlagBlock = 4096;
-__global__ void k_id_store(Raw in, const uint32_t *entry_locus, const uint32_t *id_base, const uint32_t *id_negmin,
-                           const Scalars *sc, uint32_t *dense, uint32_t *last, int vec) {
+__device__ __forceinline__ void load_id_quad(const Raw &in, uint32_t q, int vec, uint32_t (&id)[4]) {
+    const uint32_t n = in.n_entries, e0 = q * 4u;
+    if (vec && e0 + 4u <= n) {
+        const uint4 iv = reinterpret_cast<const uint4 *>(in.read_ids)[q];
+        id[0] = iv.x, id[1] = iv.y, id[2] = iv.z, id[3] = iv.w;
+    } else {
+#pragma unroll
+        for (int u = 0; u < 4; ++u) id[u] = in.read_ids[min(e0 + (uint32_t)u, n - 1u)];
+    }
+}
+__global__ void k_id_store(Raw in, const uint32_t *chr_entry, const uint32_t *id_base, const uint32_t *id_negmin,
+                           const Scalars *sc, uint32_t *last, int vec) {
     if (sc->id_exceeded) return;
     __shared__ ChrTables tables;
-    const bool in_lds = chr_tables_load(in, id_base, id_negmin, tables);
+    const bool in_lds = chr_tables_load(in, chr_entry, id_base, id_negmin, tables);
     const uint32_t n = in.n_entries, stride = gridDim.x * TPB;
     for (uint32_t q = blockIdx.x * TPB + threadIdx.x; q < (n + 3u) / 4u; q += stride) {
         const uint32_t e0 = q * 4u;
-        uint32_t l[4], id[4], d[4];
-        if (vec && e0 + 4u <= n) {
-            const uint4 lv = reinterpret_cast<const uint4 *>(entry_locus)[q];
-            const uint4 iv = reinterpret_cast<const uint4 *>(in.read_ids)[q];
-            l[0] = lv.x, l[1] = lv.y, l[2] = lv.z, l[3] = lv.w;
-            id[0] = iv.x, id[1] = iv.y, id[2] = iv.z, id[3] = iv.w;
-        } else {
+        uint32_t id[4], d[4];
+        load_id_quad(in, q, vec, id);
+        dense_id_quad(in, chr_entry, id_base, id_negmin, tables, in_lds, e0, id, d);
 #pragma unroll
-            for (int u = 0; u < 4; ++u) {
-                const uint32_t e = min(e0 + (uint32_t)u, n - 1u);
-                l[u] = entry_locus[e];
-                id[u] = in.read_ids[e];
-            }
-        }
-#pragma unroll
-        for (int u = 0; u < 4; ++u) d[u] = dense_id(in, id_base, id_negmin, tables, in_lds, l[u], id[u]);
-        if (e0 + 4u <= n) {
-            reinterpret_cast<uint4 *>(dense)[q] = make_uint4(d[0], d[1], d[2], d[3]);
-#pragma unroll
-            for (int u = 0; u < 4; ++u) last[d[u]] = e0 + (uint32_t)u + 1u;
-        } else {
-            for (uint32_t u = 0; e0 + u < n; ++u) {
-                dense[e0 + u] = d[u];
-                last[d[u]] = e0 + u + 1u;
-            }
-        }
-    }
-}
-__global__ void k_id_check(uint32_t n, const Scalars *sc, const uint32_t *dense, const uint32_t *last, uint8_t *multi) {
+        for (int u = 0; u < 4; ++u)
+            if (e0 + (uint32_t)u < n) last[d[u]] = e0 + (uint32_t)u + 1u;
+    }
+}
+__global__ void k_id_check(Raw in, const uint32_t *chr_entry, const uint32_t *id_base, const uint32_t *id_negmin,
+                           const Scalars *sc, const uint32_t *last, uint8_t *multi, int vec) {
     if (sc->id_exceeded) return;
-    const uint32_t stride = gridDim.x * TPB;
+    __shared__ ChrTables tables;
+    const bool in_lds = chr_tables_load(in, chr_entry, id_base, id_negmin, tables);
+    const uint32_t n = in.n_entries, stride = gridDim.x * TPB;
     for (uint32_t q = blockIdx.x * TPB + threadIdx.x; q < (n + 3u) / 4u; q += stride) {
         const uint32_t e0 = q * 4u;
-        uint32_t d[4], w[4];
-        if (e0 + 4u <= n) {
-            const uint4 dv = reinterpret_cast<const uint4 *>(dense)[q];
-            d[0] = dv.x, d[1] = dv.y, d[2] = dv.z, d[3] = dv.w;
-        } else {
+        uint32_t id[4], d[4], w[4];
+        load_id_quad(in, q, vec, id);
+        dense_id_quad(in, chr_entry, id_base, id_negmin, tables, in_lds, e0, id, d);
 #pragma unroll
-            for (int u = 0; u < 4; ++u) d[u] = dense[min(e0 + (uint32_t)u, n - 1u)];
-        }
-#pragma unroll
-        for (int u = 0; u < 4; ++u) w[u] = last[d[u]];
+        for (int u = 0; u < 4; ++u) w[u] = e0 + (uint32_t)u < n ? last[d[u]] : 0u;
 #pragma unroll
         for (int u = 0; u < 4; ++u) {
             const uint32_t e = e0 + (uint32_t)u;
@@ -463,7 +489,7 @@
 }
 constexpr int TPB_SCAN = 1024;
 __global__ __launch_bounds__(TPB_SCAN) void k_flag_scan(const uint32_t *block_sum, uint32_t n_blocks, uint32_t *block_off,
-                                                       uint32_t *m_idx_end, Scalars *sc) {
+                                                       uint32_t *total_out, Scalars *sc) {
     constexpr int TPB = TPB_SCAN;
     __shared__ uint32_t part[TPB / 64];
     __shared__ uint32_t carry;
@@ -488,20 +514,30 @@
         __syncthreads();
     }
     if (threadIdx.x == 0u) {
-        *m_idx_end = carry;
+        *total_out = carry;
         if (sc) sc->n_multi_id = carry;
     }
 }
+struct MIndex {
+    const uint32_t *chunk_pre;
+    const unsigned long long *chunk_mask;
+    __device__ __forceinline__ uint32_t operator()(uint32_t e) const {
+        const uint32_t c = e >> 6, r = e & 63u;
+        return chunk_pre[c] + (uint32_t)__popcll(chunk_mask[c] & ((1ull << r) - 1ull));
+    }
+};
 __global__ __launch_bounds__(TPB) void k_compact_m(Raw in, const uint8_t *multi, const uint32_t *block_off,
-                                                  uint32_t *m_idx, uint32_t *m_entry) {
+                                                  uint32_t *chunk_pre, unsigned long long *chunk_mask,
+                                                  uint32_t *m_entry) {
     __shared__ uint32_t part[TPB / 64];
     const uint32_t lane = threadIdx.x & 63u, wv = threadIdx.x >> 6;
     const uint32_t e0 = blockIdx.x * kFlagBlock + threadIdx.x * 16u;
     const uint4 w = reinterpret_cast<const uint4 *>(multi + (size_t)blockIdx.x * kFlagBlock)[threadIdx.x];
     const uint32_t words[4] = {w.x, w.y, w.z, w.w};
-    uint32_t mine = 0;
+    uint32_t bits = 0;
 #pragma unroll
-    for (int i = 0; i < 4; ++i) mine += (words[i] * 0x01010101u) >> 24;
+    for (int i = 0; i < 16; ++i) bits |= ((words[i >> 2] >> ((i & 3) * 8)) & 1u) << i;
+    const uint32_t mine = (uint32_t)__popc(bits);
     uint32_t incl = mine;
     for (int off = 1; off < 64; off <<= 1) {
         const uint32_t up = __shfl_up(incl, off);
@@ -511,29 +547,16 @@
     __syncthreads();
     uint32_t j = block_off[blockIdx.x] + incl - mine;
     for (uint32_t w2 = 0; w2 < wv; ++w2) j += part[w2];
-    const uint32_t n = in.n_entries;
-    __shared__ uint32_t tile[TPB * 17];
-    {
-        uint32_t jj = j;
-#pragma unroll
-        for (int i = 0; i < 16; ++i) {
-            tile[threadIdx.x * 17u + (uint32_t)i] = jj;
-            jj += (words[i >> 2] >> ((i & 3) * 8)) & 1u;
-        }
-    }
-    __syncthreads();
-#pragma unroll
-    for (int k = 0; k < 16; ++k) {
-        const uint32_t i = (uint32_t)k * TPB + threadIdx.x;
-        const uint32_t e = blockIdx.x * kFlagBlock + i;
-        if (e < n) m_idx[e] = tile[(i >> 4) * 17u + (i & 15u)];
-    }
-#pragma unroll
-    for (int i = 0; i < 16; ++i) {
-        const uint32_t e = e0 + (uint32_t)i;
-        if (e >= n) break;
-        if ((words[i >> 2] >> ((i & 3) * 8)) & 1u) m_entry[j++] = e;
-    }
+    unsigned long long m = (unsigned long long)bits << ((lane & 3u) * 16u);
+    m |= __shfl_xor(m, 1);
+    m |= __shfl_xor(m, 2);
+    if ((lane & 3u) == 0u) {
+        const uint32_t chunk = blockIdx.x * (kFlagBlock / 64u) + (threadIdx.x >> 2);
+        chunk_pre[chunk] = j;
+        chunk_mask[chunk] = m;
+    }
+    if (blockIdx.x == gridDim.x - 1u && threadIdx.x == 0u) chunk_mask[gridDim.x * (kFlagBlock / 64u)] = 0ull;
+    for (uint32_t b = bits; b; b &= b - 1u) m_entry[j++] = e0 + (uint32_t)__ffs((int)b) - 1u;
 }
 __global__ __launch_bounds__(TPB) void k_pflag_count(const uint32_t *entry32, uint32_t n, uint32_t *block_sum) {
     __shared__ uint32_t part[TPB / 64];
@@ -670,15 +693,19 @@
     flag_groups(fs, blk_off, n_off, grp, stream);
 }
 
-__global__ void k_m_fields(Raw in, const uint32_t *eloc, const uint32_t *dense, const uint32_t *last,
-                           const uint32_t *m_idx, const uint32_t *m_entry, uint32_t n_m, uint32_t *rid_m,
+__global__ void k_m_fields(Raw in, const uint32_t *chr_entry, const uint32_t *id_base, const uint32_t *id_negmin,
+                           const uint32_t *last, MIndex m_index, const uint32_t *m_entry, uint32_t n_m, uint32_t *rid_m,
                            uint32_t *idb_m, uint32_t *eloc_m, uint32_t *winner_m, uint32_t *count_m) {
+    __shared__ ChrTables tables;
+    const bool in_lds = chr_tables_load(in, chr_entry, id_base, id_negmin, tables);
     for (uint32_t j = blockIdx.x * TPB + threadIdx.x; j < n_m; j += gridDim.x * TPB) {
         const uint32_t e = m_entry[j];
-        rid_m[j] = in.read_ids[e];
+        const uint32_t id = in.read_ids[e];
+        rid_m[j] = id;
         idb_m[j] = in.id_base(e);
-        eloc_m[j] = eloc[e];
-        const uint32_t w = m_idx[last[dense[e]] - 1u];
+        eloc_m[j] = last_le<uint64_t>(in.locus_entry_off, in.n_loci + 1, (uint64_t)e);
+        const uint32_t d = dense_id(in, chr_entry, id_base, id_negmin, tables, in_lds, e, id);
+        const uint32_t w = m_index(last[d] - 1u);
         winner_m[j] = w;
         atomicAdd(&count_m[w], 1u);
     }
@@ -719,9 +746,10 @@
 constexpr uint32_t kSingleTail = 4u;
 
 struct Ranks {
-    const uint32_t *m_idx, *unm;
+    MIndex m_index;
+    const uint32_t *unm;
     const uint32_t *arank;
-    __device__ __forceinline__ uint32_t operator()(uint32_t e) const { return unm ? e - unm[m_idx[e]] : arank[e]; }
+    __device__ __forceinline__ uint32_t operator()(uint32_t e) const { return unm ? e - unm[m_index(e)] : arank[e]; }
 };
 struct UnmarkedM {
     const uint32_t *mark_m;
@@ -1019,7 +1047,7 @@
 }
 
 __global__ __launch_bounds__(TPB) void k_bin_hist(Raw in, uint32_t nb, uint32_t TL, unsigned long long *__restrict__ entry_kc,
-                                                 const uint32_t *__restrict__ m_idx, uint32_t num_cells,
+                                                 const unsigned long long *__restrict__ m_mask, uint32_t num_cells,
                                                  uint32_t B_log2, uint32_t *__restrict__ blk_cnt, Scalars *sc,
                                                  uint32_t g2p_lds) {
     extern __shared__ uint32_t lds_hist[];
@@ -1041,21 +1069,23 @@
         for (uint32_t base = eb + threadIdx.x; base < ee; base += TPB * U) {
             uint32_t slot[U];
             constexpr uint32_t kNone = 0xFFFFFFFFu;
-            if (m_idx) {
-                uint32_t m0[U], m1[U], ib[U], cell[U];
+            if (m_mask) {
+                unsigned long long mw[U];
+                uint32_t ib[U], cell[U];
+                bool is_m[U];
 #pragma unroll
                 for (int u = 0; u < U; ++u) {
                     const uint32_t e = base + (uint32_t)u * TPB;
                     const bool in_tile = e < ee;
-                    m0[u] = in_tile ? m_idx[e] : 0u;
-                    m1[u] = in_tile ? m_idx[e + 1] : 1u;
+                    mw[u] = in_tile ? m_mask[e >> 6] : ~0ull;
                     ib[u] = in_tile ? in.id_base(e) : 0u;
                 }
 #pragma unroll
                 for (int u = 0; u < U; ++u) {
                     const uint32_t group = ib[u] >> 2;
                     cell[u] = 0;
-                    if (m1[u] == m0[u]) {
+                    is_m[u] = (mw[u] >> ((base + (uint32_t)u * TPB) & 63u)) & 1ull;
+                    if (!is_m[u]) {
                         if (group >= in.n_groups) sc->error = 1;
                         else cell[u] = g2p_lds ? (uint32_t)s_g2p[group] : in.g2p[group];
                     }
@@ -1063,7 +1093,7 @@
 #pragma unroll
                 for (int u = 0; u < U; ++u) {
                     slot[u] = kNone;
-                    if (m1[u] != m0[u]) continue;
+                    if (is_m[u]) continue;
                     const uint32_t e = base + (uint32_t)u * TPB;
                     uint32_t c = cell[u];
                     if (c >= num_cells) {
@@ -1671,14 +1701,14 @@
     DevicePacked &pk = *out;
     const size_t n_off_max = (size_t)((num_cells + 63) / 64) * ((size_t)L + 1);
     enum { KEY_A, KEY_B, VAL_A, VAL_B, ELOC, WORK_A, WORK_B, RUNS, CUB, TMP, MISC, BIN, ENTRY_KC,
-           M_IDX, M_ENTRY, RID_M, IDB_M, ELOC_M, DENSE_M, MARK_M, ARANK_M, DUPF, SEGS };
+           M_CHUNKS, M_ENTRY, RID_M, IDB_M, ELOC_M, DENSE_M, MARK_M, ARANK_M, DUPF, SEGS };
     auto &S = pk.scratch;
     const size_t id_space_cap = std::min<size_t>((size_t)kIdSpaceFactor * E + 1024, (size_t)1 << 30);
 
     Raw raw{in.chr_locus_off, C, in.locus_pos, in.locus_entry_off, in.read_ids, in.id_base16,
             in.id_base32, in.group_id_to_pos, in.n_groups, L, E};
 
-    HIP_OK(S[MISC].ensure(sizeof(Scalars) + sizeof(uint32_t) * ((size_t)7 * C + 4 + (size_t)4 * L) + 64));
+    HIP_OK(S[MISC].ensure(sizeof(Scalars) + sizeof(uint32_t) * ((size_t)8 * C + 8 + (size_t)4 * L) + 64));
     Scalars *sc = S[MISC].as<Scalars>();
     uint32_t *id_max = reinterpret_cast<uint32_t *>(sc + 1);
     uint32_t *id_negmin = id_max + C;
@@ -1689,11 +1719,11 @@
     uint32_t *locus_chr = cnt + L, *locus_rel = locus_chr + L;
     uint32_t *flush_loci = locus_rel + L, *flush_count = flush_loci + L;
     uint32_t *tail_begin = flush_count + C;
+    uint32_t *chr_entry = tail_begin + C;
     HIP_OK(S[KEY_A].ensure(std::max<size_t>((size_t)E * 8, ((size_t)2 * E + 4 + n_off_max + 1) * 4)));
     HIP_OK(S[KEY_B].ensure((size_t)E * 8));
     HIP_OK(S[VAL_A].ensure(std::max<size_t>(E, 64) * 4));
     HIP_OK(S[VAL_B].ensure((size_t)E * 4));
-    HIP_OK(S[ELOC].ensure((size_t)E * 4 + 16));
     HIP_OK(S[WORK_A].ensure(((size_t)E + 1) * 4));
     HIP_OK(S[WORK_B].ensure(((size_t)2 * E + 2) * 4));
     HIP_OK(S[RUNS].ensure(((size_t)3 * E + 8) * 4));
@@ -1703,7 +1733,6 @@
     HIP_OK(S[BIN].ensure((size_t)E * 24 + ((size_t)num_cells + 130) * 8 + 64));
     unsigned long long *key_a = S[KEY_A].as<unsigned long long>(), *key_b = S[KEY_B].as<unsigned long long>();
     uint32_t *val_a = S[VAL_A].as<uint32_t>(), *val_b = S[VAL_B].as<uint32_t>();
-    uint32_t *eloc = S[ELOC].as<uint32_t>();
     {
         size_t need = 0, most = 0;
         HIP_OK(hipcub::DeviceRadixSort::SortPairs(nullptr, need, key_a, key_b, val_a, val_b, (int)E, 0, 64, stream));
@@ -1743,11 +1772,11 @@
 
     const HostTrace trace;
     trace.mark("begin");
-    hipLaunchKernelGGL(k_entry_locus, dim3(blocks_for((uint64_t)L * 64)), dim3(TPB), 0, stream, raw, eloc, sc);
-    hipLaunchKernelGGL(k_id_range, dim3(std::min<uint32_t>(256, (E + 4095) / 4096)), dim3(TPB), 0, stream, raw,
-                       eloc, id_max, id_negmin, (reinterpret_cast<uintptr_t>(raw.read_ids) & 15u) == 0 ? 1 : 0);
+    const int ids_aligned = (reinterpret_cast<uintptr_t>(raw.read_ids) & 15u) == 0 ? 1 : 0;
+    hipLaunchKernelGGL(k_id_range, dim3(std::min<uint32_t>(256, (E + 4095) / 4096)), dim3(TPB), 0, stream, raw, id_max,
+                       id_negmin, ids_aligned, sc);
     const bool assume = !force_radix && !no_assumptions && pk.id_space_hint && pk.id_space_hint <= id_space_cap;
-    hipLaunchKernelGGL(k_id_bases, dim3(1), dim3(64), 0, stream, C, id_max, id_negmin, id_base,
+    hipLaunchKernelGGL(k_id_bases, dim3(1), dim3(64), 0, stream, raw, id_max, id_negmin, id_base, chr_entry,
                        (unsigned long long)(assume ? pk.id_space_hint : 0), sc);
     Scalars hsc;
     std::memset(&hsc, 0, sizeof(hsc));
@@ -1770,10 +1799,22 @@
         pk.calls_without_split = 0;
     }
     bool split_singles = counting && split_allowed && pk.split_pays;
+    uint32_t *eloc = nullptr;
+    auto make_entry_locus = [&]() -> std::string {
+        HIP_OK(S[ELOC].ensure((size_t)E * 4 + 16));
+        eloc = S[ELOC].as<uint32_t>();
+        hipLaunchKernelGGL(k_entry_locus, dim3(blocks_for((uint64_t)L * 64)), dim3(TPB), 0, stream, raw, eloc, sc);
+        return std::string();
+    };
+    if (!split_singles) {
+        const std::string err = make_entry_locus();
+        if (!err.empty()) return err;
+    }
     Raw sub = raw;
-    const uint32_t *sub_eloc = eloc;
+    const uint32_t *sub_eloc = nullptr;
     uint32_t n_m = E;
-    uint32_t *m_idx = nullptr, *m_entry = nullptr;
+    MIndex m_index{nullptr, nullptr};
+    uint32_t *m_entry = nullptr;
     if (counting) {
         uint32_t *hist = work_a, *id_off = work_b, *grouped = val_a;
         uint32_t *dense = S[KEY_A].as<uint32_t>();
@@ -1781,22 +1822,27 @@
         if (split_singles) {
             const size_t padded = ((size_t)E + kFlagBlock - 1) / kFlagBlock * kFlagBlock + 16;
             const uint32_t n_flag_blocks = (uint32_t)((padded - 16) / kFlagBlock);
-            HIP_OK(S[M_IDX].ensure(((size_t)E + 2) * 4));
-            m_idx = S[M_IDX].as<uint32_t>();
+            const size_t n_chunks = (size_t)n_flag_blocks * (kFlagBlock / 64) + 1;
+            HIP_OK(S[M_CHUNKS].ensure(n_chunks * 12 + 16));
+            unsigned long long *chunk_mask = S[M_CHUNKS].as<unsigned long long>();
+            uint32_t *chunk_pre = reinterpret_cast<uint32_t *>(chunk_mask + n_chunks);
+            m_index = MIndex{chunk_pre, chunk_mask};
             HIP_OK(S[MARK_M].ensure(std::max(((size_t)E + 2) * 4, padded)));
             uint8_t *multi = S[MARK_M].as<uint8_t>();
             HIP_OK(hipMemsetAsync(multi, 0, padded, stream));
-            hipLaunchKernelGGL(k_id_store, dim3(blocks_for((E + 3) / 4)), dim3(TPB), 0, stream, raw, eloc, id_base, id_negmin,
-                               sc, dense, hist, (reinterpret_cast<uintptr_t>(raw.read_ids) & 15u) == 0 ? 1 : 0);
-            hipLaunchKernelGGL(k_id_check, dim3(blocks_for((E + 3) / 4)), dim3(TPB), 0, stream, E, sc, dense, hist, multi);
+            hipLaunchKernelGGL(k_id_store, dim3(blocks_for((E + 3) / 4)), dim3(TPB), 0, stream, raw, chr_entry, id_base,
+                               id_negmin, sc, hist, ids_aligned);
+            hipLaunchKernelGGL(k_id_check, dim3(blocks_for((E + 3) / 4)), dim3(TPB), 0, stream, raw, chr_entry, id_base,
+                               id_negmin, sc, hist, multi, ids_aligned);
             for (int a : {M_ENTRY, RID_M, IDB_M, ELOC_M, ARANK_M}) HIP_OK(S[a].ensure((size_t)E * 4 + 16));
             HIP_OK(S[DENSE_M].ensure(((size_t)6 * (E / 2 + 1) + 8) * 4));
             m_entry = S[M_ENTRY].as<uint32_t>();
             uint32_t *block_sum = grouped, *block_off = grouped + n_flag_blocks + 1;
             hipLaunchKernelGGL(k_flag_count, dim3(n_flag_blocks), dim3(TPB), 0, stream, multi, block_sum);
-            hipLaunchKernelGGL(k_flag_scan, dim3(1), dim3(TPB_SCAN), 0, stream, block_sum, n_flag_blocks, block_off, m_idx + E,
-                               sc);
-            hipLaunchKernelGGL(k_compact_m, dim3(n_flag_blocks), dim3(TPB), 0, stream, raw, multi, block_off, m_idx, m_entry);
+            hipLaunchKernelGGL(k_flag_scan, dim3(1), dim3(TPB_SCAN), 0, stream, block_sum, n_flag_blocks, block_off,
+                               chunk_pre + (n_chunks - 1), sc);
+            hipLaunchKernelGGL(k_compact_m, dim3(n_flag_blocks), dim3(TPB), 0, stream, raw, multi, block_off, chunk_pre,
+                               chunk_mask, m_entry);
             HIP_OK(read_scalars(pk, stream, sc, nullptr, &hsc, nullptr));
             if (hsc.error == 3) return "positions must be strictly increasing within a chromosome";
             if (hsc.id_exceeded) {
@@ -1810,9 +1856,11 @@
                 pk.split_pays = false;
                 pk.calls_without_split = 0;
                 n_m = E;
-                m_idx = nullptr;
+                m_index = MIndex{nullptr, nullptr};
                 m_entry = nullptr;
                 HIP_OK(hipMemsetAsync(hist, 0, (id_space + 1) * 4, stream));
+                const std::string err = make_entry_locus();
+                if (!err.empty()) return err;
             }
         }
         if (split_singles) {
@@ -1826,9 +1874,9 @@
                 uint32_t *count_m = S[DENSE_M].as<uint32_t>(), *goff = count_m + n_m + 1, *winner_m = goff + n_m + 1;
                 uint32_t *g_begin = winner_m + n_m, *g_len = g_begin + n_m, *members = g_len + n_m;
                 HIP_OK(hipMemsetAsync(count_m, 0, ((size_t)n_m + 1) * 4, stream));
-                hipLaunchKernelGGL(k_m_fields, dim3(blocks_for(n_m)), dim3(TPB), 0, stream, raw, eloc, dense, hist, m_idx, m_entry,
-                                   n_m, S[RID_M].as<uint32_t>(), S[IDB_M].as<uint32_t>(), S[ELOC_M].as<uint32_t>(), winner_m,
-                                   count_m);
+                hipLaunchKernelGGL(k_m_fields, dim3(blocks_for(n_m)), dim3(TPB), 0, stream, raw, chr_entry, id_base, id_negmin,
+                                   hist, m_index, m_entry, n_m, S[RID_M].as<uint32_t>(), S[IDB_M].as<uint32_t>(),
+                                   S[ELOC_M].as<uint32_t>(), winner_m, count_m);
                 cub_cap = S[CUB].bytes;
                 HIP_OK(hipcub::DeviceScan::ExclusiveSum(cub_tmp, cub_cap, count_m, goff, (int)n_m + 1, stream));
                 hipLaunchKernelGGL(k_group_scatter, dim3(blocks_for(n_m)), dim3(TPB), 0, stream, winner_m, n_m, goff, count_m,
@@ -1856,6 +1904,7 @@
     }
     const unsigned long long *skey = key_b;
     const uint32_t *sval = val_b;
+    pk.used_single_entry = split_singles;
 
     uint32_t *keep = work_a;
     unsigned long long *incl = reinterpret_cast<unsigned long long *>(work_b);
@@ -1875,7 +1924,7 @@
     HIP_OK(pk.blk_off.ensure((n_off_max + 1) * 4));
     uint32_t *read_off = pk.read_off.as<uint32_t>(), *read_locus = pk.read_locus.as<uint32_t>();
     uint8_t *read_base = pk.read_base.as<uint8_t>();
-    const Ranks ranks{split_singles ? m_idx : nullptr, split_singles ? arank : nullptr, arank};
+    const Ranks ranks{m_index, split_singles ? arank : nullptr, arank};
     auto build_reads = [&]() -> std::string {
         uint32_t *mark_sub = split_singles ? S[MARK_M].as<uint32_t>() : mark;
         if (n_m) {
@@ -2056,7 +2105,7 @@
         const size_t g2p_bytes = ((size_t)in.n_groups * 2 + 15) / 16 * 16;
         const bool g2p_lds = g2p_allowed && num_cells <= 0xFFFFu && lds + g2p_bytes <= 49152;
         hipLaunchKernelGGL(k_bin_hist, dim3(g2p_lds ? std::min<uint32_t>(locus_grid, 1024) : locus_grid), dim3(TPB),
-                           lds + (g2p_lds ? g2p_bytes : 0), stream, raw, nb, TL, entry_kc, m_idx, num_cells, B_log2, blk_cnt,
+                           lds + (g2p_lds ? g2p_bytes : 0), stream, raw, nb, TL, entry_kc, m_index.chunk_mask, num_cells, B_log2, blk_cnt,
                            sc, g2p_lds ? 1u : 0u);
     }
     if (n_m)
@@ -2198,6 +2247,7 @@
                                hipStream_t stream, DevicePacked *out, bool *need_host) {
     *need_host = false;
     out->flag_lists_built = false;
+    out->used_single_entry = false;
     if ((in.id_base16 != nullptr) == (in.id_base32 != nullptr))
         return "exactly one of id_base16 / id_base32 must be given";
     if (num_threads == 0) return "num_threads must be positive";
diff --git a/secedo_amd/csrc/pack_device.hpp b/secedo_amd/csrc/pack_device.hpp
--- a/secedo_amd/csrc/pack_device.hpp
+++ b/secedo_amd/csrc/pack_device.hpp
@@ -59,6 +59,7 @@
     uint64_t id_space_hint = 0;
     bool split_pays = true;
     uint32_t calls_without_split = 0;
+    bool used_single_entry = false;
     hipStream_t side = nullptr;
     hipEvent_t ev_fork = nullptr, ev_join = nullptr, ev_offsets = nullptr, ev_flush = nullptr;
     struct FlagListBuffers {
diff --git a/secedo_amd/csrc/simmat_api.cpp b/secedo_amd/csrc/simmat_api.cpp
--- a/secedo_amd/csrc/simmat_api.cpp
+++ b/secedo_amd/csrc/simmat_api.cpp
@@ -367,6 +367,9 @@
 }
 
 int secedo_simmat_used_device_packing(const secedo_simmat_t *h) { return h ? h->used_device_packing : 0; }
+int secedo_simmat_used_single_entry_path(const secedo_simmat_t *h) {
+    return h && h->used_device_packing && h->pk.used_single_entry ? 1 : 0;
+}
 
 int secedo_simmat_prepare(secedo_simmat_t *h, uint32_t num_cells, uint32_t max_fragment_length,
                           uint32_t num_threads, uint32_t block_cells, void *stream) {
diff --git a/secedo_amd/similarity_matrix.py b/secedo_amd/similarity_matrix.py
--- a/secedo_amd/similarity_matrix.py
+++ b/secedo_amd/similarity_matrix.py
@@ -120,6 +120,10 @@
     def used_device_packing(self) -> bool:
         return bool(_lib.lib().secedo_simmat_used_device_packing(self._h))
 
+    @property
+    def used_single_entry_path(self) -> bool:
+        return bool(_lib.lib().secedo_simmat_used_single_entry_path(self._h))
+
     def upload(self, pos_data, group_id_to_pos=None, num_cells=None):
         p = _as_flat(pos_data)
         t = self._torch
```

Result: faster. 804.0 billion updates/s (median of 6 runs) (+2.5%).
